# ruanjue/smartdenovo

Hardware: AMD Instinct MI355X
Metric: Gbp of candidate pairs aligned/sec (wtzmo all-vs-all) (higher is better)
Workload: dtype int32/int16

## Files before the change

### smartdenovo_amd/csrc/wtz_ctx.h

```cpp
struct wtz_switches {
	uint32_t xcd_group = 256;
	int zread = 1;
	int ext_fused = 1;
	int ext_pk = 1;
	int heavy_first = -1;
	int gap_lane = 1;
	int lane = 1;
	bool trace = false;
	bool fail_once = false;
	unsigned fail_at = 0, tfail_at = 0;
	int dm_first_big = 1;
	int sw_mode = 0;
	int gap_side = 0;
	bool profile = false;
};
static int env_int(const char *name, int dflt){ const char *e = getenv(name); return e ? atoi(e) : dflt; }
static void wtz_switches_read(wtz_switches *s){
	s->xcd_group = (uint32_t)env_int("WTZ_XCD_GROUP", (int)s->xcd_group);
	s->zread = env_int("WTZ_ZREAD", s->zread);
	s->ext_fused = env_int("WTZ_EXT_FUSED", s->ext_fused);
	s->ext_pk = env_int("WTZ_EXT_PK", s->ext_pk);
	s->heavy_first = env_int("WTZ_PAIR_HEAVY_FIRST", s->heavy_first);
	s->gap_lane = env_int("WTZ_GAP_LANE", s->gap_lane);
	s->lane = env_int("WTZ_WINALIGN_LANE", s->lane);
	s->trace = getenv("WTZ_STAGE_TRACE") != NULL;
	s->fail_once = getenv("WTZ_POOL_FAIL_ONCE") != NULL;
	s->fail_at = (unsigned)env_int("WTZ_POOL_FAIL_AT", 0);
	s->tfail_at = (unsigned)env_int("WTZ_TPOOL_FAIL_AT", 0);
#ifndef WTZ_EMUL
	s->dm_first_big = env_int("WTZ_DM_FIRST_BIG", s->dm_first_big);
	s->sw_mode = env_int("WTZ_SW_CHECK", 0) ? 2 : env_int("WTZ_SW_SCALAR", 0) ? 1 : 0;
	s->gap_side = env_int("WTZ_GAP_SIDESTREAM", 0) ? 1 : 0;
	s->profile = getenv("WTZ_PROFILE_PAIR") != NULL;
#endif
}

struct wtz_ctx {
	int device = 0;
	wtz_switches sw;
	struct zslot_t {
		std::vector<std::pair<void*, size_t> > parked, live;
		uint64_t *zoff = NULL; uint64_t n_z = 0; wtz_zindex_t Z; bool have = false; bool sub = false; uint64_t sub_cap = 0;
		std::vector<uint32_t> members;
		zslot_t(){ memset(&Z, 0, sizeof Z); }
		bool holds(uint32_t r) const { return have && (!sub || std::binary_search(members.begin(), members.end(), r)); }
	} zs[2];
#ifndef WTZ_EMUL
	hipStream_t stream = 0;
	hipStream_t stream_side = 0; hipEvent_t ev_side_fork = 0, ev_side_join = 0;
	hipStream_t stream_gap = 0; hipEvent_t ev_gap_fork = 0, ev_gap_join = 0;
#endif
	bool shares_indexes = false;
	void *kpark_p[2] = {NULL, NULL}; size_t kpark_b[2] = {0, 0}, klive_b[2] = {0, 0};
	wtz_arena arena;
	uint32_t cap_pairs = 0, cap_items = 0;
	wtz_params_t P = wtz_params_t(); wtz_params_t *dP = NULL;
	uint64_t *bits = NULL; uint64_t n_words = 0; uint64_t *rdoff = NULL; uint32_t *rdlen = NULL; uint32_t n_reads = 0;
	std::vector<uint32_t> h_rdlen;
	wtz_kslot_t *ktab = NULL; uint64_t kmask = 0; uint32_t *kseeds = NULL; uint64_t n_kocc = 0;
	uint64_t *pend_keys = NULL; uint32_t *pend_vals = NULL; uint64_t pend_tot = 0; uint64_t *pend_dk = NULL, *pend_dstart = NULL; uint32_t *pend_dc = NULL; uint64_t pend_nd = 0; uint32_t pend_beg = 0, pend_end = 0;
	uint64_t *cq_gptr = NULL; uint32_t cq_gcap = 0; bool cq_groups = false; std::vector<uint32_t> cq_ng;
	uint32_t idx_beg = 0, idx_end = 0; bool idx_len_sorted = false;
	wtz_pool_t *dpool = NULL; uint8_t *pool_base = NULL; uint64_t pool_bytes = 0, main_bytes = 0;
	uint32_t *d_qid = NULL, *d_cid = NULL; wtz_pairres_t *d_pairres = NULL; uint32_t n_pairs = 0; std::vector<wtz_pairres_t> h_pairres;
	wtz_alnres_dev_t *d_alnres = NULL; uint32_t n_items = 0; std::vector<wtz_alnres_dev_t> h_alnres;
	char *d_text = NULL; size_t cap_text = 0;
#ifndef WTZ_EMUL
	hipStream_t stream_copy = 0; hipEvent_t ev_text_ready = 0, ev_text_done[2] = {0, 0}; std::atomic<uint64_t> text_begun{0}, text_known_done{0}, text_ended{0};
#endif
	bool have_pairs = false, have_items = false;
	uint32_t *cq_thr = NULL;
	uint32_t *cq_q = NULL, *cq_nc = NULL; uint64_t *cq_cand = NULL; unsigned long long *cq_bytes = NULL; uint32_t cq_cap = 0, cq_n = 0; bool cq_pending = false; wtz_timer cq_tm;
	wtz_counters_t cnt = wtz_counters_t();
	uint64_t tpool_peak_call = 0, main_used_call = 0;
	int last_pool_fail = 0;
	double ext_use_ratio = 0.4; uint64_t tpool_last_used = 0;
	bool fused_ran = false;
	unsigned long long ext_fr_total = 0;
	unsigned long long ext_open_total = 0;
};

#ifndef WTZ_EMUL
#define CTX_ENTER(c) (void)hipSetDevice((c)->device); g_stream = (c)->stream; wtz_arena_scope arena_scope_(&(c)->arena)
#else
#define CTX_ENTER(c) wtz_arena_scope arena_scope_(&(c)->arena)
#endif

#define STAGE(c, name) do { if((c)->sw.trace){ (void)dev_sync(); fprintf(stderr, "[stage] %s\n", name); fflush(stderr); } } while(0)

static wtz_reads_t ctx_reads(const wtz_ctx *c){ wtz_reads_t R; R.bits = c->bits; R.rdoff = c->rdoff; R.rdlen = c->rdlen; R.n_reads = c->n_reads; return R; }
static wtz_env_t ctx_env(const wtz_ctx *c){ wtz_env_t V; V.R = ctx_reads(c); V.Z = c->zs[0].Z; V.ZQ = c->zs[1].have ? c->zs[1].Z : c->zs[0].Z; V.P = c->dP; V.pool = c->dpool; V.dm_first_big = (uint32_t)c->sw.dm_first_big; return V; }

static int tpool_reset(wtz_ctx *c){
	wtz_pool_t p; wtz_pool_init(&p, c->pool_base + c->main_bytes, c->pool_bytes - c->main_bytes, c->sw.tfail_at);
	return dev_h2d(c->dpool + 1, &p, sizeof p);
}
static int pool_reset(wtz_ctx *c){
	wtz_pool_t p; wtz_pool_init(&p, c->pool_base, c->main_bytes, c->sw.fail_at);
	CHK(dev_h2d(c->dpool, &p, sizeof p));
	c->tpool_peak_call = 0;
	return tpool_reset(c);
}
static int tpool_check(wtz_ctx *c, const char *stage){
	wtz_pool_t p; CHK(dev_d2h(&p, c->dpool + 1, sizeof p));
	const uint64_t u = p.used > p.cap ? p.cap : p.used;
	c->tpool_last_used = u;
	if(u > c->tpool_peak_call) c->tpool_peak_call = u;
	if(p.overflow && c->sw.fail_once) c->sw.tfail_at = 0;
	if(p.overflow) c->last_pool_fail = 2;
	if(p.overflow) return wtz_fail(WTZ_E_POOL, "%s: transient trace pool exhausted (%llu of %llu bytes requested); use a larger pool",
		stage, (unsigned long long)p.used, (unsigned long long)p.cap);
	return WTZ_OK;
}
static int pool_check(wtz_ctx *c, const char *stage){
	wtz_pool_t p; CHK(dev_d2h(&p, c->dpool, sizeof p));
	const uint64_t u = (p.used > p.cap ? p.cap : p.used);
	c->main_used_call = u;
	if(u + c->tpool_peak_call > c->cnt.pool_peak) c->cnt.pool_peak = u + c->tpool_peak_call;
	if(p.overflow && c->sw.fail_once) c->sw.fail_at = 0;
	if(p.overflow) c->last_pool_fail = 1;
	if(p.overflow) return wtz_fail(WTZ_E_POOL, "%s: device scratch pool exhausted (%llu of %llu bytes requested); use fewer items per call or a larger pool",
		stage, (unsigned long long)p.used, (unsigned long long)p.cap);
	return WTZ_OK;
}
extern "C" int wtz_device_count(void){
#ifndef WTZ_EMUL
	int n = 0; if(hipGetDeviceCount(&n) != hipSuccess) return 0; return n;
#else
	return 1;
#endif
}

extern "C" int wtz_device_memory(int device, uint64_t *free_bytes, uint64_t *total_bytes){
	if(!free_bytes || !total_bytes) return wtz_fail(WTZ_E_ARG, "null argument");
#ifndef WTZ_EMUL
	int prev = 0; HIPCHK(hipGetDevice(&prev)); HIPCHK(hipSetDevice(device));
	size_t fr = 0, tot = 0; const hipError_t e = hipMemGetInfo(&fr, &tot); (void)hipSetDevice(prev);
	if(e != hipSuccess) return wtz_fail(WTZ_E_HIP, "hipMemGetInfo: %s", hipGetErrorString(e));
	*free_bytes = fr; *total_bytes = tot;
#else
	(void)device; *free_bytes = *total_bytes = 16ull << 30;
#endif
	return WTZ_OK;
}

extern "C" int wtz_ctx_create(int device, const wtz_params_c *params, uint64_t pool_bytes, wtz_ctx_t **out){
	if(!params || !out) return wtz_fail(WTZ_E_ARG, "null argument");
	if(params->ksize < 5 || params->ksize > 32 || params->zsize < 5 || params->zsize > 16 || params->ksave < 1) return wtz_fail(WTZ_E_ARG, "k/z/S out of range (wtzmo.c:1658-1660)");
#ifndef WTZ_EMUL
	int ndev = 0;
	if(hipGetDeviceCount(&ndev) != hipSuccess || ndev == 0) return wtz_fail(WTZ_E_HIP, "no HIP device visible: libwtzmo_hip needs an MI355X (gfx950); there is no CPU fallback");
	if(device < 0 || device >= ndev) return wtz_fail(WTZ_E_ARG, "device %d out of range (%d visible)", device, ndev);
	HIPCHK(hipSetDevice(device));
#endif
	wtz_ctx *c = new wtz_ctx();
	c->device = device; c->P = *params; wtz_switches_read(&c->sw);
	c->pool_bytes = pool_bytes ? pool_bytes : (4ull << 30);
#ifndef WTZ_EMUL
	if(!pool_bytes){
		size_t fr = 0, tot = 0;
		if(hipMemGetInfo(&fr, &tot) == hipSuccess && fr / 20 * 9 > c->pool_bytes) c->pool_bytes = (uint64_t)(fr / 20 * 9);
		if(c->pool_bytes > (128ull << 30)) c->pool_bytes = 128ull << 30;
		if(const char *e = getenv("WTZ_DEFAULT_POOL_MB")){ const long long mb = atoll(e); if(mb >= 64 && ((uint64_t)mb << 20) < c->pool_bytes) c->pool_bytes = (uint64_t)mb << 20; }
	}
#endif
	c->pool_bytes &= ~(uint64_t)4095; c->main_bytes = (c->pool_bytes / 2) & ~(uint64_t)4095;
#ifndef WTZ_EMUL
	{ void *ab = NULL; const size_t acap = (size_t)3 << 29;
	  if(hipMalloc(&ab, acap) == hipSuccess){ c->arena.base = (uint8_t*)ab; c->arena.cap = acap; } }
	if(hipStreamCreateWithFlags(&c->stream, hipStreamNonBlocking) != hipSuccess
			|| hipStreamCreateWithFlags(&c->stream_side, hipStreamNonBlocking) != hipSuccess || hipEventCreateWithFlags(&c->ev_side_fork, hipEventDisableTiming) != hipSuccess
			|| hipEventCreateWithFlags(&c->ev_side_join, hipEventDisableTiming) != hipSuccess
			|| hipStreamCreateWithFlags(&c->stream_gap, hipStreamNonBlocking) != hipSuccess || hipEventCreateWithFlags(&c->ev_gap_fork, hipEventDisableTiming) != hipSuccess
			|| hipEventCreateWithFlags(&c->ev_gap_join, hipEventDisableTiming) != hipSuccess){ wtz_ctx_destroy(c); return wtz_fail(WTZ_E_HIP, "hipStreamCreate / hipEventCreate failed"); }
	g_stream = c->stream;
#endif
	int rc;
	if((rc = dev_alloc_persist((void**)&c->dP, sizeof(wtz_params_t))) || (rc = dev_h2d(c->dP, &c->P, sizeof(wtz_params_t))) ||
	   (rc = dev_alloc_persist((void**)&c->dpool, 2 * sizeof(wtz_pool_t)))){
		wtz_ctx_destroy(c); return rc;
	}
	for(;;){
#ifndef WTZ_EMUL
		if(!pool_bytes && c->pool_bytes > (4ull << 30)){
			if(hipMalloc((void**)&c->pool_base, c->pool_bytes) == hipSuccess){ rc = WTZ_OK; break; }
			(void)hipGetLastError();
			c->pool_base = NULL;
			uint64_t nb = c->pool_bytes / 2; if(nb < (4ull << 30)) nb = 4ull << 30;
			c->pool_bytes = nb & ~(uint64_t)4095; c->main_bytes = (c->pool_bytes / 2) & ~(uint64_t)4095;
			continue;
		}
#endif
		rc = dev_alloc_persist((void**)&c->pool_base, c->pool_bytes);
		break;
	}
	if(rc || (rc = pool_reset(c))){
		wtz_ctx_destroy(c); return rc;
	}
	*out = c;
	return WTZ_OK;
}

static void free_pending_index(wtz_ctx *c);
static void kpark(wtz_ctx *c, int w, void *p, size_t bytes){ if(!p) return; if(c->kpark_p[w]) dev_free_persist(c->kpark_p[w]); c->kpark_p[w] = p; c->kpark_b[w] = bytes; }
static void kflush(wtz_ctx *c){ for(int w = 0; w < 2; w++){ if(c->kpark_p[w]) dev_free_persist(c->kpark_p[w]); c->kpark_p[w] = NULL; c->kpark_b[w] = 0; } }
static int kalloc(wtz_ctx *c, int w, void **p, size_t n){
	if(c->kpark_p[w] && c->kpark_b[w] >= n && c->kpark_b[w] <= n + n / 8 + ((size_t)1 << 20)){ *p = c->kpark_p[w]; c->klive_b[w] = c->kpark_b[w]; c->kpark_p[w] = NULL; c->kpark_b[w] = 0; return WTZ_OK; }
	if(c->kpark_p[w]){ dev_free_persist(c->kpark_p[w]); c->kpark_p[w] = NULL; c->kpark_b[w] = 0; }
	int rc = dev_alloc_persist(p, n); if(rc == WTZ_OK) c->klive_b[w] = n; return rc;
}
static void free_kindex(wtz_ctx *c){
	if(!c->shares_indexes){
		if(c->klive_b[0]) kpark(c, 0, c->ktab, c->klive_b[0]); else dev_free_persist(c->ktab);
		if(c->klive_b[1]) kpark(c, 1, c->kseeds, c->klive_b[1]); else dev_free_persist(c->kseeds);
		c->klive_b[0] = c->klive_b[1] = 0;
	}
	c->ktab = NULL; c->kseeds = NULL; c->kmask = 0;
}
static int zalloc(wtz_ctx::zslot_t *z, void **p, size_t n){
	if(n == 0) n = 16;
	for(size_t i = 0; i < z->parked.size(); i++){
		if(z->parked[i].second >= n && z->parked[i].second <= n + n / 8 + 4096){
			*p = z->parked[i].first; z->live.push_back(z->parked[i]); z->parked.erase(z->parked.begin() + (long)i); return WTZ_OK;
		}
	}
	int rc = dev_alloc_persist(p, n); if(rc) return rc;
	z->live.push_back(std::make_pair(*p, n)); return WTZ_OK;
}
static void zpark_all(wtz_ctx::zslot_t *z){ for(size_t i = 0; i < z->live.size(); i++) z->parked.push_back(z->live[i]); z->live.clear(); }
static void zflush_parked(wtz_ctx::zslot_t *z){ for(size_t i = 0; i < z->parked.size(); i++) dev_free_persist(z->parked[i].first); z->parked.clear(); }
static void free_zindex(wtz_ctx *c){
	for(int k = 0; k < 2; k++){
		wtz_ctx::zslot_t *z = &c->zs[k];
		if(!c->shares_indexes){ zpark_all(z); zflush_parked(z); }
		z->zoff = NULL; memset(&z->Z, 0, sizeof z->Z); z->have = false; z->sub = false; z->sub_cap = 0; z->n_z = 0; z->members.clear();
	}
}
static void free_batch(wtz_ctx *c){ c->n_pairs = 0; c->n_items = 0; c->have_pairs = false; c->have_items = false; }
static void free_batch_storage(wtz_ctx *c){
	dev_free_persist(c->d_qid); dev_free_persist(c->d_cid); dev_free_persist(c->d_pairres); dev_free_persist(c->d_alnres);
	c->d_qid = c->d_cid = NULL; c->d_pairres = NULL; c->d_alnres = NULL; c->cap_pairs = c->cap_items = 0; free_batch(c);
}
static int reserve_pairs(wtz_ctx *c, uint32_t n){
	if(n <= c->cap_pairs && c->d_pairres) return WTZ_OK;
	uint32_t cap = c->cap_pairs ? c->cap_pairs : 4096; while(cap < n) cap *= 2;
	(void)dev_sync();
	dev_free_persist(c->d_qid); dev_free_persist(c->d_cid); dev_free_persist(c->d_pairres); c->d_qid = c->d_cid = NULL; c->d_pairres = NULL; c->cap_pairs = 0;
	CHK(dev_alloc_persist((void**)&c->d_qid, (size_t)cap * 4)); CHK(dev_alloc_persist((void**)&c->d_cid, (size_t)cap * 4));
	CHK(dev_alloc_persist((void**)&c->d_pairres, (size_t)cap * sizeof(wtz_pairres_t)));
	c->cap_pairs = cap; return WTZ_OK;
}
static int reserve_items(wtz_ctx *c, uint32_t m){
	if(m <= c->cap_items && c->d_alnres) return WTZ_OK;
	uint32_t cap = c->cap_items ? c->cap_items : 4096; while(cap < m) cap *= 2;
	(void)dev_sync();
	dev_free_persist(c->d_alnres); c->d_alnres = NULL; c->cap_items = 0;
	CHK(dev_alloc_persist((void**)&c->d_alnres, (size_t)cap * sizeof(wtz_alnres_dev_t)));
	c->cap_items = cap; return WTZ_OK;
}

extern "C" void wtz_ctx_destroy(wtz_ctx_t *c){
	if(!c) return;
	{ CTX_ENTER(c); (void)dev_sync(); }
	free_batch_storage(c); free_kindex(c); if(!c->shares_indexes) kflush(c); free_zindex(c);
	dev_free_persist(c->d_text);
	dev_free_persist(c->cq_q); dev_free_persist(c->cq_nc); dev_free_persist(c->cq_cand); dev_free_persist(c->cq_bytes); dev_free_persist(c->cq_thr); dev_free_persist(c->cq_gptr);
	free_pending_index(c);
#ifndef WTZ_EMUL
	arena_cache_flush(&c->arena);
	if(c->arena.base) (void)hipFree(c->arena.base);
#endif
	if(!c->shares_indexes){ dev_free_persist(c->bits); dev_free_persist(c->rdoff); dev_free_persist(c->rdlen); }
	dev_free_persist(c->dP); dev_free_persist(c->dpool); dev_free_persist(c->pool_base);
#ifndef WTZ_EMUL
	if(c->stream_side) (void)hipStreamDestroy(c->stream_side);
	if(c->stream_gap) (void)hipStreamDestroy(c->stream_gap);
	if(c->stream_copy){ (void)hipStreamSynchronize(c->stream_copy); (void)hipStreamDestroy(c->stream_copy); if(c->ev_text_ready) (void)hipEventDestroy(c->ev_text_ready); for(int k = 0; k < 2; k++) if(c->ev_text_done[k]) (void)hipEventDestroy(c->ev_text_done[k]); }
	{ hipEvent_t evs[4] = { c->ev_side_fork, c->ev_side_join, c->ev_gap_fork, c->ev_gap_join }; for(int k = 0; k < 4; k++) if(evs[k]) (void)hipEventDestroy(evs[k]); }
	if(c->stream) (void)hipStreamDestroy(c->stream);
#endif
	delete c;
}

extern "C" int wtz_ctx_clone(wtz_ctx_t *p, uint64_t pool_bytes, wtz_ctx_t **out){
	if(!p || !out) return wtz_fail(WTZ_E_ARG, "null argument");
	wtz_ctx_t *c = NULL;
	int rc = wtz_ctx_create(p->device, &p->P, pool_bytes ? pool_bytes : p->pool_bytes, &c);
	if(rc) return rc;
	c->shares_indexes = true;
	c->bits = p->bits; c->n_words = p->n_words; c->rdoff = p->rdoff; c->rdlen = p->rdlen; c->n_reads = p->n_reads; c->h_rdlen = p->h_rdlen;
	c->ktab = p->ktab; c->kmask = p->kmask; c->kseeds = p->kseeds; c->n_kocc = p->n_kocc;
	c->idx_beg = p->idx_beg; c->idx_end = p->idx_end; c->idx_len_sorted = p->idx_len_sorted;
	for(int k = 0; k < 2; k++){ c->zs[k].zoff = p->zs[k].zoff; c->zs[k].n_z = p->zs[k].n_z; c->zs[k].Z = p->zs[k].Z; c->zs[k].have = p->zs[k].have; c->zs[k].sub = p->zs[k].sub; c->zs[k].members = p->zs[k].members; }
	*out = c;
	return WTZ_OK;
}
```

### smartdenovo_amd/csrc/wtz_lib_align.h

```cpp
#ifndef WTZ_EMUL
WTZ_HD uint64_t wtz_ext_trace_need(int32_t qlen, int32_t tlen, int32_t init, int32_t W, int32_t M, int32_t O, int32_t E, int32_t T, int32_t *ql_out, int32_t *ncol_out){
	if(ql_out) *ql_out = 0;
	if(ncol_out) *ncol_out = 0;
	if(qlen <= 0 || tlen <= 0) return 0;
	if(init < 0) init = 0;
	int32_t ql, tl, n_col;
	wtz_ext_geometry(qlen, tlen, init, W, M, O, O, E, T, ql, tl, n_col);
	if(ql_out) *ql_out = ql;
	if(ncol_out) *ncol_out = n_col;
	const uint64_t c_reg = ((uint64_t)(n_col + 63) / 64 + 3) / 4, c_mw = ((uint64_t)(n_col + 255) / 256 + 3) / 4 * 4, c_gen = ((((uint64_t)(n_col + 63) / 64) | 1) + 3) / 4;
	uint64_t zrow = (c_reg > c_gen ? c_reg : c_gen) * 256; if(c_mw * 256 > zrow) zrow = c_mw * 256;
	uint64_t nb = ((uint64_t)(ql + 63) / 64) * 64 * zrow + (uint64_t)WTZ_TRACE_MAXCHUNK * 8 + (uint64_t)(ql + 2) * 4 + 256;
	if((n_col + 63) / 64 > 32 || (tl + 63) / 32 + 1 > 1032){
		uint64_t z = 1024; while(z < (uint64_t)ql * (uint64_t)n_col) z <<= 1;
		uint64_t r = 64; while(r < (uint64_t)tl + 3) r <<= 1;
		uint64_t zb = 64; while(zb < (uint64_t)ql + 2) zb <<= 1;
		nb = z + 8 * r + 4 * zb + 256;
	}
	return nb;
}
static uint64_t ext_trace_need(const wtz_ctx *c, int32_t qlen, int32_t tlen, int32_t init, int32_t W, int32_t *ql_out, int32_t *ncol_out){
	return wtz_ext_trace_need(qlen, tlen, init, W, c->P.M, c->P.O, c->P.E, c->P.T, ql_out, ncol_out);
}

static int run_stitch_fused(wtz_ctx *c, const wtz_env_t &V, const wtz_alnitem_t *d_items, wtz_stitch_state_t *d_st, wtz_extjob_t *d_jl, wtz_extjob_t *d_jr, const wtz_gapres_t *d_gaps, const int32_t *d_rgeo, uint32_t m){
	c->fused_ran = false;
	if(m == 0) return WTZ_OK;
	uint64_t *d_k = NULL; uint32_t *d_order = NULL; unsigned long long *d_acc = NULL;
	uint32_t *d_open = NULL;
	CHK(dev_alloc((void**)&d_k, (size_t)m * 8)); CHK(dev_alloc((void**)&d_order, (size_t)m * 4)); CHK(dev_alloc((void**)&d_acc, 24)); CHK(dev_set(d_acc, 0, 24));
	if(c->sw.ext_pk) CHK(dev_alloc((void**)&d_open, ((size_t)m + 1) * 4));
	{
		const int32_t pM = c->P.M, pO = c->P.O, pE = c->P.E, pT = c->P.T, pW = -c->P.ew;
		const bool use_pk = c->sw.ext_pk != 0; const wtz_params_t *dP = V.P;
		CHK(wtz_launch<K_misc>(m, [=] WTZ_LAMBDA (uint64_t t){
			const wtz_extjob_t &j = d_jl[t];
			int32_t qa = 0, qb = 0;
			unsigned long long nb = wtz_ext_trace_need(j.valid ? j.qlen : -1, j.tlen, 0, pW, pM, pO, pE, pT, &qa, (int32_t*)NULL);
			nb += wtz_ext_trace_need(d_rgeo[2 * t], d_rgeo[2 * t + 1], 0, pW, pM, pO, pE, pT, &qb, (int32_t*)NULL);
			const uint32_t rows = (uint32_t)qa + (uint32_t)qb;
			uint32_t to_fr = 0;
			if(use_pk){
				if(j.valid && j.qlen > 0 && j.tlen > 0){
					int32_t W = pW, ql = 0, tl = 0, nc = 0, bias, ng, sh; const int32_t in0 = j.init_score < 0 ? 0 : j.init_score;
					wtz_ext_geometry(j.qlen, j.tlen, in0, W, pM, pO, pO, pE, pT, ql, tl, nc);
					if(!wtz_pk_window(dP, in0, ql, tl, &bias, &ng, &sh)) to_fr = 1;
				}
				if(d_rgeo[2 * t] > 0 && d_rgeo[2 * t + 1] > 0){
					const wtz_stitch_state_t &st = d_st[t]; const wtz_alnitem_t &it = d_items[t];
					long long i_lo = st.x.score, gain = 0;
					if(j.valid && j.qlen > 0 && j.tlen > 0) gain = (long long)pM * (j.qlen < j.tlen ? j.qlen : j.tlen);
					const wtz_gapres_t *gp = d_gaps + (it.regs - d_items[0].regs);
					for(uint32_t k = st.first + 1; k < it.nwin; k++) if(it.regs[k].pass == 1) i_lo += (long long)gp[k].score + it.regs[k].x.score;
					int32_t W = pW, ql = 0, tl = 0, nc = 0;
					wtz_ext_geometry(d_rgeo[2 * t], d_rgeo[2 * t + 1], 0, W, pM, pO, pO, pE, pT, ql, tl, nc);
					if(!wtz_pk_window_range(dP, ql, tl, i_lo, i_lo + gain)) to_fr = 1;
				}
			}
			d_k[t] = ((uint64_t)to_fr << 32) | (uint64_t)(0xFFFFFFFFu - rows); d_order[t] = (uint32_t)t;
			if(to_fr) WTZ_ATOMIC_ADD64(&d_acc[2], 1ull);
			if(nb) WTZ_ATOMIC_ADD64(&d_acc[0], nb);
			if(rows) WTZ_ATOMIC_ADD64(&d_acc[1], (unsigned long long)rows);
		}));
	}
	CHK(dev_sort_pairs_u64_u32(d_k, d_order, m, 33));
	unsigned long long h_acc[3] = {0, 0, 0}; CHK(dev_d2h(h_acc, d_acc, 24));
	const uint64_t acc = h_acc[0]; const unsigned long long ext_sum = h_acc[1];
	const uint64_t budget = (c->pool_bytes - c->main_bytes) / 16 * 15;
	uint32_t ng = 1; while(ng < 4 && (double)acc * c->ext_use_ratio / ng > (double)budget) ng++;
	if((double)acc * c->ext_use_ratio / ng > (double)budget){ if(c->sw.profile) fprintf(stderr, "[ext-profile] fused launch declined: %u items, trace bounds %.1f GB x %.2f against %.1f GB\n", m, acc / 1e9, c->ext_use_ratio, budget / 1e9); return WTZ_OK; }
	double ms_l = 0; uint64_t used_sum = 0;
	for(uint32_t g = 0; g < ng; g++){
		const uint32_t mg = (m - g + ng - 1) / ng;
		if(mg == 0) continue;
		CHK(tpool_reset(c));
		wtz_timer te; te.start();
		if(c->sw.ext_pk){
			uint32_t n_fr = ng == 1 ? (uint32_t)h_acc[2] : 0u;
			if(n_fr > mg) n_fr = mg;
			CHK(dev_set(d_open, 0, 4));
			if(n_fr){
				HIPCHK(hipEventRecord(c->ev_side_fork, g_stream)); HIPCHK(hipStreamWaitEvent(c->stream_side, c->ev_side_fork, 0));
				WTZ_LAUNCH((wtz_kernel_stitch_ext_fr<1032>), n_fr, 64, WTZ_WAVE_LDS_BYTES, c->stream_side, V, d_items, d_st, d_jl, d_jr, d_gaps, (const uint32_t*)d_order + (mg - n_fr), n_fr, 1u, 0u);
				HIPCHK(hipEventRecord(c->ev_side_join, c->stream_side));
			}
			const uint32_t n_pk = mg - n_fr;
			if(n_pk){
				WTZ_LAUNCH((wtz_kernel_stitch_ext_pk<1032>), n_pk, 64, WTZ_PK_LDS_BYTES(1032), g_stream, V, d_items, d_st, d_jl, d_jr, d_gaps, (const uint32_t*)d_order, n_pk, ng, g, d_open);
			}
			if(n_fr) HIPCHK(hipStreamWaitEvent(g_stream, c->ev_side_join, 0));
			uint32_t n_open = 0; CHK(dev_d2h(&n_open, d_open, 4));
			c->ext_open_total += n_open; c->ext_fr_total += n_fr;
			if(n_open){ WTZ_LAUNCH((wtz_kernel_stitch_ext_fr<1032>), n_open, 64, WTZ_WAVE_LDS_BYTES, g_stream, V, d_items, d_st, d_jl, d_jr, d_gaps, (const uint32_t*)d_open + 1, n_open, 1u, 0u); }
		} else WTZ_LAUNCH((wtz_kernel_stitch_ext_fr<1032>), mg, 64, WTZ_WAVE_LDS_BYTES, g_stream, V, d_items, d_st, d_jl, d_jr, d_gaps, (const uint32_t*)d_order, mg, ng, g);
		ms_l += te.stop();
		{
			const int rc_t = tpool_check(c, "K-sw3 extension jobs (both ends on one wavefront)");
			if(rc_t != WTZ_OK){
				c->ext_use_ratio = c->ext_use_ratio * 2.0 > 1.0 ? 1.0 : c->ext_use_ratio * 2.0;
				return rc_t;
			}
		}
		used_sum += c->tpool_last_used;
	}
	c->cnt.ms_ext += ms_l; c->cnt.n_extjobs += 2ull * m;
	c->fused_ran = true;
	if(c->sw.profile) fprintf(stderr, "[ext-profile] fused launch: %u items in %u group(s), rows (upper bound) sum %llu, %.2f ms; items of the 32-bit form so far: dealt %llu, declined by the packed form %llu\n", m, ng, ext_sum, ms_l, c->ext_fr_total, c->ext_open_total);
	c->tpool_last_used = used_sum;
	if(acc){ const double seen = 1.3 * (double)c->tpool_last_used / (double)acc, keep = c->ext_use_ratio * 0.9; c->ext_use_ratio = seen > keep ? seen : keep; if(c->ext_use_ratio < 0.2) c->ext_use_ratio = 0.2; if(c->ext_use_ratio > 1.0) c->ext_use_ratio = 1.0; }
	return WTZ_OK;
}
#endif

static int run_extjobs(wtz_ctx *c, const wtz_env_t &V, wtz_extjob_t *d_jobs, uint32_t m, bool leftover = false){
	if(m == 0) return WTZ_OK;
#ifdef WTZ_EMUL
	(void)c; (void)leftover;
	return wtz_launch_wave<K_extjob_scalar>(m, [=] WTZ_LAMBDA (uint64_t t){ wtz_task_extjob_scalar((uint32_t)t, V, d_jobs); });
#else
	if(leftover){
		if(!c->fused_ran) leftover = false;
		else {
			wtz_timer te; te.start();
			WTZ_LAUNCH((wtz_kernel_extjobs<2048, 1032>), m, 64, 0, g_stream, d_jobs, (const uint32_t*)NULL, m, V.P, V.pool, V.pool + 1);
			c->cnt.ms_ext += te.stop();
			return tpool_check(c, "K-sw3 extension jobs");
		}
	}
	const int mode = c->sw.sw_mode;
	if(mode == 1) return wtz_launch_wave<K_extjob_scalar>(m, [=] WTZ_LAMBDA (uint64_t t){ wtz_task_extjob_scalar((uint32_t)t, V, d_jobs); });
	std::vector<wtz_extjob_t> ref;
	if(mode == 2){
		wtz_extjob_t *d_copy = NULL; CHK(dev_alloc((void**)&d_copy, (size_t)m * sizeof(wtz_extjob_t)));
		HIPCHK(hipMemcpyAsync(d_copy, d_jobs, (size_t)m * sizeof(wtz_extjob_t), hipMemcpyDeviceToDevice, g_stream));
		CHK(wtz_launch_wave<K_extjob_scalar>(m, [=] WTZ_LAMBDA (uint64_t t){ wtz_task_extjob_scalar((uint32_t)t, V, d_copy); }));
		CHK(dev_sync());
		ref.resize(m); CHK(dev_d2h(ref.data(), d_copy, (size_t)m * sizeof(wtz_extjob_t)));
	}
	uint32_t *d_order = NULL; unsigned long long ext_sum = 0; int32_t ext_max = 0;
	std::vector<uint32_t> ord(m); std::vector<uint64_t> need(m); std::vector<uint8_t> cw(m, 0);
	unsigned long long geo_n[9] = {0}, geo_rows[9] = {0}, geo_cells[9] = {0};
	{
		int32_t *d_key = NULL; CHK(dev_alloc((void**)&d_key, (size_t)m * 16));
		CHK(wtz_launch<K_misc>(m, [=] WTZ_LAMBDA (uint64_t t){ const wtz_extjob_t &j = d_jobs[t]; d_key[4 * t] = j.valid ? j.qlen : -1; d_key[4 * t + 1] = j.tlen; d_key[4 * t + 2] = j.init_score; d_key[4 * t + 3] = j.W; }));
		std::vector<int32_t> key4((size_t)m * 4); CHK(dev_d2h(key4.data(), d_key, (size_t)m * 16));
		std::vector<int32_t> key(m);
		for(uint32_t i = 0; i < m; i++){ key[i] = key4[(size_t)i * 4]; if(key[i] > 0){ ext_sum += (unsigned long long)key[i]; if(key[i] > ext_max) ext_max = key[i]; } }
		std::vector<int32_t> rows(m, -1);
		for(uint32_t i = 0; i < m; i++){
			const int32_t qlen = key4[(size_t)i * 4], tlen = key4[(size_t)i * 4 + 1];
			need[i] = 0;
			if(qlen <= 0 || tlen <= 0) continue;
			int32_t ql = 0, n_col = 0;
			need[i] = ext_trace_need(c, qlen, tlen, key4[(size_t)i * 4 + 2], key4[(size_t)i * 4 + 3], &ql, &n_col);
			cw[i] = (uint8_t)((n_col + 63) / 64 > 255 ? 255 : (n_col + 63) / 64);
			rows[i] = ql;
			if(c->sw.profile){ const int b = (n_col + 63) / 64 > 32 ? 8 : ((n_col + 63) / 64 - 1) / 4; geo_n[b]++; geo_rows[b] += (unsigned long long)ql; geo_cells[b] += (unsigned long long)ql * (unsigned long long)n_col; }
		}
		for(uint32_t i = 0; i < m; i++) ord[i] = i;
		std::stable_sort(ord.begin(), ord.end(), [&](uint32_t a, uint32_t b){ return rows[a] > rows[b]; });
		CHK(dev_alloc((void**)&d_order, (size_t)m * 4)); CHK(dev_h2d(d_order, ord.data(), (size_t)m * 4));
		if(c->sw.profile){
			fprintf(stderr, "[ext-profile] geometry by columns per lane (upper bounds):");
			for(int b = 0; b < 9; b++) if(geo_n[b]) fprintf(stderr, " C<=%d: %llu jobs %.1f Mrows %.1f Gcells;", b < 8 ? 4 * b + 4 : 999, geo_n[b], (double)geo_rows[b] / 1e6, (double)geo_cells[b] / 1e9);
			fprintf(stderr, "\n");
		}
	}
	{
		wtz_timer te; te.start();
		const uint64_t budget = (c->pool_bytes - c->main_bytes) / 16 * 15;
		uint32_t g0 = 0, n_groups = 0;
		while(g0 < m){
			uint32_t g1 = g0; uint64_t acc = 0;
			while(g1 < m && (g1 == g0 || acc + need[ord[g1]] <= budget)){ acc += need[ord[g1]]; g1++; }
			CHK(tpool_reset(c));
			if(c->sw.ext_pk){
				WTZ_LAUNCH((wtz_kernel_extjobs_pk<1032>), g1 - g0, 64, 0, g_stream, d_jobs, (const uint32_t*)d_order + g0, g1 - g0, V.P, V.pool, V.pool + 1);
			}
			WTZ_LAUNCH((wtz_kernel_extjobs_fr<1032>), g1 - g0, 64, 0, g_stream, d_jobs, (const uint32_t*)d_order + g0, g1 - g0, V.P, V.pool, V.pool + 1);
			WTZ_LAUNCH((wtz_kernel_extjobs<2048, 1032>), g1 - g0, 64, 0, g_stream, d_jobs, (const uint32_t*)d_order + g0, g1 - g0, V.P, V.pool, V.pool + 1);
			if(g1 < m || n_groups){ CHK(dev_sync()); CHK(tpool_check(c, "K-sw3 extension jobs")); }
			g0 = g1; n_groups++;
		}
		const double ms_l = te.stop();
		CHK(tpool_check(c, "K-sw3 extension jobs"));
		c->cnt.ms_ext += ms_l; c->cnt.n_extjobs += m;
		if(c->sw.profile){
			std::vector<int32_t> key(m); uint32_t nv = 0, n256 = 0, n512 = 0, n1k = 0, n2k = 0, n4k = 0; unsigned long long s512 = 0;
			CHK(dev_sync());
			{ std::vector<wtz_extjob_t> jj(m); CHK(dev_d2h(jj.data(), d_jobs, (size_t)m * sizeof(wtz_extjob_t))); uint32_t nd[4] = {0, 0, 0, 0}; for(uint32_t i = 0; i < m; i++){ key[i] = jj[i].valid ? jj[i].x.qe : -1; if(jj[i].valid) nd[jj[i].done & 3]++; }
			  if(const char *dp = getenv("WTZ_EXT_DUMP")){
				if(FILE *df = fopen(dp, "ab")){ for(uint32_t i = 0; i < m; i++) if(jj[i].valid){ const int32_t r[8] = {jj[i].qlen, jj[i].tlen, jj[i].init_score, jj[i].W, jj[i].x.qe, jj[i].x.te, (int32_t)(jj[i].cells > 0x7FFFFFFFull ? 0x7FFFFFFF : jj[i].cells), (int32_t)jj[i].done}; fwrite(r, 4, 8, df); } fclose(df); } }
			  fprintf(stderr, "[ext-profile] %u launch group(s); valid jobs finished by: nobody %u, 32-bit frame form %u, packed form or general kernel %u\n", n_groups, nd[0], nd[1], nd[3]); }
			for(uint32_t i = 0; i < m; i++){ if(key[i] < 0) continue; nv++; if(key[i] >= 256) n256++; if(key[i] >= 512){ n512++; s512 += key[i]; } if(key[i] >= 1024) n1k++; if(key[i] >= 2048) n2k++; if(key[i] >= 4096) n4k++; }
			fprintf(stderr, "[ext-profile] %u jobs (%u valid), rows (upper bound) sum %llu max %d, %.2f ms; qe>=256 %u >=512 %u (sum %llu) >=1k %u >=2k %u >=4k %u; transient pool peak %.2f GB\n", m, nv, ext_sum, ext_max, ms_l, n256, n512, s512, n1k, n2k, n4k, c->tpool_peak_call / 1073741824.0);
		}
	}
	if(mode == 2){
		CHK(dev_sync());
		std::vector<wtz_extjob_t> got(m); CHK(dev_d2h(got.data(), d_jobs, (size_t)m * sizeof(wtz_extjob_t)));
		for(uint32_t i = 0; i < m; i++){
			if(!got[i].valid) continue;
			if(memcmp(&got[i].x, &ref[i].x, sizeof(wtz_aln_t)) || got[i].cigar_len != ref[i].cigar_len || got[i].cells != ref[i].cells)
				return wtz_fail(WTZ_E_STATE, "K-sw3 wave kernel differs from the scalar body on job %u: qlen %d tlen %d init %d W %d; score %d/%d qe %d/%d te %d/%d aln %d/%d cigar %u/%u cells %llu/%llu",
					i, got[i].qlen, got[i].tlen, got[i].init_score, got[i].W, got[i].x.score, ref[i].x.score, got[i].x.qe, ref[i].x.qe, got[i].x.te, ref[i].x.te,
					got[i].x.aln, ref[i].x.aln, got[i].cigar_len, ref[i].cigar_len, (unsigned long long)got[i].cells, (unsigned long long)ref[i].cells);
			if(got[i].cigar_len){
				std::vector<uint32_t> a(got[i].cigar_len), b(got[i].cigar_len);
				CHK(dev_d2h(a.data(), got[i].cigar, a.size() * 4)); CHK(dev_d2h(b.data(), ref[i].cigar, b.size() * 4));
				if(a != b) return wtz_fail(WTZ_E_STATE, "K-sw3 wave kernel: CIGAR differs on job %u", i);
			}
		}
	}
	return WTZ_OK;
#endif
}

#ifdef WTZ_EMUL
#define WTZ_HOST_WAVE 1u
#else
#define WTZ_HOST_WAVE 64u
#endif
static int pool_alloc_host(wtz_ctx *c, int which, size_t bytes, void **out){
	unsigned long long *d_p = NULL; CHK(dev_alloc((void**)&d_p, 8));
	wtz_pool_t *pool = c->dpool + which;
	CHK(wtz_launch<K_poolalloc>(1, [=] WTZ_LAMBDA (uint64_t){ *d_p = (unsigned long long)(uintptr_t)wtz_pool_alloc(pool, bytes); }));
	unsigned long long h = 0; CHK(dev_d2h(&h, d_p, 8));
	if(h == 0) return wtz_fail(WTZ_E_POOL, "device scratch pool exhausted (%zu bytes for the K-sw1 problem lists)", bytes);
	*out = (void*)(uintptr_t)h; return WTZ_OK;
}
static uint32_t lane_classes(const uint32_t ccnt[4], wtz_lclass_t *L){
	uint32_t lo = 0, wv = 0;
	for(int k = 0; k < 4; k++){ const uint32_t n = ccnt[3 - k]; L->lo[k] = lo; L->hi[k] = lo + n; wv += (n + WTZ_HOST_WAVE - 1) / WTZ_HOST_WAVE; L->wend[k] = wv; lo += n; }
	return wv;
}
static size_t carve_bytes(size_t n, size_t elem){ return (n * elem + 255) & ~(size_t)255; }
template<typename T> static void carve(uint8_t *&blk, T *&out, size_t n){ out = (T*)blk; blk += carve_bytes(n, sizeof(T)); }
template<typename KEYS> static int sort_leftovers(uint32_t *d_list, uint32_t nl, KEYS launch_keys){
	if(nl <= 64) return WTZ_OK;
	uint64_t *d_k2 = NULL; CHK(dev_alloc((void**)&d_k2, (size_t)nl * 8));
	CHK(launch_keys(d_k2));
	return dev_sort_pairs_u64_u32(d_k2, d_list + 1, nl, 32);
}
static int run_winalign_lane(wtz_ctx *c, const wtz_env_t &V, const wtz_wintask_t *d_wt, uint64_t nwt, const wtz_alnitem_t *d_items, uint32_t *d_fb, uint32_t *n_fb){
	*n_fb = 0;
	if(nwt == 0) return WTZ_OK;
	const bool prof = c->sw.profile; double tp[8] = {0, 0, 0, 0, 0, 0, 0, 0}, tp0 = 0;
	if(prof){ (void)dev_sync(); tp0 = wtz_wall(); }
	auto lap = [&](int k){ if(prof){ (void)dev_sync(); const double t = wtz_wall(); tp[k] += t - tp0; tp0 = t; } };
	uint32_t *d_na = NULL, *d_woff = NULL;
	CHK(dev_alloc((void**)&d_na, (nwt + 1) * 4)); CHK(dev_alloc((void**)&d_woff, (nwt + 1) * 4));
	CHK(dev_set(d_na, 0, (nwt + 1) * 4));
	CHK(wtz_launch<K_lcount>(nwt, [=] WTZ_LAMBDA (uint64_t t){ wtz_task_lcount((uint32_t)t, d_wt, d_items, d_na); }));
	CHK(dev_exclusive_scan_u32(d_na, d_woff, nwt + 1));
	uint32_t NS = 0; CHK(dev_d2h(&NS, d_woff + nwt, 4));
	lap(0);
	wtz_lprob_t *d_prob = NULL; uint32_t *d_cap = NULL, *d_roff = NULL, *d_val = NULL, *d_ccnt = NULL, *d_uidx = NULL, *d_nu = NULL; uint64_t *d_key = NULL; uint8_t *d_flag = NULL; wtz_lres_t *d_res = NULL;
	{
		const size_t nsp = (size_t)NS + 64;
		uint8_t *blk = NULL; CHK(pool_alloc_host(c, 0, carve_bytes(nsp, sizeof(wtz_lprob_t)) + carve_bytes(nsp, sizeof(wtz_lres_t)) + 4 * carve_bytes(nsp, 4) + carve_bytes(nsp, 8), (void**)&blk));
		carve(blk, d_prob, nsp); carve(blk, d_res, nsp); carve(blk, d_cap, nsp); carve(blk, d_roff, nsp); carve(blk, d_val, nsp); carve(blk, d_uidx, nsp); carve(blk, d_key, nsp);
	}
	CHK(dev_alloc((void**)&d_flag, nwt + 16)); CHK(dev_alloc((void**)&d_nu, (nwt + 1) * 4)); CHK(dev_alloc((void**)&d_ccnt, 32)); CHK(dev_set(d_ccnt, 0, 32));
	CHK(dev_set(d_cap, 0, ((size_t)NS + 1) * 4));
	CHK(dev_set(d_res, 0, ((size_t)NS + 1) * sizeof(wtz_lres_t)));
	CHK(wtz_launch<K_lplan>(nwt, [=] WTZ_LAMBDA (uint64_t t){ wtz_task_lplan((uint32_t)t, V, d_wt, d_items, d_woff, d_prob, d_cap, d_key, d_val, d_flag, d_ccnt, d_uidx, d_nu); }));
	lap(1);
	CHK(dev_exclusive_scan_u32(d_cap, d_roff, (uint64_t)NS + 1));
	uint32_t NR = 0, ccnt[4] = {0, 0, 0, 0};
	CHK(dev_d2h(&NR, d_roff + NS, 4)); CHK(dev_d2h(ccnt, d_ccnt, 16));
	uint32_t *d_runs = NULL; CHK(pool_alloc_host(c, 0, ((size_t)NR + 16) * 4, (void**)&d_runs));
	lap(2);
	CHK(dev_sort_pairs_u64_u32(d_key, d_val, NS, 16));
	lap(3);
	CHK(dev_set(d_fb, 0, 4));
	{
		const uint32_t *d_ord = d_val; const wtz_lprob_t *pp = d_prob; const uint32_t *ro = d_roff; uint32_t *rn = d_runs; wtz_lres_t *rs = d_res;
		wtz_lclass_t L; const uint32_t wv = lane_classes(ccnt, &L);
		uint64_t *d_wtr = NULL; uint32_t *d_wrm = NULL;
		CHK(dev_alloc((void**)&d_wtr, ((size_t)wv + 1) * 8)); CHK(dev_alloc((void**)&d_wrm, ((size_t)wv + 1) * 4)); CHK(dev_set(d_wtr, 0, ((size_t)wv + 1) * 8));
		if(wv) CHK(wtz_launch_coop<K_ldp>(wv, [=] WTZ_LAMBDA (uint64_t t){ wtz_task_ldp_all((uint32_t)t, L, V, d_wt, d_items, d_ord, pp, rs, d_wtr, d_wrm); }, 0));
		lap(4);
		if(wv) CHK(wtz_launch_coop<K_ltb>(wv, [=] WTZ_LAMBDA (uint64_t t){ wtz_task_ltb_all((uint32_t)t, L, V, d_wt, d_items, d_ord, pp, ro, rn, rs, d_wtr, d_wrm); }, 0));
		lap(6);
		CHK(wtz_launch<K_lfold>(nwt, [=] WTZ_LAMBDA (uint64_t t){ wtz_task_lfold((uint32_t)t, V, d_wt, d_items, d_woff, pp, ro, rn, rs, d_flag, d_fb, d_uidx, d_nu); }));
	}
	CHK(dev_d2h(n_fb, d_fb, 4));
	{
		const uint32_t nl = *n_fb; const uint32_t *lst = d_fb + 1;
		CHK(sort_leftovers(d_fb, nl, [&](uint64_t *d_k2){ return wtz_launch<K_misc>(nl, [=] WTZ_LAMBDA (uint64_t i){
			const wtz_wintask_t tk = d_wt[lst[i]];
			const wtz_win_t &w = d_items[tk.item].win[tk.widx];
			d_k2[i] = 0xFFFFFFFFull - (unsigned long long)(w.anchors[1] - w.anchors[0]);
		}); }));
	}
	lap(5);
	if(c->sw.profile) fprintf(stderr, "[lane-profile] %llu windows, %u anchor slots, K-sw1 problems by band class <=16 / <=32 / <=64 / <=104: %u / %u / %u / %u, %u run entries, %u windows left to the chained kernel; ms: count+scan %.2f plan %.2f scan+alloc %.2f sort %.2f dp %.2f traceback %.2f fold %.2f\n",
		(unsigned long long)nwt, NS, ccnt[0], ccnt[1], ccnt[2], ccnt[3], NR, *n_fb, tp[0] * 1e3, tp[1] * 1e3, tp[2] * 1e3, tp[3] * 1e3, tp[4] * 1e3, tp[6] * 1e3, tp[5] * 1e3);
	return WTZ_OK;
}

static int run_gap_lane(wtz_ctx *c, const wtz_env_t &V, const wtz_wintask_t *d_wt, uint64_t nwt, const wtz_alnitem_t *d_items, wtz_gapres_t *d_gaps, uint32_t *d_list, uint32_t *n_list){
	*n_list = 0;
	if(nwt == 0) return WTZ_OK;
	wtz_lgap_t *d_gp = NULL; uint32_t *d_cap = NULL, *d_roff = NULL, *d_val = NULL, *d_ccnt = NULL; uint64_t *d_key = NULL; uint8_t *d_done = NULL;
	{
		const size_t nsp = (size_t)nwt + 64;
		uint8_t *blk = NULL; CHK(pool_alloc_host(c, 0, carve_bytes(nsp, sizeof(wtz_lgap_t)) + 3 * carve_bytes(nsp, 4) + carve_bytes(nsp, 8) + carve_bytes(nsp, 1), (void**)&blk));
		carve(blk, d_gp, nsp); carve(blk, d_cap, nsp); carve(blk, d_roff, nsp); carve(blk, d_val, nsp); carve(blk, d_key, nsp); carve(blk, d_done, nsp);
	}
	CHK(dev_alloc((void**)&d_ccnt, 32)); CHK(dev_set(d_ccnt, 0, 32));
	CHK(dev_set(d_cap, 0, ((size_t)nwt + 1) * 4));
	CHK(wtz_launch<K_gplan>(nwt, [=] WTZ_LAMBDA (uint64_t t){ wtz_task_gplan((uint32_t)t, V, d_wt, d_items, d_gaps, d_gp, d_cap, d_key, d_val, d_done, d_ccnt); }));
	CHK(dev_exclusive_scan_u32(d_cap, d_roff, nwt + 1));
	uint32_t NR = 0, ccnt[4] = {0, 0, 0, 0};
	CHK(dev_d2h(&NR, d_roff + nwt, 4)); CHK(dev_d2h(ccnt, d_ccnt, 16));
	uint32_t *d_runs = NULL; CHK(pool_alloc_host(c, 0, ((size_t)NR + 16) * 4, (void**)&d_runs));
	CHK(dev_sort_pairs_u64_u32(d_key, d_val, nwt, 18));
	CHK(dev_set(d_list, 0, 4));
	{
		const uint32_t *d_ord = d_val; const wtz_lgap_t *gp = d_gp; const uint32_t *ro = d_roff; uint32_t *rn = d_runs; uint8_t *dn = d_done;
		wtz_lclass_t L; const uint32_t wv = lane_classes(ccnt, &L);
		uint64_t *d_wtr = NULL; uint32_t *d_wrm = NULL; wtz_lres_t *d_res = NULL;
		CHK(dev_alloc((void**)&d_wtr, ((size_t)wv + 1) * 8)); CHK(dev_alloc((void**)&d_wrm, ((size_t)wv + 1) * 4)); CHK(dev_set(d_wtr, 0, ((size_t)wv + 1) * 8));
		CHK(pool_alloc_host(c, 0, ((size_t)nwt + 1) * sizeof(wtz_lres_t), (void**)&d_res)); CHK(dev_set(d_res, 0, ((size_t)nwt + 1) * sizeof(wtz_lres_t)));
		if(wv) CHK(wtz_launch_coop<K_gdp>(wv, [=] WTZ_LAMBDA (uint64_t t){ wtz_task_gdp_all((uint32_t)t, L, V, d_wt, d_items, d_ord, gp, d_res, d_wtr, d_wrm); }, 0));
		if(wv) CHK(wtz_launch_coop<K_gtb>(wv, [=] WTZ_LAMBDA (uint64_t t){ wtz_task_gtb_all((uint32_t)t, L, V, d_wt, d_items, d_ord, gp, ro, rn, d_res, d_gaps, dn, d_wtr, d_wrm); }, 0));
		CHK(wtz_launch<K_glist>(nwt, [=] WTZ_LAMBDA (uint64_t t){ wtz_task_glist((uint32_t)t, dn, d_list); }));
	}
	CHK(dev_d2h(n_list, d_list, 4));
	{
		const uint32_t nl = *n_list; const wtz_lgap_t *gp = d_gp; const uint32_t *lst = d_list + 1;
		CHK(sort_leftovers(d_list, nl, [&](uint64_t *d_k2){ return wtz_launch<K_misc>(nl, [=] WTZ_LAMBDA (uint64_t i){
			const wtz_lgap_t G = gp[lst[i]];
			const int32_t nc = G.dq < 2 * G.w + 1 ? G.dq : 2 * G.w + 1;
			unsigned long long wgt = (unsigned long long)(G.dt > 0 ? G.dt : 0) * (unsigned long long)((nc > 0 ? nc : 0) / 64 + 1);
			if(wgt > 0xFFFFFFFEull) wgt = 0xFFFFFFFEull;
			d_k2[i] = 0xFFFFFFFFull - wgt;
		}); }));
	}
	if(c->sw.profile) fprintf(stderr, "[lane-profile] %llu window slots, K-sw2 gaps by band class <=16 / <=32 / <=64 / <=104: %u / %u / %u / %u, %u left to the wavefront kernel\n",
		(unsigned long long)nwt, ccnt[0], ccnt[1], ccnt[2], ccnt[3], *n_list);
	return WTZ_OK;
}

static int run_winalign_chained(wtz_ctx *c, const wtz_env_t &V, const wtz_wintask_t *d_wt, const wtz_alnitem_t *d_items, uint32_t *d_list, uint64_t n, uint32_t *n_redone = NULL){
	if(n_redone) *n_redone = 0;
	if(n == 0) return WTZ_OK;
#ifdef WTZ_EMUL
	if(d_list) return wtz_launch_coop<K_winalign>(n, [=] WTZ_LAMBDA (uint64_t t){ wtz_task_winalign((uint32_t)t, V, d_wt, d_items, (uint32_t*)NULL, d_list); }, WTZ_WINALIGN_LDS_BYTES + WTZ_WINALIGN_QW_BYTES);
	return wtz_launch_coop<K_winalign>(n, [=] WTZ_LAMBDA (uint64_t t){ wtz_task_winalign((uint32_t)t, V, d_wt, d_items); }, WTZ_WINALIGN_LDS_BYTES + WTZ_WINALIGN_QW_BYTES);
#else
	uint32_t *d_defer = NULL, n_def = 0; CHK(dev_alloc((void**)&d_defer, ((size_t)n + 1) * 4)); CHK(dev_set(d_defer, 0, 4));
	if(d_list) CHK(wtz_launch_coop<K_winalign>(n, [=] WTZ_LAMBDA (uint64_t t){ wtz_task_winalign<false>((uint32_t)t, V, d_wt, d_items, d_defer, d_list); }, WTZ_WINALIGN_LDS_BYTES + WTZ_WINALIGN_QW_BYTES));
	else CHK(wtz_launch_coop<K_winalign>(n, [=] WTZ_LAMBDA (uint64_t t){ wtz_task_winalign<false>((uint32_t)t, V, d_wt, d_items, d_defer, NULL); }, WTZ_WINALIGN_LDS_BYTES + WTZ_WINALIGN_QW_BYTES));
	CHK(dev_d2h(&n_def, d_defer, 4));
	if(n_def) CHK(wtz_launch_coop<K_winalign_big>(n_def, [=] WTZ_LAMBDA (uint64_t t){ wtz_task_winalign<true>((uint32_t)t, V, d_wt, d_items, NULL, d_defer); }, WTZ_WINALIGN_LDS_BYTES + WTZ_WINALIGN_QW_BYTES));
	if(n_redone) *n_redone = n_def;
	return WTZ_OK;
#endif
}

static int compare_lane_with_chained(const wtz_reg_t *ra, const wtz_reg_t *rb, uint64_t nreg){
	unsigned int *d_bad = NULL; CHK(dev_alloc((void**)&d_bad, 16)); CHK(dev_set(d_bad, 0, 16));
	CHK(wtz_launch<K_misc>(nreg, [=] WTZ_LAMBDA (uint64_t i){
		const wtz_reg_t &a = ra[i], &b = rb[i];
		bool same = a.pass == 2 || b.pass == 2 || (a.x.score == b.x.score && a.x.tb == b.x.tb && a.x.te == b.x.te && a.x.qb == b.x.qb && a.x.qe == b.x.qe && a.x.aln == b.x.aln && a.x.mat == b.x.mat && a.x.mis == b.x.mis && a.x.ins == b.x.ins && a.x.del == b.x.del && a.pass == b.pass && a.cigar_len == b.cigar_len && (a.cells == b.cells || a.cells == 0 || b.cells == 0));
		if(same && a.pass != 2 && b.pass != 2) for(uint32_t k = 0; k < a.cigar_len; k++) if(a.cigar[k] != b.cigar[k]){ same = false; break; }
		if(!same){ const unsigned int z = WTZ_ATOMIC_INC32(&d_bad[0]); if(z == 0) d_bad[1] = (unsigned int)i; }
	}));
	unsigned int hb[4]; CHK(dev_d2h(hb, d_bad, 16));
	if(hb[0]){
		wtz_reg_t a, b; CHK(dev_d2h(&a, ra + hb[1], sizeof a)); CHK(dev_d2h(&b, rb + hb[1], sizeof b));
		return wtz_fail(WTZ_E_STATE, "K-sw1 lane pipeline differs from the chained kernel on %u of %llu windows; first: window slot %u chained/lane score %d/%d tb %d/%d te %d/%d qb %d/%d qe %d/%d aln %d/%d mat %d/%d mis %d/%d ins %d/%d del %d/%d cigar %u/%u pass %u/%u cells %llu/%llu",
			hb[0], (unsigned long long)nreg, hb[1], a.x.score, b.x.score, a.x.tb, b.x.tb, a.x.te, b.x.te, a.x.qb, b.x.qb, a.x.qe, b.x.qe, a.x.aln, b.x.aln, a.x.mat, b.x.mat, a.x.mis, b.x.mis, a.x.ins, b.x.ins, a.x.del, b.x.del, a.cigar_len, b.cigar_len, a.pass, b.pass, a.cells, b.cells);
	}
	return WTZ_OK;
}

static int run_gap_wave(wtz_ctx *c, const wtz_env_t &V, const wtz_wintask_t *d_wt, const wtz_alnitem_t *d_items, wtz_gapres_t *d_gaps, const uint32_t *d_glist, uint32_t n_glist, uint64_t nwt){
#ifdef WTZ_EMUL
	(void)c; (void)nwt;
	return wtz_launch_coop<K_gap>(n_glist, [=] WTZ_LAMBDA (uint64_t t){ wtz_task_gap((uint32_t)t, V, d_wt, d_items, d_gaps, (uint32_t*)NULL, (const uint32_t*)d_glist); }, WTZ_GAP_LDS_BYTES);
#else
	uint32_t *d_defer = NULL, n_def = 0; CHK(dev_alloc((void**)&d_defer, (size_t)(nwt + 1) * 4)); CHK(dev_set(d_defer, 0, 4));
	STAGE(c, "K_gap");
	CHK(wtz_launch_coop<K_gap>(n_glist, [=] WTZ_LAMBDA (uint64_t t){ wtz_task_gap((uint32_t)t, V, d_wt, d_items, d_gaps, d_defer, (const uint32_t*)d_glist, 0u); }, WTZ_GAP_LDS_BYTES));
	CHK(dev_d2h(&n_def, d_defer, 4));
	if(n_def) CHK(wtz_launch_coop<K_gap_wide>(n_def, [=] WTZ_LAMBDA (uint64_t t){ wtz_task_gap((uint32_t)t, V, d_wt, d_items, d_gaps, NULL, d_defer, (uint32_t)WTZ_GAP_WIDE_LDS_BYTES); }, WTZ_GAP_WIDE_LDS_BYTES));
	if(c->sw.profile){ CHK(dev_sync()); fprintf(stderr, "[gap-profile] %llu window slots, %u wide gaps redone with 72 KB of LDS\n", (unsigned long long)nwt, n_def); }
	return WTZ_OK;
#endif
}

#ifdef WTZ_EMUL
static int check_right_geometry(const int32_t *d_rgeo, const wtz_extjob_t *d_jr, const wtz_stitch_state_t *d_st, uint32_t m){
	for(uint32_t t = 0; t < m; t++){
		const wtz_extjob_t &jr = d_jr[t];
		const int32_t pq = d_rgeo[2 * (size_t)t], pt = d_rgeo[2 * (size_t)t + 1];
		if(jr.valid ? (pq != jr.qlen || pt != jr.tlen) : (pq >= 0 && !d_st[t].bad))
			return wtz_fail(WTZ_E_STATE, "stitch: predicted right extension of item %u (%d x %d) differs from the one K_stitch_mid asks for (valid %u: %d x %d)", t, pq, pt, jr.valid, jr.qlen, jr.tlen);
	}
	return WTZ_OK;
}
#endif

extern "C" int wtz_pairs_align(wtz_ctx_t *c, const uint32_t *pair_idx, const uint8_t *dir, uint32_t m, wtz_aln_result_t *out){
	if(!c || !c->have_pairs) return wtz_fail(WTZ_E_STATE, "wtz_pairs_align before wtz_pairs_seed");
	if(m == 0) return WTZ_OK;
	CTX_ENTER(c);
	if(!pair_idx || !dir || !out) return wtz_fail(WTZ_E_ARG, "null argument");
	c->n_items = 0; c->have_items = false;
	const bool prof_wall = c->sw.profile; double tw[6] = {0, 0, 0, 0, 0, 0}; double tw0 = prof_wall ? wtz_wall() : 0;
	auto lapw = [&](int k){ if(prof_wall){ const double t = wtz_wall(); tw[k] += t - tw0; tw0 = t; } };
	CHK(reserve_items(c, m));
	std::vector<wtz_alnitem_t> items(m); uint64_t nreg = 0;
	std::vector<uint32_t> h_q(c->n_pairs), h_c(c->n_pairs);
	CHK(dev_d2h(h_q.data(), c->d_qid, (size_t)c->n_pairs * 4)); CHK(dev_d2h(h_c.data(), c->d_cid, (size_t)c->n_pairs * 4));
	for(uint32_t i = 0; i < m; i++){
		if(pair_idx[i] >= c->n_pairs || dir[i] > 1) return wtz_fail(WTZ_E_ARG, "align item %u out of range", i);
		const wtz_pairres_t &r = c->h_pairres[pair_idx[i]];
		wtz_alnitem_t it; it.q = h_q[pair_idx[i]]; it.c = h_c[pair_idx[i]]; it.dir = dir[i];
		it.win = r.win[dir[i]]; it.anchors = r.anchors[dir[i]]; it.nwin = r.nwin[dir[i]]; it.regs = (wtz_reg_t*)(uintptr_t)nreg;
		nreg += it.nwin; items[i] = it;
	}
	const uint64_t nwt = (size_t)nreg;
	wtz_reg_t *d_regs = NULL; wtz_alnitem_t *d_items = NULL; wtz_wintask_t *d_wt = NULL;
	CHK(dev_alloc((void**)&d_regs, (size_t)(nreg + 1) * sizeof(wtz_reg_t)));
	for(uint32_t i = 0; i < m; i++) items[i].regs = d_regs + (uintptr_t)items[i].regs;
	CHK(dev_alloc((void**)&d_items, (size_t)m * sizeof(wtz_alnitem_t))); CHK(dev_h2d(d_items, items.data(), (size_t)m * sizeof(wtz_alnitem_t)));
	CHK(dev_alloc((void**)&d_wt, (size_t)(nreg + 1) * sizeof(wtz_wintask_t)));
	{ const wtz_alnitem_t *di = d_items; wtz_wintask_t *dw = d_wt; const wtz_reg_t *r0 = d_regs;
	  CHK(wtz_launch<K_misc>(m, [=] WTZ_LAMBDA (uint64_t i){ const wtz_alnitem_t &it = di[i]; wtz_wintask_t *w = dw + (it.regs - r0); for(uint32_t k = 0; k < it.nwin; k++){ w[k].item = (uint32_t)i; w[k].widx = k; } })); }
	const wtz_env_t V = ctx_env(c); wtz_alnres_dev_t *d_res = c->d_alnres;
	lapw(0);
	wtz_timer tm; tm.start();
	wtz_reg_t *d_regs_chk = NULL;
	if(c->sw.lane){
		uint32_t *d_fb = NULL, n_fb = 0;
		CHK(dev_alloc((void**)&d_fb, (nwt + 1) * 4));
		STAGE(c, "K-sw1 lane pipeline");
		CHK(run_winalign_lane(c, V, d_wt, nwt, d_items, d_fb, &n_fb));
		CHK(run_winalign_chained(c, V, d_wt, d_items, d_fb, n_fb));
		if(c->sw.lane == 2){ CHK(dev_sync()); CHK(dev_alloc((void**)&d_regs_chk, (size_t)(nreg + 1) * sizeof(wtz_reg_t))); CHK(dev_d2d(d_regs_chk, d_regs, (size_t)nreg * sizeof(wtz_reg_t))); }
	}
	if(c->sw.lane == 0 || c->sw.lane == 2){
		uint32_t n_redone = 0;
		STAGE(c, "K_winalign");
		CHK(run_winalign_chained(c, V, d_wt, d_items, NULL, nwt, &n_redone));
		if(c->sw.profile) fprintf(stderr, "[winalign-profile] %zu windows, %u redone by the full task\n", (size_t)nreg, n_redone);
	}
	CHK(dev_sync());
	if(d_regs_chk) CHK(compare_lane_with_chained(d_regs, d_regs_chk, nreg));
	c->cnt.ms_winalign += tm.stop(); c->cnt.n_winalign += (size_t)nreg;
	lapw(1);
	tm.start();
	wtz_stitch_state_t *d_st = NULL; wtz_extjob_t *d_jl = NULL, *d_jr = NULL; wtz_gapres_t *d_gaps = NULL; int32_t *d_rgeo = NULL;
	CHK(dev_alloc((void**)&d_st, (size_t)m * sizeof(wtz_stitch_state_t)));
	CHK(dev_alloc((void**)&d_jl, (size_t)m * sizeof(wtz_extjob_t))); CHK(dev_alloc((void**)&d_jr, (size_t)m * sizeof(wtz_extjob_t)));
	CHK(dev_alloc((void**)&d_gaps, (size_t)(nreg + 1) * sizeof(wtz_gapres_t)));
#ifndef WTZ_EMUL
	const bool fused = c->sw.ext_fused && c->sw.sw_mode == 0, gap_side = c->sw.gap_side != 0;
	if(fused) CHK(dev_alloc((void**)&d_rgeo, (size_t)m * 8));
#else
	const bool fused = false, gap_side = false;
	CHK(dev_alloc((void**)&d_rgeo, (size_t)m * 8));
#endif
	STAGE(c, "K_stitch_left");
	CHK(wtz_launch_wave<K_stitch_left>(m, [=] WTZ_LAMBDA (uint64_t t){ wtz_task_stitch_left((uint32_t)t, V, d_items, d_st, d_jl, d_rgeo); }));
	uint32_t *d_glist = NULL, n_glist = (uint32_t)nwt;
	wtz_timer tgap; tgap.start();
	if(c->sw.gap_lane){
		CHK(dev_alloc((void**)&d_glist, (size_t)(nwt + 1) * 4));
		STAGE(c, "K-sw2 lane pipeline");
		CHK(run_gap_lane(c, V, d_wt, nwt, d_items, d_gaps, d_glist, &n_glist));
	}
#ifndef WTZ_EMUL
	if(gap_side){ HIPCHK(hipEventRecord(c->ev_gap_fork, g_stream)); HIPCHK(hipStreamWaitEvent(c->stream_gap, c->ev_gap_fork, 0)); }
	{ wtz_stream_scope on_gap_stream(gap_side ? c->stream_gap : g_stream); CHK(run_gap_wave(c, V, d_wt, d_items, d_gaps, d_glist, n_glist, nwt)); }
	if(gap_side) HIPCHK(hipEventRecord(c->ev_gap_join, c->stream_gap));
#else
	CHK(run_gap_wave(c, V, d_wt, d_items, d_gaps, d_glist, n_glist, nwt));
#endif
	if(!gap_side) tgap.lap();
#ifndef WTZ_EMUL
	if(fused){
		if(gap_side) HIPCHK(hipStreamWaitEvent(g_stream, c->ev_gap_join, 0));
		STAGE(c, "extjobs left + join + right on one wavefront"); CHK(run_stitch_fused(c, V, d_items, d_st, d_jl, d_jr, d_gaps, d_rgeo, m));
	}
#endif
	STAGE(c, "extjobs left");
	CHK(run_extjobs(c, V, d_jl, m, fused));
#ifndef WTZ_EMUL
	if(gap_side) HIPCHK(hipStreamWaitEvent(g_stream, c->ev_gap_join, 0));
#endif
	if(!gap_side) c->cnt.ms_gap += tgap.read();
	STAGE(c, "K_stitch_mid");
	CHK(wtz_launch_coop<K_stitch_mid>(m, [=] WTZ_LAMBDA (uint64_t t){ wtz_task_stitch_mid((uint32_t)t, V, d_items, d_st, d_jl, d_jr, d_gaps); }));
	STAGE(c, "extjobs right");
#ifdef WTZ_EMUL
	CHK(check_right_geometry(d_rgeo, d_jr, d_st, m));
#endif
	CHK(run_extjobs(c, V, d_jr, m, fused));
	STAGE(c, "K_stitch_fin");
	CHK(wtz_launch_coop<K_stitch_fin>(m, [=] WTZ_LAMBDA (uint64_t t){ wtz_task_stitch_fin((uint32_t)t, V, d_items, d_st, d_jl, d_jr, d_res); }));
	if(c->P.refine) STAGE(c, "K_refine");
	if(c->P.refine) CHK(wtz_launch_coop<K_refine>(m, [=] WTZ_LAMBDA (uint64_t t){ wtz_task_refine((uint32_t)t, V, d_items, d_res); }, WTZ_REFINE_LDS_BYTES));
	CHK(dev_sync());
	c->cnt.ms_stitch += tm.stop(); c->cnt.n_stitch += m;
	lapw(2);
	c->h_alnres.resize(m); c->n_items = m; c->have_items = true;
	CHK(dev_d2h(c->h_alnres.data(), c->d_alnres, (size_t)m * sizeof(wtz_alnres_dev_t)));
	CHK(pool_check(c, "wtz_pairs_align"));
	uint64_t coff = 0, toff = 0;
	for(uint32_t i = 0; i < m; i++){
		const wtz_alnres_dev_t &r = c->h_alnres[i];
		if(r.bad) return wtz_fail(WTZ_E_POOL, "wtz_pairs_align: item %u ran out of scratch", i);
		wtz_aln_result_t o; memset(&o, 0, sizeof o);
		o.score = r.x.score; o.tb = r.x.tb; o.te = r.x.te; o.qb = r.x.qb; o.qe = r.x.qe; o.aln = r.x.aln; o.mat = r.x.mat; o.mis = r.x.mis; o.ins = r.x.ins; o.del = r.x.del;
		o.n_regs = r.n_regs; o.cigar_len = r.cigar_len; o.cigar_off = coff; coff += r.cigar_len; o.text_len = r.text_len; o.text_off = toff; toff += r.text_len;
		c->cnt.cells_shift += r.cells_shift; c->cnt.cells_fixed += r.cells_fixed; c->cnt.cells_global += r.cells_global;
		out[i] = o;
	}
	lapw(3);
	if(prof_wall) fprintf(stderr, "[align-profile] %u items: host wall ms prep %.2f winalign %.2f stitch %.2f results %.2f\n", m, tw[0] * 1e3, tw[1] * 1e3, tw[2] * 1e3, tw[3] * 1e3);
	return WTZ_OK;
}
```

### smartdenovo_amd/csrc/wtz_tasks.h

```cpp
#ifndef WTZ_TASKS_H
#define WTZ_TASKS_H

#include "wtz_sw.h"
#include "wtz_sw_wave.h"
#include "wtz_sw_lane.h"
#include "wtz_dotmatrix.h"

typedef struct {
	wtz_reads_t R; wtz_zindex_t Z; const wtz_params_t *P; wtz_pool_t *pool;
	wtz_zindex_t ZQ;
	uint32_t dm_first_big;
} wtz_env_t;

#define WTZ_WAVE_LDS_BYTES 8192
#ifndef WTZ_GAP_LDS_BYTES
#define WTZ_GAP_LDS_BYTES 12288
#endif
#ifndef WTZ_PAIR_LDS_BYTES
#define WTZ_PAIR_LDS_BYTES 8192
#endif
#ifndef WTZ_PAIR_DM_LDS_BYTES
#define WTZ_PAIR_DM_LDS_BYTES 24576
#endif
#if defined(__HIP_DEVICE_COMPILE__)
WTZ_D int32_t *wtz_wave_scratch(){ extern __shared__ int32_t wtz_dyn_lds[]; return wtz_dyn_lds; }
#else
WTZ_COOP_HOST int32_t *wtz_wave_scratch(){ return NULL; }
#endif

#if defined(WTZ_DEBUG_CRUMBS) && defined(__HIPCC__)
__device__ unsigned int *wtz_crumbs = NULL;
#endif
#if defined(WTZ_DEBUG_CRUMBS) && defined(__HIP_DEVICE_COMPILE__)
#define WTZ_CRUMB(t, code) do { if(wtz_crumbs && WTZ_LANE == 0) __hip_atomic_store(&wtz_crumbs[t], (unsigned int)(code), __ATOMIC_RELAXED, __HIP_MEMORY_SCOPE_SYSTEM); } while(0)
#else
#define WTZ_CRUMB(t, code) do { } while(0)
#endif
#define WTZ_PAIR_NEEDS_ZBIG (-3)
template<int ENGINE = -1, bool ZBIG = true, bool REGION = false>
WTZ_HD void wtz_task_pair(uint32_t t, const wtz_env_t &V, const uint32_t *qid, const uint32_t *cid, wtz_pairres_t *res, const int32_t *reg_beg = NULL, const int32_t *reg_end = NULL){
	const wtz_params_t *P = V.P;
	const int32_t rtb = REGION ? reg_beg[t] : 0, rte = REGION ? reg_end[t] : 0;
	const bool dm = ENGINE < 0 ? (P->dot_matrix != 0) : (ENGINE == 1);
	const uint32_t q = qid[t], c = cid[t];
	wtz_pairres_t r; memset(&r, 0, sizeof r);
	wtz_zhit_t *hits = NULL; uint32_t n = 0;
#if defined(__HIP_DEVICE_COMPILE__)
#define WTZ_TICK() ((uint64_t)clock64())
#else
#define WTZ_TICK() ((uint64_t)0)
#endif
	const uint64_t tk0 = WTZ_TICK();
	WTZ_CRUMB(t, 1);
	const bool aux = P->aux_strand != 0;
#if defined(__HIP_DEVICE_COMPILE__)
	const bool ok0 = wtz_zmatch_coop<REGION>(V.ZQ, V.Z, q, c, V.R.rdlen[c], P->max_kmer_var, V.pool, &hits, &n, aux, (uint32_t*)wtz_wave_scratch(), dm ? (uint32_t)WTZ_PAIR_DM_LDS_BYTES : (uint32_t)WTZ_PAIR_LDS_BYTES, rtb, rte);
#else
	const bool ok0 = wtz_zmatch_coop<REGION>(V.ZQ, V.Z, q, c, V.R.rdlen[c], P->max_kmer_var, V.pool, &hits, &n, aux, NULL, 0, rtb, rte);
#endif
	const bool ok = wtz_coop_bcast32(ok0 ? 1u : 0u) != 0;
	n = wtz_coop_bcast32(n);
	hits = (wtz_zhit_t*)(uintptr_t)wtz_coop_bcast64((uint64_t)(uintptr_t)hits);
	const uint64_t tk1 = WTZ_TICK();
	WTZ_CRUMB(t, 2 | (n << 8));
	wtz_zhit_t *sorted = NULL;
#if defined(__HIP_DEVICE_COMPILE__)
	__threadfence_block();
	if(ok && (aux ? n > 0 : n * P->zsize >= P->ztot)){
		int pbad = 0;
		if(dm) sorted = wtz_sort_hits_wave<1>(hits, n, V.pool, (uint64_t*)wtz_wave_scratch(), WTZ_PAIR_DM_LDS_BYTES / 8, &pbad);
		else              sorted = wtz_sort_hits_wave<0>(hits, n, V.pool, (uint64_t*)wtz_wave_scratch(), WTZ_PAIR_LDS_BYTES / 8, &pbad);
		if(wtz_coop_bcast32((uint32_t)pbad)) r.bad = 1;
		sorted = (wtz_zhit_t*)(uintptr_t)wtz_coop_bcast64((uint64_t)(uintptr_t)sorted);
	}
#endif
	const uint32_t lane = WTZ_LANE;
	WTZ_CRUMB(t, 3 | (n << 8));
	if(!ok || r.bad){ r.bad = 1; if(lane == 0) res[t] = r; WTZ_CRUMB(t, 0xFF); return; }
	r.n_hits = n;
	if(aux ? n == 0 : n * P->zsize < P->ztot){ r.gate = 0; if(lane == 0) res[t] = r; WTZ_CRUMB(t, 0xFF); return; }
	r.gate = 1;
	if(dm){
		wtz_vec<wtz_zhit_t> cache; cache.a = sorted ? sorted : hits; cache.n = n; cache.cap = n + 2; cache.pool = V.pool; cache.bad = 0;
		const uint64_t tk2 = WTZ_TICK();
		uint64_t tkd = 0;
#if defined(__HIP_DEVICE_COMPILE__)
		uint8_t *dlds = (uint8_t*)wtz_wave_scratch();
#else
		static thread_local uint64_t emul_dm_lds[WTZ_PAIR_DM_LDS_BYTES / 8];
		uint8_t *dlds = (uint8_t*)emul_dm_lds;
#endif
		wtz_dm_result_t d = wtz_dot_matrix_align(cache, V.pool, (int32_t)V.R.rdlen[q], (int32_t)V.R.rdlen[c], P, &r.bad, sorted != NULL, &tkd, dlds, WTZ_PAIR_DM_LDS_BYTES, true, V.dm_first_big != 0);
		if(lane != 0) return;
		if(d.dir == -2){ r.anchors[0] = cache.a; r.nanchors[0] = cache.n; }
		r.dm_score = d.score; r.dm_qb = d.qb; r.dm_qe = d.qe; r.dm_tb = d.tb; r.dm_te = d.te; r.dm_dir = d.dir;
		{ const uint64_t tk3 = WTZ_TICK(); r.tick[0] = (uint32_t)((tk1 - tk0) >> 10); r.tick[1] = (uint32_t)((tk2 - tk1) >> 10); r.tick[2] = (uint32_t)((tkd - tk2) >> 10); r.tick[3] = (uint32_t)((tk3 - tk0) >> 10); }
		res[t] = r; return;
	}
	if(sorted) hits = sorted;
	else { WTZ_CRUMB(t, 4 | (n << 8)); if(lane == 0) wtz_sort_exact(hits, (size_t)n, wtz_gt_off12()); WTZ_WAVE_SYNC(); }
	WTZ_CRUMB(t, 5 | (n << 8));
	const uint64_t tk2 = WTZ_TICK();
	wtz_winscratch_t sc;
	{
		uint64_t pa = 0;
		if(lane == 0) pa = (uint64_t)(uintptr_t)wtz_pool_alloc(V.pool, (size_t)(n + 2) * (4 * 7 + 8 + sizeof(wtz_zhit_t)) + 16);
		pa = wtz_coop_bcast64(pa);
		sc.ts = (uint32_t*)(uintptr_t)pa;
	}
	if(sc.ts == NULL){ r.bad = 1; if(lane == 0) res[t] = r; WTZ_CRUMB(t, 0xFF); return; }
	sc.as = (int32_t*)(sc.ts + (n + 2)); sc.wb = sc.ts + 2 * (n + 2); sc.we = sc.ts + 3 * (n + 2); sc.wo = sc.ts + 4 * (n + 2); sc.wf = sc.ts + 5 * (n + 2); sc.wd = sc.ts + 6 * (n + 2);
	sc.tk = (uint64_t*)(sc.ts + 7 * (n + 2) + ((7 * (n + 2)) & 1)); sc.ztmp = (wtz_zhit_t*)(sc.tk + (n + 2));
#if defined(__HIP_DEVICE_COMPILE__)
	sc.lds = (uint64_t*)wtz_wave_scratch();
#else
	static thread_local uint64_t emul_lds[WTZ_PAIR_LDS_BYTES / 8];
	sc.lds = emul_lds;
#endif
	sc.lds_u64 = WTZ_PAIR_LDS_BYTES / 8;
	sc.big = NULL; sc.big_u64 = 0; sc.need_big = 0;
#ifndef WTZ_MERGE_SCALAR
	wtz_merge_prepare(hits, n, sc, P->kwin);
#endif
	for(uint32_t dir = 0; dir < 2; dir++){
		wtz_vec<wtz_win_t> wins; wtz_vec<wtz_zhit_t> anchors;
		wins.a = NULL; wins.n = wins.cap = 0; wins.pool = V.pool; wins.bad = 0;
		anchors.a = NULL; anchors.n = anchors.cap = 0; anchors.pool = V.pool; anchors.bad = 0;
		if(lane == 0){ wins.init(V.pool, 16); anchors.init(V.pool, n + 16); }
		WTZ_CRUMB(t, (6 + dir) | (n << 8));
		const unsigned long long ptm = WTZ_PROF_T(); (void)ptm;
#ifdef WTZ_MERGE_SCALAR
		const uint32_t nw = wtz_merge_windows_coop<ZBIG>(hits, n, dir, wins, anchors, sc, P->zsize, P->kwin, P->kstep, P->zovl);
#else
		const uint32_t nw = wtz_merge_windows_wave<ZBIG>(hits, n, dir, wins, anchors, sc, P->zsize, P->kwin, P->kstep, P->zovl);
#endif
		WTZ_PROF_ADD(63, ptm);
		if(!ZBIG && sc.need_big){
			if(lane == 0){ wtz_pairres_t r2; memset(&r2, 0, sizeof r2); r2.n_hits = r.n_hits; r2.gate = 1; r2.dm_dir = WTZ_PAIR_NEEDS_ZBIG; res[t] = r2; }
			WTZ_CRUMB(t, 0xFF);
			return;
		}
		WTZ_CRUMB(t, (8 + dir) | (n << 8));
		if(wtz_coop_bcast32((uint32_t)(wins.bad | anchors.bad))){ r.bad = 1; continue; }
		if(nw == 0) continue;
		const unsigned long long ptc = WTZ_PROF_T(); (void)ptc;
		WTZ_WAVE_SYNC();
		const uint32_t wn = wtz_coop_bcast32(wins.n);
		wtz_win_t *wa = (wtz_win_t*)(uintptr_t)wtz_coop_bcast64((uint64_t)(uintptr_t)wins.a);
		int32_t *mem = NULL;
		if(wn > 64u || WTZ_NLANES == 1u){
			uint64_t pa = 0;
			if(lane == 0) pa = (uint64_t)(uintptr_t)wtz_pool_alloc(V.pool, (size_t)wn * 8 + 8);
			mem = (int32_t*)(uintptr_t)wtz_coop_bcast64(pa);
			if(mem == NULL){ r.bad = 1; continue; }
		}
		r.ovl[dir] = WTZ_OVL29(wtz_chain_windows_wave(wa, wn, P->W, mem));
		if(r.ovl[dir] < P->ztot) continue;
		const uint32_t k = wtz_keep_chain_members(wa, wn);
		r.nwin[dir] = k; r.win[dir] = wa; r.anchors[dir] = anchors.a; r.nanchors[dir] = anchors.n;
		WTZ_PROF_ADD(62, ptc);
	}
	if(lane != 0) return;
	{ const uint64_t tk3 = WTZ_TICK(); r.tick[0] = (uint32_t)((tk1 - tk0) >> 10); r.tick[1] = (uint32_t)((tk2 - tk1) >> 10); r.tick[2] = (uint32_t)((tk3 - tk2) >> 10); r.tick[3] = (uint32_t)((tk3 - tk0) >> 10); }
	res[t] = r;
	WTZ_CRUMB(t, 0xFF);
}

WTZ_HD void wtz_task_pair_dm_big(uint32_t t, const wtz_env_t &V, const uint32_t *list, const uint32_t *qid, const uint32_t *cid, wtz_pairres_t *res, uint32_t lds_bytes, bool last, bool big){
	const wtz_params_t *P = V.P;
	const uint32_t pi = list[t], q = qid[pi], c = cid[pi];
	wtz_pairres_t r = res[pi];
	wtz_vec<wtz_zhit_t> cache; cache.a = r.anchors[0]; cache.n = r.nanchors[0]; cache.cap = cache.n + 2; cache.pool = V.pool; cache.bad = 0;
	uint64_t tkd = 0;
#if defined(__HIP_DEVICE_COMPILE__)
	uint8_t *dlds = (uint8_t*)wtz_wave_scratch();
	wtz_dm_result_t d = wtz_dot_matrix_align(cache, V.pool, (int32_t)V.R.rdlen[q], (int32_t)V.R.rdlen[c], P, &r.bad, true, &tkd, dlds, lds_bytes, !last, big);
#else
	(void)lds_bytes; (void)last; (void)big;
	wtz_dm_result_t d = wtz_dot_matrix_align(cache, V.pool, (int32_t)V.R.rdlen[q], (int32_t)V.R.rdlen[c], P, &r.bad, true, &tkd, (uint8_t*)NULL, 0, false, false);
#endif
	if(WTZ_LANE != 0) return;
	r.dm_score = d.score; r.dm_qb = d.qb; r.dm_qe = d.qe; r.dm_tb = d.tb; r.dm_te = d.te; r.dm_dir = d.dir;
	res[pi] = r;
}

typedef struct {
	uint32_t item;
	uint32_t widx;
} wtz_wintask_t;

typedef struct { wtz_aln_t x; uint32_t *cigar; uint32_t cigar_len; uint32_t pass; unsigned long long cells; } wtz_reg_t;

typedef struct {
	uint32_t q, c, dir;
	const wtz_win_t *win; const wtz_zhit_t *anchors; uint32_t nwin;
	wtz_reg_t *regs;
} wtz_alnitem_t;

typedef struct {
	wtz_aln_t x; uint32_t n_regs; uint32_t cigar_len; uint32_t *cigar; int32_t bad;
	unsigned long long cells_shift, cells_fixed, cells_global;
	uint32_t text_len;
} wtz_alnres_dev_t;

WTZ_HD uint32_t wtz_cigar_text_len(const uint32_t *c, uint32_t n){
	uint32_t k = 0;
	for(uint32_t i = 0; i < n; i++){ uint32_t len = c[i] >> 4; if(len == 0) continue; uint32_t d = 1; while(len >= 10){ len /= 10; d++; } k += d + 1; }
	return k;
}
WTZ_HD void wtz_cigar_text_write(const uint32_t *c, uint32_t n, char *s){
	uint32_t k = 0;
	for(uint32_t i = 0; i < n; i++){
		uint32_t op = c[i] & 0xF, len = c[i] >> 4;
		if(len == 0) continue;
		char d[12]; int nd = 0;
		while(len){ d[nd++] = (char)('0' + len % 10); len /= 10; }
		while(nd) s[k++] = d[--nd];
		s[k++] = op == 0 ? 'M' : (op == 1 ? 'I' : 'D');
	}
}

WTZ_HD bool wtz_cigar_reserve_coop(wtz_cigar_t &c, uint32_t want){
	if(want <= c.cap) return true;
	uint32_t cap = c.cap ? c.cap : 16; while(cap < want) cap <<= 1;
	uint64_t a = 0;
	if(WTZ_LANE == 0) a = (uint64_t)(uintptr_t)wtz_pool_alloc(c.pool, (size_t)cap * 4);
	a = wtz_coop_bcast64(a);
	uint32_t *b = (uint32_t*)(uintptr_t)a;
	if(b == NULL){ c.bad = 1; return false; }
	for(uint32_t i = WTZ_LANE; i < c.n; i += WTZ_NLANES) b[i] = c.a[i];
	WTZ_WAVE_SYNC();
	c.a = b; c.cap = cap; return true;
}
WTZ_HD void wtz_cigar_concat_coop(wtz_cigar_t &c, const uint32_t *src, uint32_t n){
	if(n == 0) return;
	uint32_t k0 = 0;
	if(c.n && (c.a[c.n - 1] & 0xFu) == (src[0] & 0xFu)){ if(WTZ_LANE == 0) c.a[c.n - 1] += src[0] & 0xFFFFFFF0u; k0 = 1; }
	if(!wtz_cigar_reserve_coop(c, c.n + n)) return;
	for(uint32_t k = k0 + WTZ_LANE; k < n; k += WTZ_NLANES) c.a[c.n + k - k0] = src[k];
	c.n += n - k0;
	WTZ_WAVE_SYNC();
}
WTZ_HD void wtz_cigar_reverse_coop(uint32_t *a, uint32_t n){
	for(uint32_t i = WTZ_LANE; i < n / 2; i += WTZ_NLANES){ const uint32_t t = a[i]; a[i] = a[n - 1 - i]; a[n - 1 - i] = t; }
	WTZ_WAVE_SYNC();
}
template<typename PF>
WTZ_HD bool wtz_cigar_join_coop(wtz_cigar_t &c, uint32_t np, PF piece, uint32_t *lds, uint32_t lds_words){
	if((uint64_t)np * 6u > lds_words) return false;
	const uint32_t lane = WTZ_LANE;
	uint32_t *LB = lds, *LN = lds + np, *LF = lds + 2 * np, *LW = lds + 3 * np; uint64_t *LS = (uint64_t*)(lds + 4 * np);
	uint32_t carry_valid = c.n ? 1u : 0u, carry_last = c.n ? c.a[c.n - 1] : 0u, total = 0;
	for(uint32_t p0 = 0; p0 < np; p0 += WTZ_NLANES){
		const uint32_t p = p0 + lane;
		const uint32_t *src = NULL; uint32_t n = 0, rev = 0, fw = 0, lw = 0;
		if(p < np){ piece(p, &src, &n, &rev); if(n){ fw = rev ? src[n - 1] : src[0]; lw = rev ? src[0] : src[n - 1]; } }
		const unsigned long long mask = wtz_coop_ballot(n != 0);
		const unsigned long long below = mask & ((1ull << lane) - 1ull);
		const uint32_t from = below ? 63u - (uint32_t)__builtin_clzll(below) : 0u;
		const uint32_t plw = wtz_coop_shfl32(lw, from);
		const uint32_t prev = below ? plw : carry_last; const bool prev_ok = below ? true : (carry_valid != 0);
		const uint32_t merged = (n && prev_ok && (fw & 0xFu) == (prev & 0xFu)) ? 1u : 0u;
		uint32_t tot; const uint32_t ex = wtz_coop_excl_scan(n - merged, &tot);
		if(p < np){ LB[p] = total + ex; LN[p] = n; LF[p] = merged | (rev << 1); LW[p] = fw; LS[p] = (uint64_t)(uintptr_t)src; }
		if(mask){ const uint32_t top = 63u - (uint32_t)__builtin_clzll(mask); carry_last = wtz_coop_lane32(lw, top); carry_valid = 1; }
		total += tot;
	}
	WTZ_WAVE_SYNC();
	const uint32_t n0 = c.n;
	if(!wtz_cigar_reserve_coop(c, n0 + total)) return true;
	uint32_t *dst = c.a + n0;
	for(uint32_t e = lane; e < total; e += WTZ_NLANES){
		uint32_t lo = 0, hi = np - 1;
		while(lo < hi){ const uint32_t mid = (lo + hi + 1) >> 1; if(LB[mid] <= e) lo = mid; else hi = mid - 1; }
		const uint32_t fl = LF[lo], n = LN[lo], k = e - LB[lo] + (fl & 1u);
		const uint32_t *src = (const uint32_t*)(uintptr_t)LS[lo];
		dst[e] = (fl & 2u) ? src[n - 1 - k] : src[k];
	}
	WTZ_WAVE_SYNC();
	for(uint32_t p = lane; p < np; p += WTZ_NLANES) if(LF[p] & 1u){
		const uint32_t add = LW[p] & 0xFFFFFFF0u;
		uint32_t *w = dst + LB[p]; w--;
#if defined(__HIP_DEVICE_COMPILE__)
		atomicAdd(w, add);
#else
		*w += add;
#endif
	}
	c.n = n0 + total;
	WTZ_WAVE_SYNC();
	return true;
}
WTZ_HD uint32_t wtz_cigar_text_len_coop(const uint32_t *c, uint32_t n){
	uint32_t tot = 0;
	for(uint32_t i0 = 0; i0 < n; i0 += WTZ_NLANES){
		const uint32_t i = i0 + WTZ_LANE;
		uint32_t k = 0;
		if(i < n){ uint32_t len = c[i] >> 4; if(len){ uint32_t d = 1; while(len >= 10){ len /= 10; d++; } k = d + 1; } }
		uint32_t t; (void)wtz_coop_excl_scan(k, &t); tot += t;
	}
	return tot;
}
WTZ_HD void wtz_cigar_text_write_coop(const uint32_t *c, uint32_t n, char *s){
	uint32_t base = 0;
	for(uint32_t i0 = 0; i0 < n; i0 += WTZ_NLANES){
		const uint32_t i = i0 + WTZ_LANE;
		uint32_t k = 0, op = 0, len = 0;
		if(i < n){ op = c[i] & 0xFu; len = c[i] >> 4; if(len){ uint32_t l2 = len, d = 1; while(l2 >= 10){ l2 /= 10; d++; } k = d + 1; } }
		uint32_t t; const uint32_t ex = wtz_coop_excl_scan(k, &t);
		if(k){
			char *o = s + base + ex; uint32_t p = k - 1;
			o[p] = op == 0 ? 'M' : (op == 1 ? 'I' : 'D');
			while(p){ o[--p] = (char)('0' + len % 10); len /= 10; }
		}
		base += t;
	}
}

WTZ_HD wtz_readview wtz_view(const wtz_reads_t &R, uint32_t id, uint32_t rev){ wtz_readview v; v.bits = R.bits; v.off = R.rdoff[id]; v.len = R.rdlen[id]; v.rev = rev; return v; }

template<bool FULL = true>
WTZ_HD void wtz_task_winalign(uint32_t t, const wtz_env_t &V, const wtz_wintask_t *tasks, const wtz_alnitem_t *items, uint32_t *defer = NULL, const uint32_t *list = NULL){
	if(list) t = list[1 + t];
	const wtz_params_t *P = V.P;
	const wtz_alnitem_t &it = items[tasks[t].item];
	const wtz_win_t &w = it.win[tasks[t].widx];
	wtz_reg_t reg; memset(&reg, 0, sizeof reg);
	wtz_cigar_t cigar, tmp;
	cigar.init(V.pool, WTZ_LANE == 0 ? (w.anchors[1] - w.anchors[0]) * 14u + 16u : 0); tmp.init(V.pool, 0);
	unsigned long long cells = 0;
	int32_t bad = 0;
#if defined(__HIP_DEVICE_COMPILE__)
	bool ok = true, dfr = false;
	reg.x = wtz_align_window_wave<FULL>(wtz_view(V.R, it.q, 0), wtz_view(V.R, it.c, it.dir), w, it.anchors, cigar, tmp, P, V.pool, wtz_wave_scratch(), &cells, &ok, &dfr);
	if(!FULL && dfr){ if(WTZ_LANE == 0){ const uint32_t idx = atomicAdd(&defer[0], 1u); defer[1 + idx] = t; } return; }
	if(!ok) bad = 1;
	if(WTZ_LANE != 0) return;
#else
	wtz_swmem_t mem; wtz_swmem_init_lds(mem, V.pool, wtz_wave_scratch(), WTZ_WAVE_LDS_BYTES / 4);
	reg.x = wtz_align_window(wtz_view(V.R, it.q, 0), wtz_view(V.R, it.c, it.dir), w, it.anchors, cigar, mem, tmp, P);
	if(mem.bad) bad = 1;
#endif
	reg.cigar = cigar.a; reg.cigar_len = cigar.n; reg.cells = cells;
	reg.pass = !(reg.x.aln * 2 < (int32_t)P->zovl || (float)reg.x.mat < (float)reg.x.aln * P->min_id);
	if(cigar.bad || tmp.bad || bad) reg.pass = 2;
	it.regs[tasks[t].widx] = reg;
}

#if defined(__HIP_DEVICE_COMPILE__)
#define WTZ_ATOMIC_INC32(p) atomicAdd((p), 1u)
#define WTZ_ATOMIC_ADD64(p, v) atomicAdd((p), (unsigned long long)(v))
#else
#define WTZ_ATOMIC_INC32(p) ((*(p))++)
#define WTZ_ATOMIC_ADD64(p, v) (*(p) += (unsigned long long)(v))
#endif
WTZ_HD void wtz_task_lcount(uint32_t t, const wtz_wintask_t *tasks, const wtz_alnitem_t *items, uint32_t *na){
	const wtz_alnitem_t &it = items[tasks[t].item];
	const wtz_win_t &w = it.win[tasks[t].widx];
	na[t] = w.anchors[1] - w.anchors[0];
}
WTZ_HD void wtz_task_lplan(uint32_t t, const wtz_env_t &V, const wtz_wintask_t *tasks, const wtz_alnitem_t *items, const uint32_t *woff,
		wtz_lprob_t *prob, uint32_t *runcap, uint64_t *key, uint32_t *val, uint8_t *wflag, uint32_t *ccnt, uint32_t *uidx, uint32_t *nu){
	const wtz_params_t *P = V.P;
	const wtz_alnitem_t &it = items[tasks[t].item];
	const wtz_win_t &w = it.win[tasks[t].widx];
	const wtz_readview pb1 = wtz_view(V.R, it.q, 0), pb2 = wtz_view(V.R, it.c, it.dir);
	const uint32_t base = woff[t], na = w.anchors[1] - w.anchors[0];
	const int32_t M = P->M, I = P->O, D = P->O, E = P->E, T = P->T;
	int32_t te = 0, qe = 0; bool first = true, fb = false, ended = false;
	uint32_t cc[4] = {0u, 0u, 0u, 0u}, n_used = 0;
	for(uint32_t k0 = 0; k0 < na; k0 += 4){
		wtz_zhit_t A[4]; wtz_seq_w2 Z1[4], Z2[4];
		#pragma unroll
		for(uint32_t j = 0; j < 4; j++) if(k0 + j < na) A[j] = it.anchors[w.anchors[0] + k0 + j];
		#pragma unroll
		for(uint32_t j = 0; j < 4; j++){
			Z1[j].w0 = Z1[j].w1 = Z2[j].w0 = Z2[j].w1 = 0;
			if(k0 + j < na && !ended && ZH_LEN1(A[j]) <= 64 && ZH_LEN2(A[j]) <= 64){
				Z1[j] = wtz_seq_load_w2(pb1.sub((int32_t)ZH_OFF1(A[j]), 1), ZH_LEN1(A[j])); Z2[j] = wtz_seq_load_w2(pb2.sub((int32_t)ZH_OFF2(A[j]), 1), ZH_LEN2(A[j]));
			}
		}
		#pragma unroll
		for(uint32_t j = 0; j < 4; j++){
			const uint32_t k = k0 + j;
			if(k >= na) break;
			wtz_lprob_t pr; pr.win = t; pr.qoff = pr.toff = 0; pr.qlen = -1; pr.tlen = 0; pr.run_off = 0;
			uint32_t cap = 0; uint64_t ky = 0xFFFFull;
			if(!ended){
				const wtz_zhit_t p = A[j];
				const int32_t off1 = (int32_t)ZH_OFF1(p), off2 = (int32_t)ZH_OFF2(p);
				if(first){ te = off1; qe = off2; first = false; }
				if(off1 >= te && off2 >= qe){
					pr.qoff = qe; pr.toff = te; pr.qlen = off2 - qe; pr.tlen = off1 - te;
					uidx[base + n_used++] = k;
					if(pr.qlen > 0 && pr.tlen > 0){
						int32_t W0 = P->w, W1 = P->w, ql, tl, n_col, ql1, tl1, nc1;
						wtz_ext_geometry(pr.qlen, pr.tlen, 0, W0, M, I, D, E, T, ql, tl, n_col);
						wtz_ext_geometry(pr.qlen, pr.tlen, 1 << 24, W1, M, I, D, E, T, ql1, tl1, nc1);
						if(W0 != W1 || n_col > WTZ_LN_MAXCOLS || ql > WTZ_LN_MAXROWS || ql + tl > WTZ_LN_MAXSPAN) fb = true;
						else { cap = (uint32_t)(ql + tl + 2); ky = 0xFFFFull - (uint64_t)(((uint32_t)n_col << 9) | (uint32_t)ql); cc[wtz_lane_class(n_col)]++; }
					}
					int32_t dte = 0, dqe = 0; bool past = false, ok;
					const uint32_t len1 = ZH_LEN1(p), len2 = ZH_LEN2(p);
					if(len1 <= 64 && len2 <= 64) ok = wtz_zmer_advance_w2(Z1[j], len1, Z2[j], len2, &dte, &dqe, &past); else { ok = false; past = true; }
					if(past) ok = wtz_zmer_advance_slow(pb1.sub(off1, 1), len1, pb2.sub(off2, 1), len2, &dte, &dqe);
					if(!ok) ended = true;
					else { te = off1 + dte; qe = off2 + dqe; }
				}
			}
			prob[base + k] = pr; runcap[base + k] = cap; key[base + k] = ky; val[base + k] = base + k;
		}
	}
	nu[t] = n_used;
	wflag[t] = fb ? 1 : 0;
	if(fb){ for(uint32_t k = 0; k < na; k++){ key[base + k] = 0xFFFFull; runcap[base + k] = 0; } }
#if defined(__HIP_DEVICE_COMPILE__)
	{
		const bool full = __ballot(1) == ~0ull;
		#pragma unroll
		for(int q4 = 0; q4 < 4; q4++){
			uint32_t v = fb ? 0u : cc[q4];
			if(full){
				#pragma unroll
				for(int o = 32; o > 0; o >>= 1) v += (uint32_t)__shfl_xor((int)v, o, 64);
				if((threadIdx.x & 63u) == 0u && v) atomicAdd(&ccnt[q4], v);
			} else if(v) atomicAdd(&ccnt[q4], v);
		}
	}
#else
	if(!fb) for(int q4 = 0; q4 < 4; q4++) ccnt[q4] += cc[q4];
#endif
}

template<int NC>
WTZ_HD void wtz_task_ldp(uint32_t gw, uint32_t wv, const wtz_env_t &V, const wtz_wintask_t *tasks, const wtz_alnitem_t *items, const uint32_t *order, uint32_t lo, uint32_t hi,
		const wtz_lprob_t *prob, wtz_lres_t *res, uint64_t *wtr, uint32_t *wrm){
	const wtz_params_t *P = V.P;
	const uint32_t idx = lo + wv * WTZ_NLANES + WTZ_LANE;
	const bool live = idx < hi;
	const uint32_t slot = live ? order[idx] : 0u;
	wtz_lprob_t pr; pr.win = 0; pr.qoff = pr.toff = 0; pr.qlen = pr.tlen = 0; pr.run_off = 0;
	if(live) pr = prob[slot];
	const int32_t M = P->M, X = P->X, I = P->O, D = P->O, E = P->E, T = P->T;
	int32_t W = P->w, ql = 0, tl = 0, n_col = 0;
	wtz_seq_packed q, tt; q.bits = tt.bits = V.R.bits; q.start = tt.start = 0; q.strand = tt.strand = 1; q.comp = tt.comp = 0;
	if(live){
		wtz_ext_geometry(pr.qlen, pr.tlen, 0, W, M, I, D, E, T, ql, tl, n_col);
		const wtz_alnitem_t &it = items[tasks[pr.win].item];
		q = wtz_view(V.R, it.c, it.dir).sub(pr.qoff, 1); tt = wtz_view(V.R, it.q, 0).sub(pr.toff, 1);
	}
	constexpr uint32_t RS = (uint32_t)wtz_lane_geo<NC>::RS;
	const uint32_t rows_max = (uint32_t)wtz_lane_wmax(ql);
	uint64_t pa = 0;
	if(WTZ_LANE == 0){
		pa = (uint64_t)(uintptr_t)wtz_pool_alloc(V.pool + 1, (size_t)WTZ_NLANES * rows_max * RS * 4 + 16);
		wtr[gw] = pa; wrm[gw] = rows_max;
	}
	pa = wtz_coop_bcast64(pa);
	if(pa == 0) return;
	uint32_t *tr = (uint32_t*)(uintptr_t)pa;
	wtz_lres_t R; memset(&R, 0, sizeof R);
	wtz_lane_fixed<NC, false>(live, pr.qlen, q, pr.tlen, tt, 0, W, ql, tl, M, X, I, D, E, T, tr, R);
	if(live) res[slot] = R;
}
WTZ_HD void wtz_task_ltb(uint32_t gw, uint32_t wv, uint32_t RS, const wtz_env_t &V, const wtz_wintask_t *tasks, const wtz_alnitem_t *items, const uint32_t *order, uint32_t lo, uint32_t hi,
		const wtz_lprob_t *prob, const uint32_t *runoff, uint32_t *runs, wtz_lres_t *res, const uint64_t *wtr, const uint32_t *wrm){
	const wtz_params_t *P = V.P;
	const uint32_t idx = lo + wv * WTZ_NLANES + WTZ_LANE;
	const uint64_t pa = wtr[gw];
	if(idx >= hi || pa == 0) return;
	const uint32_t slot = order[idx];
	const wtz_lprob_t pr = prob[slot];
	wtz_lres_t R = res[slot];
	int32_t W = P->w, ql, tl, n_col;
	wtz_ext_geometry(pr.qlen, pr.tlen, 0, W, P->M, P->O, P->O, P->E, P->T, ql, tl, n_col);
	const wtz_alnitem_t &it = items[tasks[pr.win].item];
	const wtz_seq_packed q = wtz_view(V.R, it.c, it.dir).sub(pr.qoff, 1), tt = wtz_view(V.R, it.q, 0).sub(pr.toff, 1);
	const uint32_t *tr = (const uint32_t*)(uintptr_t)pa;
	wtz_lane_traceback<false>(true, R.qe - 1, R.te - 1, W, RS, q, pr.qlen, tt, pr.tlen, tr, runs + runoff[slot], R);
	res[slot] = R;
}

typedef struct { uint32_t wend[4], lo[4], hi[4]; } wtz_lclass_t;
WTZ_HD void wtz_task_ldp_all(uint32_t wv, const wtz_lclass_t &L, const wtz_env_t &V, const wtz_wintask_t *tasks, const wtz_alnitem_t *items, const uint32_t *order,
		const wtz_lprob_t *prob, wtz_lres_t *res, uint64_t *wtr, uint32_t *wrm){
	uint32_t k = 0; while(k < 3 && wv >= L.wend[k]) k++;
	const uint32_t wl = wv - (k ? L.wend[k - 1] : 0u);
	if(k == 0)      wtz_task_ldp<104>(wv, wl, V, tasks, items, order, L.lo[0], L.hi[0], prob, res, wtr, wrm);
	else if(k == 1) wtz_task_ldp<64>(wv, wl, V, tasks, items, order, L.lo[1], L.hi[1], prob, res, wtr, wrm);
	else if(k == 2) wtz_task_ldp<32>(wv, wl, V, tasks, items, order, L.lo[2], L.hi[2], prob, res, wtr, wrm);
	else            wtz_task_ldp<16>(wv, wl, V, tasks, items, order, L.lo[3], L.hi[3], prob, res, wtr, wrm);
}
WTZ_HD void wtz_task_ltb_all(uint32_t wv, const wtz_lclass_t &L, const wtz_env_t &V, const wtz_wintask_t *tasks, const wtz_alnitem_t *items, const uint32_t *order,
		const wtz_lprob_t *prob, const uint32_t *runoff, uint32_t *runs, wtz_lres_t *res, const uint64_t *wtr, const uint32_t *wrm){
	uint32_t k = 0; while(k < 3 && wv >= L.wend[k]) k++;
	const uint32_t wl = wv - (k ? L.wend[k - 1] : 0u);
	wtz_task_ltb(wv, wl, 16u >> k, V, tasks, items, order, L.lo[k], L.hi[k], prob, runoff, runs, res, wtr, wrm);
}

typedef struct { wtz_cigar_t v; uint32_t tail; } wtz_lcig_t;
WTZ_HD void wtz_lcig_push(wtz_lcig_t &w, uint32_t op, uint32_t len){
	if(len == 0) return;
	if(w.tail && (w.tail & 0xFu) == op) w.tail += len << 4;
	else { if(w.tail) w.v.push(w.tail); w.tail = (len << 4) | op; }
}
template<typename S1, typename S2>
WTZ_HD wtz_aln_t wtz_align_zmer_lane_t(const S1 &pb1, uint32_t len1, const S2 &pb2, uint32_t len2, int32_t M, int32_t I, int32_t D, int32_t E, wtz_lcig_t &cw, bool bounded, bool *past){
	wtz_aln_t x, zero; memset(&zero, 0, sizeof zero); x = zero;
	uint32_t s0 = 0, s1 = 0;
	while(s0 < len1 || s1 < len2){
		if(bounded && (s0 >= len1 || s1 >= len2)){ *past = true; return zero; }
		const uint32_t b = pb1.at((int32_t)s0);
		if(b != pb2.at((int32_t)s1)) return zero;
		uint32_t e0 = s0 + 1; while(e0 < len1 && pb1.at((int32_t)e0) == b) e0++;
		uint32_t e1 = s1 + 1; while(e1 < len2 && pb2.at((int32_t)e1) == b) e1++;
		const uint32_t l0 = e0 - s0, l1 = e1 - s1;
		if(l0 < l1){ x.aln += l1; x.mat += l0; x.ins += l1 - l0; x.score += (int32_t)l0 * M + I + (int32_t)(l1 - l0) * E; wtz_lcig_push(cw, 0, l0); wtz_lcig_push(cw, 1, l1 - l0); }
		else if(l0 == l1){ x.aln += l0; x.mat += l0; x.score += (int32_t)l0 * M; wtz_lcig_push(cw, 0, l0); }
		else { x.aln += l0; x.mat += l1; x.del += l0 - l1; x.score += (int32_t)l1 * M + D + (int32_t)(l0 - l1) * E; wtz_lcig_push(cw, 0, l1); wtz_lcig_push(cw, 2, l0 - l1); }
		s0 = e0; s1 = e1;
	}
	x.te = x.mat + x.del; x.qe = x.mat + x.ins;
	return x;
}
WTZ_HD wtz_aln_t wtz_align_zmer_lane(const wtz_seq_packed &pb1, uint32_t len1, const wtz_seq_packed &pb2, uint32_t len2, int32_t M, int32_t I, int32_t D, int32_t E, wtz_lcig_t &cw){
	bool past = false;
	if(len1 <= 64 && len2 <= 64){
		const wtz_seq_w2 r1 = wtz_seq_load_w2(pb1, len1), r2 = wtz_seq_load_w2(pb2, len2);
		if(len1 == len2 && len1 && r1.w0 == r2.w0 && r1.w1 == r2.w1){
			wtz_aln_t y; memset(&y, 0, sizeof y);
			y.aln = y.mat = (int32_t)len1; y.te = y.qe = (int32_t)len1; y.score = (int32_t)len1 * M;
			wtz_lcig_push(cw, 0, len1);
			return y;
		}
		const uint32_t keep_tail = cw.tail, keep_n = cw.v.n;
		const wtz_aln_t y = wtz_align_zmer_lane_t(r1, len1, r2, len2, M, I, D, E, cw, true, &past);
		if(!past) return y;
		cw.tail = keep_tail; cw.v.n = keep_n;
	}
	return wtz_align_zmer_lane_t(pb1, len1, pb2, len2, M, I, D, E, cw, false, &past);
}

WTZ_HD void wtz_task_lfold(uint32_t t, const wtz_env_t &V, const wtz_wintask_t *tasks, const wtz_alnitem_t *items, const uint32_t *woff,
		const wtz_lprob_t *prob, const uint32_t *runoff, const uint32_t *runs, const wtz_lres_t *res, const uint8_t *wflag, uint32_t *fblist, const uint32_t *uidx, const uint32_t *nu){
	if(wflag[t]){ const uint32_t k = WTZ_ATOMIC_INC32(&fblist[0]); fblist[1 + k] = t; return; }
	const wtz_params_t *P = V.P;
	const wtz_alnitem_t &it = items[tasks[t].item];
	const wtz_win_t &w = it.win[tasks[t].widx];
	const wtz_readview pb1 = wtz_view(V.R, it.q, 0), pb2 = wtz_view(V.R, it.c, it.dir);
	const uint32_t base = woff[t], na = w.anchors[1] - w.anchors[0];
	const int32_t M = P->M, I = P->O, D = P->O, E = P->E;
	wtz_reg_t reg; memset(&reg, 0, sizeof reg);
	wtz_lcig_t cw; cw.v.init(V.pool, na * 14u + 16u); cw.tail = 0;
	wtz_aln_t x; memset(&x, 0, sizeof x);
	unsigned long long cells = 0; int32_t bad = 0;
	bool stop = false;
	const uint32_t n_used = nu[t];
	for(uint32_t u0 = 0; u0 < n_used && !stop; u0 += 2){
		uint32_t KK[2]; wtz_lprob_t PR[2]; wtz_lres_t RES[2]; wtz_zhit_t AN[2]; uint32_t RO[2];
		#pragma unroll
		for(uint32_t j = 0; j < 2; j++) KK[j] = u0 + j < n_used ? uidx[base + u0 + j] : 0u;
		#pragma unroll
		for(uint32_t j = 0; j < 2; j++) if(u0 + j < n_used){ PR[j] = prob[base + KK[j]]; AN[j] = it.anchors[w.anchors[0] + KK[j]]; RES[j] = res[base + KK[j]]; RO[j] = runoff[base + KK[j]]; }
		#pragma unroll
		for(uint32_t j = 0; j < 2; j++){
			if(u0 + j >= n_used || stop) break;
			const wtz_lprob_t pr = PR[j];
			if(pr.qlen < 0) continue;
			const wtz_zhit_t p = AN[j];
			const int32_t off1 = (int32_t)ZH_OFF1(p), off2 = (int32_t)ZH_OFF2(p);
			if(x.aln == 0){ x.tb = x.te = off1; x.qb = x.qe = off2; }
			const int32_t a = x.score < 0 ? 0 : x.score;
			if(pr.qlen > 0 && pr.tlen > 0){
				const wtz_lres_t r = RES[j];
				if(!(r.flags & WTZ_LR_DONE)){ bad = 1; stop = true; break; }
				if(a + r.minrow <= 0 || ((r.flags & WTZ_LR_USEDG) && a + r.score <= 0)){ const uint32_t z = WTZ_ATOMIC_INC32(&fblist[0]); fblist[1 + z] = t; return; }
				x.score = a + r.score;
				x.aln += r.mat + r.mis + r.ins + r.del; x.mat += r.mat; x.mis += r.mis; x.ins += r.ins; x.del += r.del;
				x.te += r.te; x.qe += r.qe;
				const uint32_t *rr = runs + RO[j];
				uint32_t jj = r.n_runs;
				for(; jj >= 4; jj -= 4){
					const uint32_t v0 = rr[jj - 1], v1 = rr[jj - 2], v2 = rr[jj - 3], v3 = rr[jj - 4];
					wtz_lcig_push(cw, v0 & 0xFu, v0 >> 4); wtz_lcig_push(cw, v1 & 0xFu, v1 >> 4); wtz_lcig_push(cw, v2 & 0xFu, v2 >> 4); wtz_lcig_push(cw, v3 & 0xFu, v3 >> 4);
				}
				for(; jj-- > 0;){ const uint32_t v = rr[jj]; wtz_lcig_push(cw, v & 0xFu, v >> 4); }
				cells += r.cells;
			} else x.score = a;
			if(x.te < off1){ x.del += off1 - x.te; x.aln += off1 - x.te; wtz_lcig_push(cw, 2, (uint32_t)(off1 - x.te)); x.te = off1; }
			if(x.qe < off2){ x.ins += off2 - x.qe; x.aln += off2 - x.qe; wtz_lcig_push(cw, 1, (uint32_t)(off2 - x.qe)); x.qe = off2; }
			const uint32_t keep_tail = cw.tail, keep_n = cw.v.n;
			const wtz_aln_t y = wtz_align_zmer_lane(pb1.sub(off1, 1), ZH_LEN1(p), pb2.sub(off2, 1), ZH_LEN2(p), M, I, D, E, cw);
			if(y.aln == 0){ cw.tail = keep_tail; cw.v.n = keep_n; stop = true; break; }
			x.score += y.score;
			x.aln += y.aln; x.mat += y.mat; x.mis += y.mis; x.ins += y.ins; x.del += y.del;
			x.te += y.te; x.qe += y.qe;
		}
	}
	if(cw.tail){ cw.v.push(cw.tail); cw.tail = 0; }
	reg.x = x; reg.cigar = cw.v.a; reg.cigar_len = cw.v.n; reg.cells = cells;
	reg.pass = !(reg.x.aln * 2 < (int32_t)P->zovl || (float)reg.x.mat < (float)reg.x.aln * P->min_id);
	if(cw.v.bad || bad) reg.pass = 2;
	it.regs[tasks[t].widx] = reg;
}

typedef struct { wtz_aln_t x; wtz_cigar_t cigar; uint32_t first, nreg; int32_t bad; unsigned long long cells_global;
	uint32_t mid;
} wtz_stitch_state_t;

typedef struct { int32_t score, aln, mat, mis, ins, del; uint32_t *cigar; uint32_t cigar_len; int32_t bad, valid; unsigned long long cells; } wtz_gapres_t;
WTZ_HD unsigned long long wtz_global_cells(int32_t qlen, int32_t tlen, int32_t w){
	unsigned long long n = 0;
	for(int32_t i = 0; i < tlen; i++){ const int32_t beg = i > w ? i - w : 0; int32_t end = i + w + 1; if(end > qlen) end = qlen; if(end > beg) n += (unsigned long long)(end - beg); }
	return n;
}

#define WTZ_GAP_WIDE_LDS_BYTES (8192 + 2 * 8192 * 4)
typedef struct { int32_t score; bool from_reg, want_defer; int32_t bad; uint32_t *runs; uint32_t n_runs; int32_t r_mat, r_mis; int form; } wtz_gapdp_t;
#define WTZ_FORM_RING 32
#if defined(__HIP_DEVICE_COMPILE__)
template<bool TEST>
WTZ_D void wtz_gap_problem_wave(int32_t dq, const wtz_seq_packed &q, int32_t dt, const wtz_seq_packed &tt, const wtz_params_t *P, int32_t w,
		int32_t *lds, uint32_t wide_lds, bool may_defer, wtz_pool_t *pool, wtz_cigar_t &tmp, wtz_trace_t &tr, wtz_swmem_t &mem, int force, wtz_gapdp_t &R){
	const int32_t M = P->M, X = P->X, I = P->O, D = P->O, E = P->E;
	wtz_wave_lds_t L; L.tb = (uint64_t*)lds; L.Hs = lds + 256; L.Es = lds + 768; L.PM = 511; L.tw = 128;
	wtz_wave_lds_t LW = L;
	if(wide_lds >= WTZ_GAP_WIDE_LDS_BYTES){ LW.Hs = lds + 2048; LW.Es = lds + 2048 + 8192; LW.PM = 8191; LW.tw = 1024; }
	uint8_t *ztr = (uint8_t*)(lds + 256); const int32_t ztr_bytes = WTZ_GAP_LDS_BYTES - 1024;
	R.score = 0; R.from_reg = false; R.want_defer = false; R.bad = 0; R.runs = NULL; R.n_runs = 0; R.r_mat = R.r_mis = 0; R.form = 0;
	int32_t score = 0;
	const int32_t n_col = dq < 2 * w + 1 ? dq : 2 * w + 1;
	const int32_t zrow = (n_col + 3) & ~3, run_bytes = 4 * (dq + dt + 4);
	const unsigned long long pt_g = WTZ_PROF_T(); (void)pt_g;
	const int32_t qwords = (dq + 63) / 32 + 1, qbytes = (qwords * 8 + 15) & ~15;
	bool lds_shape = (dq > 0 && dt > 0 && n_col <= 128 && dt <= 2048 && qwords <= 128 && ((dt + 1) / 2) * zrow + run_bytes <= ztr_bytes);
	bool reg_shape = lds_shape || (dq > 0 && dt > 0 && n_col <= 512 && qbytes + 4096 <= WTZ_GAP_LDS_BYTES);
	int32_t cmin = n_col <= 64 ? 1 : (n_col <= 128 ? 2 : (n_col <= 256 ? 4 : 8));
	bool ring_ok = true, scalar_only = false;
	if constexpr(TEST){
		if(force == 255){ lds_shape = reg_shape = false; ring_ok = false; scalar_only = true; may_defer = false; }
		else if(force == WTZ_FORM_RING){ lds_shape = reg_shape = false; may_defer = false; }
		else if(force){
			const int32_t fc = force & 15; const bool zg = (force & 16) != 0;
			const bool can = (fc == 1 || fc == 2 || fc == 4 || fc == 8) && fc >= cmin && n_col <= 64 * fc && (zg ? (dq > 0 && dt > 0 && qbytes + 4096 <= WTZ_GAP_LDS_BYTES) : (lds_shape && fc <= 2));
			if(!can){ R.form = -1; return; }
			lds_shape = !zg; reg_shape = true; cmin = fc;
		}
	}
	if(reg_shape && !lds_shape){
		uint8_t *stg = (uint8_t*)lds + qbytes;
		const bool runs_lds = (qbytes + 4096 + run_bytes <= WTZ_GAP_LDS_BYTES);
		unsigned long long za = 0, ra = 0;
		if(WTZ_LANE == 0){
			za = (unsigned long long)(uintptr_t)wtz_pool_alloc(pool, (size_t)((dt + 1) / 2) * zrow);
			if(!runs_lds) ra = (unsigned long long)(uintptr_t)wtz_pool_alloc(pool, (size_t)run_bytes);
		}
		za = __shfl(za, 0, 64); ra = __shfl(ra, 0, 64);
		if(za == 0 || (!runs_lds && ra == 0)){ R.bad = 1; score = 0; }
		else {
			R.runs = runs_lds ? (uint32_t*)(stg + 4096) : (uint32_t*)(uintptr_t)ra; R.from_reg = true; R.form = cmin | 16;
			uint8_t *zg = (uint8_t*)(uintptr_t)za;
			if(cmin == 1)      score = wtz_global_reg<1, true>(dq, q, dt, tt, M, X, -I, -E, -D, -E, w, L.tb, zg, (uint32_t)zrow, R.runs, &R.n_runs, &R.r_mat, &R.r_mis, stg);
			else if(cmin == 2) score = wtz_global_reg<2, true>(dq, q, dt, tt, M, X, -I, -E, -D, -E, w, L.tb, zg, (uint32_t)zrow, R.runs, &R.n_runs, &R.r_mat, &R.r_mis, stg);
			else if(cmin == 4) score = wtz_global_reg<4, true>(dq, q, dt, tt, M, X, -I, -E, -D, -E, w, L.tb, zg, (uint32_t)zrow, R.runs, &R.n_runs, &R.r_mat, &R.r_mis, stg);
			else               score = wtz_global_reg<8, true>(dq, q, dt, tt, M, X, -I, -E, -D, -E, w, L.tb, zg, (uint32_t)zrow, R.runs, &R.n_runs, &R.r_mat, &R.r_mis, stg);
		}
		WTZ_PROF_ADD(43, pt_g); WTZ_PROF_CNT(44, 1000000); WTZ_PROF_MAX(45, pt_g);
	} else if(lds_shape){
		R.runs = (uint32_t*)(ztr + ztr_bytes - run_bytes); R.from_reg = true; R.form = cmin;
		if(cmin == 1) score = wtz_global_reg<1>(dq, q, dt, tt, M, X, -I, -E, -D, -E, w, L.tb, ztr, (uint32_t)zrow, R.runs, &R.n_runs, &R.r_mat, &R.r_mis);
		else          score = wtz_global_reg<2>(dq, q, dt, tt, M, X, -I, -E, -D, -E, w, L.tb, ztr, (uint32_t)zrow, R.runs, &R.n_runs, &R.r_mat, &R.r_mis);
		WTZ_PROF_ADD(32, pt_g); WTZ_PROF_CNT(33, 1000000); WTZ_PROF_MAX(34, pt_g);
	} else if(may_defer && dq > 0 && dt > 0 && !(n_col + 2 <= 512 && qwords <= 128) && n_col + 2 <= 8192 && qwords <= 1024 && (dt + 63) / 64 <= WTZ_TRACE_MAXCHUNK){
		R.want_defer = true;
		return;
	} else if(ring_ok && dq > 0 && dt > 0 && n_col + 2 <= LW.PM + 1 && qwords <= LW.tw && (dt + 63) / 64 <= WTZ_TRACE_MAXCHUNK){
		bool ok = true;
		R.form = WTZ_FORM_RING;
		score = wtz_global_wave(dq, q, dt, tt, M, X, -I, -E, -D, -E, w, LW, tr, pool, tmp, &ok);
		if(!ok) R.bad = 1;
#ifdef WTZ_GAP_CHECK
		if(ok && WTZ_LANE == 0){
			wtz_cigar_t t2; t2.init(pool, 32); wtz_swmem_t m2; wtz_swmem_init(m2, pool);
			const int32_t s2 = wtz_global_banded(dq, q, dt, tt, M, X, -I, -E, -D, -E, w, m2, t2);
			uint32_t firstdiff = 0xFFFFFFFFu;
			if(!m2.bad){ if(t2.n != tmp.n) firstdiff = 0xFFFFFFFEu; else for(uint32_t z9 = 0; z9 < t2.n; z9++) if(t2.a[z9] != tmp.a[z9]){ firstdiff = z9; break; } }
			if(!m2.bad && (s2 != score || firstdiff != 0xFFFFFFFFu)) printf("[gap-check] dq %d dt %d w %d n_col %d: score wave %d scalar %d; cigar n %u / %u first diff %u\n", dq, dt, w, n_col, score, s2, tmp.n, t2.n, firstdiff);
		}
#endif
		WTZ_PROF_ADD(35, pt_g); WTZ_PROF_CNT(36, 1000000); WTZ_PROF_MAX(37, pt_g);
		WTZ_PROF_CNT(46, (unsigned long long)dt * 1000); if(n_col > 256) WTZ_PROF_CNT(47, 1000000);
	} else {
		if constexpr(TEST){ if(force == WTZ_FORM_RING){ R.form = -1; return; } }
		(void)scalar_only;
		score = 0; R.form = 255;
		if(WTZ_LANE == 0){ score = wtz_global_banded(dq, q, dt, tt, M, X, -I, -E, -D, -E, w, mem, tmp); if(mem.bad) R.bad = 1; }
		WTZ_PROF_ADD(38, pt_g); WTZ_PROF_CNT(39, 1000000); WTZ_PROF_MAX(40, pt_g);
	}
	R.score = __shfl(score, 0, 64);
	R.bad = __shfl(R.bad, 0, 64) ? 1 : 0;
}
#endif

WTZ_HD void wtz_task_gap(uint32_t t, const wtz_env_t &V, const wtz_wintask_t *tasks, const wtz_alnitem_t *items, wtz_gapres_t *gaps,
		uint32_t *defer = NULL, const uint32_t *list = NULL, uint32_t wide_lds = 0){
	if(list) t = list[1 + t];
	const wtz_params_t *P = V.P;
	const wtz_alnitem_t &it = items[tasks[t].item];
	const uint32_t k = tasks[t].widx;
	wtz_gapres_t g; memset(&g, 0, sizeof g);
	const unsigned long long pt_task = WTZ_PROF_T(); (void)pt_task;
	wtz_gapres_t *slot = gaps + (it.regs - items[0].regs) + k;
	if(k == 0 || it.regs[k].pass != 1){ if(WTZ_LANE == 0) *slot = g; return; }
	int32_t prev = -1;
	for(int32_t j = (int32_t)k - 1; j >= 0; j--) if(it.regs[j].pass == 1){ prev = j; break; }
	if(prev < 0){ if(WTZ_LANE == 0) *slot = g; return; }
	const int32_t M = P->M, X = P->X, I = P->O, D = P->O, E = P->E;
	const wtz_reg_t *reg1 = &it.regs[prev], *reg2 = &it.regs[k];
	const wtz_readview pb1 = wtz_view(V.R, it.q, 0), pb2 = wtz_view(V.R, it.c, it.dir);
	const int32_t dq = reg2->x.qb - reg1->x.qe, dt = reg2->x.tb - reg1->x.te;
	const wtz_seq_packed q = pb2.sub(reg1->x.qe, 1), tt = pb1.sub(reg1->x.te, 1);
	wtz_cigar_t tmp; tmp.init(V.pool, WTZ_LANE == 0 ? 32 : 0);
	int32_t w = P->w, score, bad = 0;
#if defined(__HIP_DEVICE_COMPILE__)
	bool from_reg = false; uint32_t n_runs = 0; uint32_t *runs = NULL; int32_t r_mat = 0, r_mis = 0;
	{
		(void)M; (void)X; (void)I; (void)D; (void)E;
		int32_t *lds = wtz_wave_scratch();
		wtz_trace_t tr; tr.chunk = NULL; tr.zb = NULL; tr.n_chunk = 0; tr.zrow = 0; tr.cap_rows = 0;
		wtz_swmem_t mem; wtz_swmem_init(mem, V.pool);
		for(;;){
			if(w < WTZ_ABSDIFF(dq, dt)){ w <<= 1; continue; }
			wtz_gapdp_t G;
			wtz_gap_problem_wave<false>(dq, q, dt, tt, P, w, lds, wide_lds, defer != NULL, V.pool, tmp, tr, mem, 0, G);
			if(G.want_defer){
				if(WTZ_LANE == 0){ const uint32_t idx = atomicAdd(&defer[0], 1u); defer[1 + idx] = t; }
				return;
			}
			score = G.score; from_reg = G.from_reg; runs = G.runs; n_runs = G.n_runs; r_mat = G.r_mat; r_mis = G.r_mis;
			if(WTZ_LANE == 0) g.cells += wtz_global_cells(dq, dt, w);
			if(G.bad){ bad = 1; break; }
			if(score < 0 && w < P->W && w < WTZ_MAX(dq, dt)) w <<= 1;
			else break;
		}
	}
	if(WTZ_LANE != 0) return;
	if(from_reg){
		g.score = score; g.valid = 1; g.mat = r_mat; g.mis = r_mis;
		tmp.n = 0;
		for(uint32_t k = n_runs; k-- > 0;){
			const uint32_t r = runs[k], op = r & 0xFu; const int32_t len = (int32_t)(r >> 4);
			tmp.push(r);
			g.aln += len;
			if(op == 1) g.ins += len; else if(op == 2) g.del += len;
		}
		g.cigar = tmp.a; g.cigar_len = tmp.n; g.bad = (tmp.bad || bad);
		*slot = g;
		WTZ_PROF_ADD(41, pt_task); WTZ_PROF_MAX(42, pt_task);
		return;
	}
#else
	{
		wtz_swmem_t mem; wtz_swmem_init_lds(mem, V.pool, wtz_wave_scratch(), WTZ_WAVE_LDS_BYTES / 4);
		for(;;){
			if(w < WTZ_ABSDIFF(dq, dt)){ w <<= 1; continue; }
			score = wtz_global_banded(dq, q, dt, tt, M, X, -I, -E, -D, -E, w, mem, tmp);
			g.cells += wtz_global_cells(dq, dt, w);
			if(score < 0 && w < P->W && w < WTZ_MAX(dq, dt)) w <<= 1;
			else break;
		}
		if(mem.bad) bad = 1;
	}
#endif
	g.score = score; g.valid = 1;
	int32_t x1 = 0, x2 = 0;
	for(uint32_t idx = 0; idx < tmp.n; idx++){
		int32_t op = (int32_t)(tmp.a[idx] & 0xF), len = (int32_t)(tmp.a[idx] >> 4);
		g.aln += len;
		if(op == 0){ for(int32_t j = 0; j < len; j++){ if(q.at(x1 + j) == tt.at(x2 + j)) g.mat++; else g.mis++; } x1 += len; x2 += len; }
		else if(op == 1){ x1 += len; g.ins += len; }
		else if(op == 2){ x2 += len; g.del += len; }
	}
	g.cigar = tmp.a; g.cigar_len = tmp.n; g.bad = (tmp.bad || bad);
	*slot = g;
}

#define WTZ_LG_MAXROWS 768
typedef struct { uint32_t slot; int32_t dq, dt, w; } wtz_lgap_t;
WTZ_HD void wtz_task_gplan(uint32_t t, const wtz_env_t &V, const wtz_wintask_t *tasks, const wtz_alnitem_t *items, wtz_gapres_t *gaps,
		wtz_lgap_t *gp, uint32_t *runcap, uint64_t *key, uint32_t *val, uint8_t *done, uint32_t *ccnt){
	const wtz_params_t *P = V.P;
	const wtz_alnitem_t &it = items[tasks[t].item];
	const uint32_t k = tasks[t].widx;
	wtz_lgap_t G; G.slot = t; G.dq = G.dt = 0; G.w = 0;
	uint32_t cap = 0; uint64_t ky = 0x3FFFFull; uint8_t dn = 0; int32_t cls = -1;
	wtz_gapres_t *slot = gaps + (it.regs - items[0].regs) + k;
	int32_t prev = -1;
	if(k && it.regs[k].pass == 1) for(int32_t j = (int32_t)k - 1; j >= 0; j--) if(it.regs[j].pass == 1){ prev = j; break; }
	if(prev < 0){ wtz_gapres_t g; memset(&g, 0, sizeof g); *slot = g; dn = 1; }
	else {
		const wtz_reg_t *reg1 = &it.regs[prev], *reg2 = &it.regs[k];
		const int32_t dq = reg2->x.qb - reg1->x.qe, dt = reg2->x.tb - reg1->x.te;
		if(dq > 0 && dt > 0){
			int32_t w = P->w; while(w < WTZ_ABSDIFF(dq, dt)) w <<= 1;
			const int32_t n_col = dq < 2 * w + 1 ? dq : 2 * w + 1;
			G.dq = dq; G.dt = dt; G.w = w;
			if(n_col <= WTZ_LN_MAXCOLS && dt <= WTZ_LG_MAXROWS){
				cap = (uint32_t)(dq + dt + 2);
				ky = 0x3FFFFull - (uint64_t)(((uint32_t)n_col << 11) | (uint32_t)dt);
				cls = (int32_t)wtz_lane_class(n_col);
			}
		}
	}
#if defined(__HIP_DEVICE_COMPILE__)
	#pragma unroll
	for(int32_t c4 = 0; c4 < 4; c4++){
		const unsigned long long m = __ballot(cls == c4);
		if(m && (threadIdx.x & 63u) == (uint32_t)__builtin_ctzll(m)) atomicAdd(&ccnt[c4], (uint32_t)__popcll(m));
	}
#else
	if(cls >= 0) WTZ_ATOMIC_INC32(&ccnt[cls]);
#endif
	gp[t] = G; runcap[t] = cap; key[t] = ky; val[t] = t; done[t] = dn;
}
template<int NC>
WTZ_HD void wtz_task_gdp(uint32_t gw, uint32_t wv, const wtz_env_t &V, const wtz_wintask_t *tasks, const wtz_alnitem_t *items, const uint32_t *order, uint32_t lo, uint32_t hi,
		const wtz_lgap_t *gp, wtz_lres_t *res, uint64_t *wtr, uint32_t *wrm){
	const wtz_params_t *P = V.P;
	const uint32_t idx = lo + wv * WTZ_NLANES + WTZ_LANE;
	const bool live = idx < hi;
	const uint32_t t = live ? order[idx] : 0u;
	wtz_lgap_t G; G.slot = 0; G.dq = G.dt = 0; G.w = P->w;
	if(live) G = gp[t];
	const int32_t M = P->M, X = P->X, I = P->O, D = P->O, E = P->E;
	wtz_seq_packed q, tt; q.bits = tt.bits = V.R.bits; q.start = tt.start = 0; q.strand = tt.strand = 1; q.comp = tt.comp = 0;
	if(live){
		const wtz_alnitem_t &it = items[tasks[t].item];
		const uint32_t k = tasks[t].widx;
		int32_t prev = -1;
		for(int32_t j = (int32_t)k - 1; j >= 0; j--) if(it.regs[j].pass == 1){ prev = j; break; }
		const wtz_reg_t *reg1 = &it.regs[prev];
		q = wtz_view(V.R, it.c, it.dir).sub(reg1->x.qe, 1); tt = wtz_view(V.R, it.q, 0).sub(reg1->x.te, 1);
	}
	constexpr uint32_t RS = (uint32_t)wtz_lane_geo<NC>::RS;
	const uint32_t rows_max = (uint32_t)wtz_lane_wmax(G.dt);
	uint64_t pa = 0;
	if(WTZ_LANE == 0){
		pa = (uint64_t)(uintptr_t)wtz_pool_alloc(V.pool + 1, (size_t)WTZ_NLANES * rows_max * RS * 4 + 16);
		wtr[gw] = pa; wrm[gw] = rows_max;
	}
	pa = wtz_coop_bcast64(pa);
	if(pa == 0) return;
	uint32_t *tr = (uint32_t*)(uintptr_t)pa;
	wtz_lres_t R; memset(&R, 0, sizeof R);
	wtz_lane_global<NC>(live, G.dq, q, G.dt, tt, G.w, M, X, -I, -E, -D, -E, tr, R);
	if(live) res[t] = R;
}
WTZ_HD void wtz_task_gtb(uint32_t gw, uint32_t wv, uint32_t RS, const wtz_env_t &V, const wtz_wintask_t *tasks, const wtz_alnitem_t *items, const uint32_t *order, uint32_t lo, uint32_t hi,
		const wtz_lgap_t *gp, const uint32_t *runoff, uint32_t *runs, const wtz_lres_t *res, wtz_gapres_t *gaps, uint8_t *done, const uint64_t *wtr, const uint32_t *wrm){
	const wtz_params_t *P = V.P;
	const uint32_t idx = lo + wv * WTZ_NLANES + WTZ_LANE;
	const uint64_t pa = wtr[gw];
	if(idx >= hi || pa == 0) return;
	const uint32_t t = order[idx];
	const wtz_lgap_t G = gp[t];
	wtz_lres_t R = res[t];
	if(!(R.flags & WTZ_LR_DONE)) return;
	if(R.score < 0 && G.w < (int32_t)P->W && G.w < WTZ_MAX(G.dq, G.dt)) return;
	const wtz_alnitem_t &it = items[tasks[t].item];
	const uint32_t k = tasks[t].widx;
	int32_t prev = -1;
	for(int32_t j = (int32_t)k - 1; j >= 0; j--) if(it.regs[j].pass == 1){ prev = j; break; }
	const wtz_reg_t *reg1 = &it.regs[prev];
	const wtz_seq_packed q = wtz_view(V.R, it.c, it.dir).sub(reg1->x.qe, 1), tt = wtz_view(V.R, it.q, 0).sub(reg1->x.te, 1);
	const uint32_t *tr = (const uint32_t*)(uintptr_t)pa;
	uint32_t *rr = runs + runoff[t];
	const int32_t r0 = G.dt - 1, c0 = (r0 + G.w + 1 < G.dq ? r0 + G.w + 1 : G.dq) - 1;
	wtz_lane_traceback<true>(true, r0, c0, G.w, RS, tt, G.dt, q, G.dq, tr, rr, R);
	wtz_gapres_t g; memset(&g, 0, sizeof g);
	g.score = R.score; g.valid = 1; g.mat = R.mat; g.mis = R.mis; g.ins = R.ins; g.del = R.del; g.aln = R.mat + R.mis + R.ins + R.del;
	for(uint32_t a = 0, b = R.n_runs; a + 1 < b; a++, b--){ const uint32_t x = rr[a]; rr[a] = rr[b - 1]; rr[b - 1] = x; }
	g.cigar = rr; g.cigar_len = R.n_runs; g.cells = R.cells;
	gaps[(it.regs - items[0].regs) + k] = g; done[t] = 1;
}
WTZ_HD void wtz_task_gdp_all(uint32_t wv, const wtz_lclass_t &L, const wtz_env_t &V, const wtz_wintask_t *tasks, const wtz_alnitem_t *items, const uint32_t *order,
		const wtz_lgap_t *gp, wtz_lres_t *res, uint64_t *wtr, uint32_t *wrm){
	uint32_t k = 0; while(k < 3 && wv >= L.wend[k]) k++;
	const uint32_t wl = wv - (k ? L.wend[k - 1] : 0u);
	if(k == 0)      wtz_task_gdp<104>(wv, wl, V, tasks, items, order, L.lo[0], L.hi[0], gp, res, wtr, wrm);
	else if(k == 1) wtz_task_gdp<64>(wv, wl, V, tasks, items, order, L.lo[1], L.hi[1], gp, res, wtr, wrm);
	else if(k == 2) wtz_task_gdp<32>(wv, wl, V, tasks, items, order, L.lo[2], L.hi[2], gp, res, wtr, wrm);
	else            wtz_task_gdp<16>(wv, wl, V, tasks, items, order, L.lo[3], L.hi[3], gp, res, wtr, wrm);
}
WTZ_HD void wtz_task_gtb_all(uint32_t wv, const wtz_lclass_t &L, const wtz_env_t &V, const wtz_wintask_t *tasks, const wtz_alnitem_t *items, const uint32_t *order,
		const wtz_lgap_t *gp, const uint32_t *runoff, uint32_t *runs, const wtz_lres_t *res, wtz_gapres_t *gaps, uint8_t *done, const uint64_t *wtr, const uint32_t *wrm){
	uint32_t k = 0; while(k < 3 && wv >= L.wend[k]) k++;
	const uint32_t wl = wv - (k ? L.wend[k - 1] : 0u);
	wtz_task_gtb(wv, wl, 16u >> k, V, tasks, items, order, L.lo[k], L.hi[k], gp, runoff, runs, res, gaps, done, wtr, wrm);
}
WTZ_HD void wtz_task_glist(uint32_t t, const uint8_t *done, uint32_t *list){ if(!done[t]){ const uint32_t k = WTZ_ATOMIC_INC32(&list[0]); list[1 + k] = t; } }

WTZ_HD void wtz_task_stitch_left(uint32_t t, const wtz_env_t &V, const wtz_alnitem_t *items, wtz_stitch_state_t *sts, wtz_extjob_t *jobs, int32_t *rgeo = NULL){
	const wtz_params_t *P = V.P;
	const wtz_alnitem_t &it = items[t];
	wtz_stitch_state_t st; memset(&st, 0, sizeof st);
	wtz_extjob_t jb; memset(&jb, 0, sizeof jb); jb.item = t;
	st.first = 0xFFFFFFFFu;
	for(uint32_t k = 0; k < it.nwin; k++){ if(it.regs[k].pass == 2) st.bad = 1; if(it.regs[k].pass == 1){ if(st.first == 0xFFFFFFFFu) st.first = k; st.nreg++; } }
	if(st.nreg && !st.bad){
		st.cigar.init(V.pool, 256);
		st.x = it.regs[st.first].x;
		if(st.x.qb && st.x.tb){
			const wtz_readview pb1 = wtz_view(V.R, it.q, 0), pb2 = wtz_view(V.R, it.c, it.dir);
			jb.valid = 1; jb.qlen = st.x.qb; jb.tlen = st.x.tb; jb.q = pb2.sub(st.x.qb - 1, -1); jb.t = pb1.sub(st.x.tb - 1, -1);
			jb.init_score = st.x.score + 100 * P->M; jb.W = -P->ew;
		}
	}
	if(rgeo){
		int32_t rq = -1, rt = -1;
		if(st.nreg && !st.bad){
			int32_t qe = st.x.qe, te = st.x.te;
			for(uint32_t k = st.first + 1; k < it.nwin; k++) if(it.regs[k].pass == 1){ qe = it.regs[k].x.qe; te = it.regs[k].x.te; }
			const int32_t len1 = (int32_t)V.R.rdlen[it.q], len2 = (int32_t)V.R.rdlen[it.c];
			if(te < len1 && qe < len2){ rq = len2 - qe; rt = len1 - te; }
		}
		rgeo[2 * (size_t)t] = rq; rgeo[2 * (size_t)t + 1] = rt;
	}
	sts[t] = st; jobs[t] = jb;
}

WTZ_HD void wtz_task_stitch_mid(uint32_t t, const wtz_env_t &V, const wtz_alnitem_t *items, wtz_stitch_state_t *sts, const wtz_extjob_t *jobsL, wtz_extjob_t *jobsR, const wtz_gapres_t *gaps, bool fused = false){
	const wtz_params_t *P = V.P;
	const wtz_alnitem_t &it = items[t];
	const int32_t M = P->M;
	const bool l0 = (WTZ_LANE == 0);
	wtz_stitch_state_t st = sts[t];
	if(st.mid) return;
	wtz_extjob_t jr; memset(&jr, 0, sizeof jr); jr.item = t;
	if(st.nreg == 0 || st.bad){ if(l0){ jobsR[t] = jr; if(fused) sts[t].mid = 1; } return; }
	const wtz_readview pb1 = wtz_view(V.R, it.q, 0), pb2 = wtz_view(V.R, it.c, it.dir);
	const int32_t len1 = (int32_t)pb1.len, len2 = (int32_t)pb2.len;
	const wtz_gapres_t *gp = gaps + (it.regs - items[0].regs);
	wtz_aln_t x = st.x;
	if(jobsL[t].valid){
		const wtz_extjob_t &jl = jobsL[t];
		if(jl.bad) st.bad = 1;
		const wtz_aln_t y = jl.x;
		x.score = y.score - 100 * M;
		x.aln += y.aln; x.mat += y.mat; x.mis += y.mis; x.ins += y.ins; x.del += y.del;
		x.qb -= y.qe; x.tb -= y.te;
	}
	const uint32_t first = st.first, nwr = it.nwin - first - 1;
	const wtz_reg_t *regs = it.regs;
	const uint32_t *lc = jobsL[t].valid ? jobsL[t].cigar : NULL; const uint32_t ln = jobsL[t].valid ? jobsL[t].cigar_len : 0u;
#if defined(__HIP_DEVICE_COMPILE__)
	uint32_t *jlds = (uint32_t*)wtz_wave_scratch(); const uint32_t jwords = WTZ_WAVE_LDS_BYTES / 4;
#else
	std::vector<uint64_t> jbuf(3 * (size_t)(2u + 2u * nwr) + 1); uint32_t *jlds = (uint32_t*)jbuf.data(); const uint32_t jwords = (uint32_t)(jbuf.size() * 2);
#endif
#ifdef WTZ_NO_CIGAR_JOIN
	const bool joined = false; (void)jlds; (void)jwords; (void)lc;
#else
	const bool joined = wtz_cigar_join_coop(st.cigar, 2u + 2u * nwr, [=](uint32_t p, const uint32_t **src, uint32_t *n, uint32_t *rev){
		*rev = 0;
		if(p == 0){ *src = lc; *n = ln; *rev = 1; return; }
		if(p == 1){ *src = regs[first].cigar; *n = regs[first].cigar_len; return; }
		const uint32_t k = first + 1 + ((p - 2) >> 1);
		if(regs[k].pass != 1){ *src = NULL; *n = 0; return; }
		if(p & 1u){ *src = regs[k].cigar; *n = regs[k].cigar_len; } else { *src = gp[k].cigar; *n = gp[k].cigar_len; }
	}, jlds, jwords);
#endif
	if(!joined){
		if(ln){ wtz_cigar_reverse_coop(jobsL[t].cigar, ln); wtz_cigar_concat_coop(st.cigar, jobsL[t].cigar, ln); }
		wtz_cigar_concat_coop(st.cigar, regs[first].cigar, regs[first].cigar_len);
	}
	for(uint32_t k = first + 1; k < it.nwin; k++){
		if(regs[k].pass != 1) continue;
		const wtz_reg_t *reg2 = &regs[k];
		const wtz_gapres_t &g = gp[k];
		if(!g.valid || g.bad) st.bad = 1;
		st.cells_global += g.cells;
		x.score += g.score;
		x.aln += g.aln; x.mat += g.mat; x.mis += g.mis; x.ins += g.ins; x.del += g.del;
		if(!joined) wtz_cigar_concat_coop(st.cigar, g.cigar, g.cigar_len);
		x.score += reg2->x.score;
		x.aln += reg2->x.aln; x.mat += reg2->x.mat; x.mis += reg2->x.mis; x.ins += reg2->x.ins; x.del += reg2->x.del;
		x.qe = reg2->x.qe; x.te = reg2->x.te;
		if(!joined) wtz_cigar_concat_coop(st.cigar, reg2->cigar, reg2->cigar_len);
	}
	if(st.cigar.bad) st.bad = 1;
	if(x.te < len1 && x.qe < len2){
		jr.valid = 1; jr.qlen = len2 - x.qe; jr.tlen = len1 - x.te; jr.q = pb2.sub(x.qe, 1); jr.t = pb1.sub(x.te, 1);
		jr.init_score = x.score; jr.W = -P->ew;
	}
	if(l0){ st.x = x; st.mid = fused ? 1u : 0u; sts[t] = st; jobsR[t] = jr; }
}

WTZ_HD void wtz_task_stitch_fin(uint32_t t, const wtz_env_t &V, const wtz_alnitem_t *items, wtz_stitch_state_t *sts, const wtz_extjob_t *jobsL, const wtz_extjob_t *jobsR, wtz_alnres_dev_t *out){
	wtz_stitch_state_t st = sts[t];
	wtz_alnres_dev_t r; memset(&r, 0, sizeof r);
	r.n_regs = st.nreg; r.bad = st.bad; r.cells_global = st.cells_global;
	for(uint32_t k = 0; k < items[t].nwin; k++) r.cells_fixed += items[t].regs[k].cells;
	if(st.nreg && !st.bad){
		wtz_aln_t x = st.x;
		if(jobsR[t].valid){
			const wtz_extjob_t &jr = jobsR[t];
			if(jr.bad) r.bad = 1;
			const wtz_aln_t y = jr.x;
			x.score = y.score;
			x.aln += y.aln; x.mat += y.mat; x.mis += y.mis; x.ins += y.ins; x.del += y.del;
			x.qe += y.qe; x.te += y.te;
			wtz_cigar_concat_coop(st.cigar, jr.cigar, jr.cigar_len);
			r.cells_shift += jr.cells;
		}
		if(jobsL[t].valid) r.cells_shift += jobsL[t].cells;
		if(st.cigar.bad) r.bad = 1;
		r.x = x; r.cigar = st.cigar.a; r.cigar_len = st.cigar.n; r.text_len = wtz_cigar_text_len_coop(st.cigar.a, st.cigar.n);
	}
	if(WTZ_LANE == 0) out[t] = r;
}

#define WTZ_REFINE_LDS_BYTES (2048 * 4 * 2 + 1032 * 8)
#if !defined(__HIP_DEVICE_COMPILE__)
static inline bool wtz_refine_scalar(const wtz_seq_packed &query, int32_t qb, const wtz_seq_packed &target, int32_t tb, int32_t W, int32_t M, int32_t X, int32_t I, int32_t D, int32_t E,
		const uint32_t *cig, uint32_t ncig, wtz_pool_t *pool, wtz_cigar_t &out, wtz_aln_t *res){
	wtz_aln_t y; memset(&y, 0, sizeof y);
	out.n = 0;
	int32_t qe = qb, te = tb;
	for(uint32_t i = 0; i < ncig; i++){ const uint32_t op = cig[i] & 0xFu; const int32_t len = (int32_t)(cig[i] >> 4); if(op == 0){ qe += len; te += len; } else if(op == 1) qe += len; else te += len; }
	const int32_t ql = qe - qb, tl = te - tb;
	if(ql == 0 || tl == 0){ *res = y; return true; }
	int32_t *zw = (int32_t*)wtz_pool_alloc(pool, (size_t)(ql + 2) * (4 * 3 + 8) + (size_t)(tl + 2) * 8);
	if(zw == NULL) return false;
	unsigned long long *zoff = (unsigned long long*)zw; zw = (int32_t*)(zoff + (ql + 2));
	int32_t *zb = zw + (ql + 2), *ze = zb + (ql + 2);
	int32_t *rh = ze + (ql + 2), *re = rh + (tl + 2);
	for(int32_t i = 0; i < ql + 2; i++) zw[i] = 0;
	int32_t qx = 0, tx = 0;
	for(uint32_t i = 0; i < ncig; i++){
		const uint32_t op = cig[i] & 0xFu; const int32_t len = (int32_t)(cig[i] >> 4);
		if(op == 0){ for(int32_t j = 0; j < len; j++) zw[qx++] = W; } else if(op == 1){ for(int32_t j = 0; j < len; j++) zw[qx++] = W + len; }
	}
	qx = 0;
	for(uint32_t i = 0; i < ncig; i++){
		const uint32_t op = cig[i] & 0xFu; const int32_t len = (int32_t)(cig[i] >> 4);
		if(op == 0) qx += len;
		else if(op == 1){ for(int32_t j = 1; j < len && j < qx; j++) zw[qx - j] += len - j; qx += len - 1; for(int32_t j = 1; j < len && j + qx < ql; j++) zw[qx + j] += len - j; qx++; }
		else { for(int32_t j = 1; j < len && j < qx; j++) zw[qx - j] += len - j; for(int32_t j = 1; j < len && j + qx < ql; j++) zw[qx + j] += len - j; }
	}
	qx = 0;
	for(uint32_t i = 0; i < ncig; i++){
		const uint32_t op = cig[i] & 0xFu; const int32_t len = (int32_t)(cig[i] >> 4);
		if(op == 0 || op == 1){ for(int32_t j = 0; j < len; j++){ int32_t b = tx - zw[qx]; if(b < 0) b = 0; int32_t e = tx + 1 + zw[qx]; if(e > tl) e = tl; zb[qx] = b; ze[qx] = e; if(op == 0) tx++; qx++; } }
		else tx += len;
	}
	{ int32_t b = 0; for(int32_t i = 0; i < ql; i++){ if(zb[i] < b) zb[i] = b; else if(zb[i] > b) b = zb[i]; } }
	{ int32_t e = tl; for(int32_t i = ql - 1; i >= 0; i--){ if(ze[i] > e) ze[i] = e; else if(ze[i] < e) e = ze[i]; } }
	unsigned long long ztot = 0;
	for(int32_t i = 0; i < ql; i++){ zoff[i] = ztot; ztot += (unsigned long long)(ze[i] > zb[i] ? ze[i] - zb[i] : 0); }
	uint8_t *z = (uint8_t*)wtz_pool_alloc(pool, (size_t)ztot + 64);
	if(z == NULL) return false;
	rh[0] = 0; for(int32_t j = 1; j <= tl; j++) rh[j] = -10000;
	for(int32_t j = 0; j <= tl; j++) re[j] = -10000;
	for(int32_t i = 0; i < ql; i++){
		const uint32_t qc = query.at(i);
		int32_t h1 = -10000, f = -10000, j;
		uint8_t *zi = z + zoff[i];
		for(j = zb[i]; j < ze[i]; j++){
			const bool eq = (qc == target.at(j));
			int32_t m = rh[j] + (eq ? M : X), e, h, t; uint32_t d;
			rh[j] = h1;
			e = re[j];
			if(m >= e){ d = 0; h = m; } else { d = 1; h = e; }
			if(h < f){ d = 2; h = f; }
			h1 = h;
			t = m + I + E; e = e + E; if(e > t) d |= 1u << 2; else e = t;
			re[j] = e;
			t = m + D + E; f = f + E; if(f > t) d |= 2u << 4; else f = t;
			if(eq) d |= 0x80u;
			zi[j - zb[i]] = (uint8_t)d;
		}
		rh[j] = h1; re[j] = -10000;
	}
	y.qb = qb; y.qe = qe; y.tb = tb; y.te = te; y.score = rh[tl];
	int32_t i_ = ql - 1, j_ = tl - 1; uint32_t d_ = 0;
	while(i_ >= 0 && j_ >= 0){
		const uint32_t zv = (j_ >= zb[i_] && j_ < ze[i_]) ? z[zoff[i_] + (unsigned long long)(j_ - zb[i_])] : 0u;
		d_ = (zv >> (d_ << 1)) & 0x03;
		if(d_ == 0){ if(zv & 0x80u) y.mat++; else y.mis++; i_--; j_--; }
		else if(d_ == 1){ i_--; y.ins++; }
		else { j_--; y.del++; }
		wtz_cigar_push(out, d_, 1);
	}
	if(i_ >= 0){ y.ins += i_ + 1; wtz_cigar_push(out, 1, (uint32_t)(i_ + 1)); }
	if(j_ >= 0){ y.del += j_ + 1; wtz_cigar_push(out, 2, (uint32_t)(j_ + 1)); }
	wtz_cigar_reverse(out.a, out.n);
	y.aln = y.mat + y.mis + y.ins + y.del;
	*res = y;
	return true;
}
#endif

WTZ_HD void wtz_task_refine(uint32_t t, const wtz_env_t &V, const wtz_alnitem_t *items, wtz_alnres_dev_t *res){
	const wtz_params_t *P = V.P;
	wtz_alnres_dev_t r = res[t];
	if(r.n_regs == 0 || r.bad) return;
	const wtz_alnitem_t &it = items[t];
	if(P->aux_strand){
		const int32_t tl = (int32_t)V.R.rdlen[it.q], ql = (int32_t)V.R.rdlen[it.c];
		int32_t beg = r.x.qb - r.x.tb; if(beg < 0) beg = 0;
		int32_t end = r.x.qe + tl - r.x.te; if(end > ql) end = ql;
		const int32_t ovl = end - beg;
		if(r.x.score < 0 || (float)r.x.mat < (float)r.x.aln * P->min_id || (float)r.x.mat < (float)ovl * P->min_id){
			if(WTZ_LANE == 0){ r.n_regs = 0; res[t] = r; }
			return;
		}
	}
	const wtz_readview pb1 = wtz_view(V.R, it.q, 0), pb2 = wtz_view(V.R, it.c, it.dir);
	wtz_cigar_t out; out.a = NULL; out.n = out.cap = 0; out.pool = V.pool; out.bad = 0;
	if(WTZ_LANE == 0) out.init(V.pool, r.cigar_len + 64);
	wtz_aln_t y; memset(&y, 0, sizeof y);
	bool ok;
#if defined(__HIP_DEVICE_COMPILE__)
	int32_t *lds = wtz_wave_scratch();
	wtz_wave_lds_t L; L.Hs = lds; L.Es = lds + 2048; L.tb = (uint64_t*)(lds + 4096); L.PM = 2047; L.tw = 1032;
	ok = wtz_refine_wave(pb2.sub(r.x.qb, 1), r.x.qb, pb1.sub(r.x.tb, 1), r.x.tb, P->w, P->M, P->X, P->O, P->O, P->E, r.cigar, r.cigar_len, L, V.pool, out, &y);
	if(WTZ_LANE != 0) return;
#else
	ok = wtz_refine_scalar(pb2.sub(r.x.qb, 1), r.x.qb, pb1.sub(r.x.tb, 1), r.x.tb, P->w, P->M, P->X, P->O, P->O, P->E, r.cigar, r.cigar_len, V.pool, out, &y);
#endif
	if(!ok || out.bad){ r.bad = 1; res[t] = r; return; }
	r.x = y; r.cigar = out.a; r.cigar_len = out.n; r.text_len = wtz_cigar_text_len(out.a, out.n);
	res[t] = r;
}

WTZ_HD void wtz_task_extjob_scalar(uint32_t t, const wtz_env_t &V, wtz_extjob_t *jobs){
	const wtz_params_t *P = V.P;
	wtz_extjob_t &jb = jobs[t];
	if(!jb.valid) return;
	wtz_swmem_t mem; wtz_swmem_init(mem, V.pool);
	wtz_cigar_t cg; cg.init(V.pool, 64);
	unsigned long long cells = 0;
	jb.x = wtz_extend_shift(jb.qlen, jb.q, jb.tlen, jb.t, jb.init_score, jb.W, P->M, P->X, P->O, P->O, P->E, P->T, mem, cg, &cells);
	jb.cigar = cg.a; jb.cigar_len = cg.n; jb.bad = (mem.bad || cg.bad); jb.cells = cells;
}

#endif
```

### smartdenovo_amd/csrc/wtz_testdp.h

```cpp
#ifndef WTZ_TESTDP_H
#define WTZ_TESTDP_H

struct K_test_fixed;
struct K_test_global;
struct K_test_global_wide;
struct K_test_lane;

typedef struct { wtz_seq_packed q, t; int32_t qlen, tlen, init_score, W; } wtz_dpprob_dev_t;
typedef struct { wtz_aln_t x; uint32_t *cigar; uint32_t cigar_len; int32_t form, bad; unsigned long long cells; } wtz_dpres_dev_t;

#ifndef WTZ_EMUL
static __device__ void wtz_testdp_store(wtz_dpres_dev_t *res, const wtz_aln_t &x, bool from_runs, const uint32_t *runs, uint32_t n_runs, const wtz_cigar_t &tmp,
		wtz_pool_t *pool, int form, int bad, unsigned long long cells){
	wtz_dpres_dev_t r; memset(&r, 0, sizeof r);
	r.x = x; r.form = form; r.bad = bad; r.cells = cells;
	if(from_runs){
		wtz_cigar_t cg; cg.init(pool, n_runs ? n_runs : 1);
		for(uint32_t k = n_runs; k-- > 0;) cg.push(runs[k]);
		r.cigar = cg.a; r.cigar_len = cg.n; if(cg.bad) r.bad = 1;
	} else { r.cigar = tmp.a; r.cigar_len = tmp.n; if(tmp.bad) r.bad = 1; }
	*res = r;
}

static __device__ void wtz_task_test_fixed(uint32_t t, const wtz_dpprob_dev_t *pr, const wtz_params_t *P, wtz_pool_t *pool, int force, wtz_dpres_dev_t *res){
	const wtz_dpprob_dev_t p = pr[t];
	int32_t *lds = wtz_wave_scratch();
	wtz_wave_lds_t L; L.tb = (uint64_t*)lds; L.Hs = lds + 256; L.Es = lds + 768; L.PM = 511; L.tw = 128; L.qw = (uint32_t*)(lds + WTZ_WINALIGN_LDS_BYTES / 4);
	uint8_t *ztr = (uint8_t*)(lds + 256); const int32_t ztr_bytes = WTZ_WINALIGN_LDS_BYTES - 1024;
	wtz_swmem_t mem; wtz_swmem_init(mem, pool);
	wtz_cigar_t tmp; tmp.init(pool, WTZ_LANE == 0 ? 64 : 0);
	unsigned long long cells = 0;
	wtz_fixres_t R;
	wtz_fixed_problem_wave<true, true>(p.qlen, p.q, p.tlen, p.t, p.init_score, P, L, ztr, ztr_bytes, tmp, mem, pool, &cells, force, R);
	if(WTZ_LANE != 0) return;
	if(R.form < 0){ wtz_dpres_dev_t r; memset(&r, 0, sizeof r); r.form = 0; res[t] = r; return; }
	wtz_testdp_store(&res[t], R.y, R.lds_runs, R.runs, R.n_runs, tmp, pool, R.form ? R.form : (force ? force : 1), !R.ok, cells);
}

static __device__ void wtz_task_test_lane(uint32_t t, const wtz_dpprob_dev_t *pr, const wtz_params_t *P, wtz_pool_t *pool, wtz_dpres_dev_t *res){
	const wtz_dpprob_dev_t p = pr[t];
	const int32_t M = P->M, X = P->X, I = P->O, D = P->O, E = P->E, T = P->T;
	const int32_t init = p.init_score < 0 ? 0 : p.init_score;
	wtz_dpres_dev_t r; memset(&r, 0, sizeof r);
	if(p.qlen <= 0 || p.tlen <= 0){ r.x.score = init; r.form = 64; if(WTZ_LANE == 0) res[t] = r; return; }
	int32_t W = P->w, ql, tl, n_col;
	wtz_ext_geometry(p.qlen, p.tlen, init, W, M, I, D, E, T, ql, tl, n_col);
	if(n_col > WTZ_LN_MAXCOLS || ql > WTZ_LN_MAXROWS || ql + tl > WTZ_LN_MAXSPAN || init > (1 << 20)){ if(WTZ_LANE == 0) res[t] = r; return; }
	const uint32_t RS = wtz_lane_rs(n_col);
	unsigned long long pa = 0;
	if(WTZ_LANE == 0) pa = (unsigned long long)(uintptr_t)wtz_pool_alloc(pool, (size_t)ql * RS * 4 * WTZ_NLANES + (size_t)(ql + tl + 4) * 4 + 32);
	pa = __shfl(pa, 0, 64);
	if(pa == 0){ r.bad = 1; r.form = 64; if(WTZ_LANE == 0) res[t] = r; return; }
	uint32_t *tr = (uint32_t*)(uintptr_t)pa, *runs = tr + (size_t)ql * RS * WTZ_NLANES + 4;
	const bool live = WTZ_LANE == 0;
	wtz_lres_t R; memset(&R, 0, sizeof R);
	if(n_col <= 16)      wtz_lane_fixed<16, true>(live, p.qlen, p.q, p.tlen, p.t, init, W, ql, tl, M, X, I, D, E, T, tr, R);
	else if(n_col <= 32) wtz_lane_fixed<32, true>(live, p.qlen, p.q, p.tlen, p.t, init, W, ql, tl, M, X, I, D, E, T, tr, R);
	else if(n_col <= 64) wtz_lane_fixed<64, true>(live, p.qlen, p.q, p.tlen, p.t, init, W, ql, tl, M, X, I, D, E, T, tr, R);
	else                 wtz_lane_fixed<104, true>(live, p.qlen, p.q, p.tlen, p.t, init, W, ql, tl, M, X, I, D, E, T, tr, R);
	if(!live) return;
	wtz_lane_traceback<false>(true, R.qe - 1, R.te - 1, W, RS, p.q, p.qlen, p.t, p.tlen, tr, runs, R);
	wtz_aln_t x; memset(&x, 0, sizeof x);
	x.score = R.score; x.qe = R.qe; x.te = R.te; x.mat = R.mat; x.mis = R.mis; x.ins = R.ins; x.del = R.del; x.aln = R.mat + R.mis + R.ins + R.del;
	wtz_cigar_t none; none.a = NULL; none.n = none.cap = 0; none.pool = pool; none.bad = 0;
	wtz_testdp_store(&res[t], x, true, runs, R.n_runs, none, pool, 64, 0, R.cells);
}

static __device__ void wtz_task_test_lane_global(uint32_t t, const wtz_dpprob_dev_t *pr, const wtz_params_t *P, wtz_pool_t *pool, wtz_dpres_dev_t *res){
	const wtz_dpprob_dev_t p = pr[t];
	const int32_t M = P->M, X = P->X, I = P->O, D = P->O, E = P->E;
	wtz_dpres_dev_t r; memset(&r, 0, sizeof r);
	const int32_t w = p.W, n_col = p.qlen < 2 * w + 1 ? p.qlen : 2 * w + 1;
	if(p.qlen <= 0 || p.tlen <= 0 || WTZ_ABSDIFF(p.qlen, p.tlen) > w || n_col > WTZ_LN_MAXCOLS || p.tlen > WTZ_LG_MAXROWS){ if(WTZ_LANE == 0) res[t] = r; return; }
	const uint32_t RS = wtz_lane_rs(n_col);
	unsigned long long pa = 0;
	if(WTZ_LANE == 0) pa = (unsigned long long)(uintptr_t)wtz_pool_alloc(pool, (size_t)p.tlen * RS * 4 * WTZ_NLANES + (size_t)(p.qlen + p.tlen + 4) * 4 + 32);
	pa = __shfl(pa, 0, 64);
	if(pa == 0){ r.bad = 1; r.form = 64; if(WTZ_LANE == 0) res[t] = r; return; }
	uint32_t *tr = (uint32_t*)(uintptr_t)pa, *runs = tr + (size_t)p.tlen * RS * WTZ_NLANES + 4;
	const bool live = WTZ_LANE == 0;
	wtz_lres_t R; memset(&R, 0, sizeof R);
	if(n_col <= 16)      wtz_lane_global<16>(live, p.qlen, p.q, p.tlen, p.t, w, M, X, -I, -E, -D, -E, tr, R);
	else if(n_col <= 32) wtz_lane_global<32>(live, p.qlen, p.q, p.tlen, p.t, w, M, X, -I, -E, -D, -E, tr, R);
	else if(n_col <= 64) wtz_lane_global<64>(live, p.qlen, p.q, p.tlen, p.t, w, M, X, -I, -E, -D, -E, tr, R);
	else                 wtz_lane_global<104>(live, p.qlen, p.q, p.tlen, p.t, w, M, X, -I, -E, -D, -E, tr, R);
	if(!live) return;
	{ const int32_t r0 = p.tlen - 1, c0 = (r0 + w + 1 < p.qlen ? r0 + w + 1 : p.qlen) - 1; wtz_lane_traceback<true>(true, r0, c0, w, RS, p.t, p.tlen, p.q, p.qlen, tr, runs, R); }
	wtz_aln_t x; memset(&x, 0, sizeof x);
	x.score = R.score; x.mat = R.mat; x.mis = R.mis; x.ins = R.ins; x.del = R.del; x.aln = R.mat + R.mis + R.ins + R.del;
	wtz_cigar_t none; none.a = NULL; none.n = none.cap = 0; none.pool = pool; none.bad = 0;
	wtz_testdp_store(&res[t], x, true, runs, R.n_runs, none, pool, 64, 0, R.cells);
}

static __device__ void wtz_task_test_global(uint32_t t, const wtz_dpprob_dev_t *pr, const wtz_params_t *P, wtz_pool_t *pool, int force, uint32_t wide_lds, wtz_dpres_dev_t *res){
#if defined(__HIP_DEVICE_COMPILE__)
	const wtz_dpprob_dev_t p = pr[t];
	int32_t *lds = wtz_wave_scratch();
	wtz_trace_t tr; tr.chunk = NULL; tr.zb = NULL; tr.n_chunk = 0; tr.zrow = 0; tr.cap_rows = 0;
	wtz_swmem_t mem; wtz_swmem_init(mem, pool);
	wtz_cigar_t tmp; tmp.init(pool, WTZ_LANE == 0 ? 32 : 0);
	wtz_gapdp_t G;
	wtz_gap_problem_wave<true>(p.qlen, p.q, p.tlen, p.t, P, p.W, lds, wide_lds, false, pool, tmp, tr, mem, force == 33 ? WTZ_FORM_RING : force, G);
	if(WTZ_LANE != 0) return;
	if(G.form < 0){ wtz_dpres_dev_t r; memset(&r, 0, sizeof r); r.form = 0; res[t] = r; return; }
	wtz_aln_t x; memset(&x, 0, sizeof x); x.score = G.score;
	if(G.from_reg){
		x.mat = G.r_mat; x.mis = G.r_mis;
		for(uint32_t k = 0; k < G.n_runs; k++){ const uint32_t r = G.runs[k], op = r & 0xFu; const int32_t len = (int32_t)(r >> 4); x.aln += len; if(op == 1) x.ins += len; else if(op == 2) x.del += len; }
	} else {
		int32_t x1 = 0, x2 = 0;
		for(uint32_t idx = 0; idx < tmp.n; idx++){
			const int32_t op = (int32_t)(tmp.a[idx] & 0xF), len = (int32_t)(tmp.a[idx] >> 4);
			x.aln += len;
			if(op == 0){ for(int32_t j = 0; j < len; j++){ if(p.q.at(x1 + j) == p.t.at(x2 + j)) x.mat++; else x.mis++; } x1 += len; x2 += len; }
			else if(op == 1){ x1 += len; x.ins += len; }
			else if(op == 2){ x2 += len; x.del += len; }
		}
	}
	wtz_testdp_store(&res[t], x, G.from_reg, G.runs, G.n_runs, tmp, pool, (G.form == WTZ_FORM_RING && force == 33) ? 33 : G.form, G.bad, 0);
#endif
}
#endif

extern "C" int wtz_test_dp(wtz_ctx_t *c, int32_t kind, int32_t form, const wtz_dp_problem_t *pr, uint32_t n, wtz_dp_result_t *out, uint32_t *cigar, uint64_t cigar_cap){
	BATCH_ARGS(c, n, pr && out && (cigar || !cigar_cap), NULL, NULL);
#ifdef WTZ_EMUL
	(void)kind; (void)form;
	return wtz_fail(WTZ_E_STATE, "wtz_test_dp drives the DEVICE forms of the banded DPs: it needs the HIP build");
#else
	CTX_ENTER(c);
	std::vector<uint64_t> h_off; CHK(batch_begin(c, h_off));
	std::vector<wtz_dpprob_dev_t> hp(n);
	for(uint32_t i = 0; i < n; i++){
		const wtz_dp_problem_t &p = pr[i];
		wtz_dpprob_dev_t d; CHK(dp_problem_views(c, h_off, p, i, true, 0, &d.q, &d.t)); d.qlen = p.q_len; d.tlen = p.t_len; d.init_score = p.init_score; d.W = p.W;
		hp[i] = d;
	}
	const wtz_env_t V = ctx_env(c);
	std::vector<wtz_dpres_dev_t> hr(n);
	if(kind == WTZ_DP_SHIFT){
		std::vector<wtz_extjob_t> jobs(n);
		for(uint32_t i = 0; i < n; i++){ wtz_extjob_t j; memset(&j, 0, sizeof j); j.q = hp[i].q; j.t = hp[i].t; j.qlen = hp[i].qlen; j.tlen = hp[i].tlen; j.init_score = hp[i].init_score; j.W = hp[i].W; j.item = i; j.valid = 1; jobs[i] = j; }
		wtz_extjob_t *d_jobs = NULL; CHK(dev_alloc((void**)&d_jobs, (size_t)n * sizeof(wtz_extjob_t))); CHK(dev_h2d(d_jobs, jobs.data(), (size_t)n * sizeof(wtz_extjob_t)));
		wtz_timer tform; tform.start();
		if(form == 0){ CHK(run_extjobs(c, V, d_jobs, n)); }
		else if(form == 3){ WTZ_LAUNCH((wtz_kernel_extjobs<2048, 1032>), n, 64, 0, g_stream, d_jobs, (const uint32_t*)NULL, n, V.P, V.pool, V.pool + 1); }
		else if(form == 4){ CHK(wtz_launch_wave<K_extjob_scalar>(n, [=] WTZ_LAMBDA (uint64_t t){ wtz_task_extjob_scalar((uint32_t)t, V, d_jobs); })); }
		else if(form == 5){ WTZ_LAUNCH((wtz_kernel_extjobs_fr<1032>), n, 64, 0, g_stream, d_jobs, (const uint32_t*)NULL, n, V.P, V.pool, V.pool + 1); }
		else if(form == 7){ WTZ_LAUNCH((wtz_kernel_extjobs_pk<1032>), n, 64, 0, g_stream, d_jobs, (const uint32_t*)NULL, n, V.P, V.pool, V.pool + 1); }
		else return wtz_fail(WTZ_E_ARG, "WTZ_DP_SHIFT: unknown form %d", form);
		CHK(dev_sync());
		if(form != 0){ c->cnt.ms_ext += tform.stop(); c->cnt.n_extjobs += n; }
		CHK(tpool_check(c, "wtz_test_dp"));
		CHK(dev_d2h(jobs.data(), d_jobs, (size_t)n * sizeof(wtz_extjob_t)));
		for(uint32_t i = 0; i < n; i++){
			wtz_dpres_dev_t r; memset(&r, 0, sizeof r);
			const int done = form == 4 ? 4 : (int)jobs[i].done;
			const bool empty = jobs[i].qlen <= 0 || jobs[i].tlen <= 0;
			if(done || (form == 0) || (form == 3 && empty)){ r.x = jobs[i].x; r.cigar = jobs[i].cigar; r.cigar_len = jobs[i].cigar_len; r.form = done ? done : 3; r.bad = jobs[i].bad; r.cells = jobs[i].cells; }
			hr[i] = r;
		}
	} else if(kind == WTZ_DP_FIXED || kind == WTZ_DP_GLOBAL){
		wtz_dpprob_dev_t *d_pr = NULL; wtz_dpres_dev_t *d_res = NULL;
		CHK(batch_upload(hp, std::vector<uint32_t>(), &d_pr, (uint32_t**)NULL, &d_res));
		const wtz_params_t *dP = c->dP; wtz_pool_t *pool = c->dpool;
		if(kind == WTZ_DP_FIXED && form == 64){
			CHK(wtz_launch_coop<K_test_lane>(n, [=] WTZ_LAMBDA (uint64_t t){ wtz_task_test_lane((uint32_t)t, d_pr, dP, pool, d_res); }, 0));
		} else if(kind == WTZ_DP_FIXED){
			CHK(wtz_launch_coop<K_test_fixed>(n, [=] WTZ_LAMBDA (uint64_t t){ wtz_task_test_fixed((uint32_t)t, d_pr, dP, pool, form, d_res); }, WTZ_WINALIGN_LDS_BYTES + WTZ_WINALIGN_QW_BYTES));
		} else if(form == 64){
			CHK(wtz_launch_coop<K_test_lane>(n, [=] WTZ_LAMBDA (uint64_t t){ wtz_task_test_lane_global((uint32_t)t, d_pr, dP, pool, d_res); }, 0));
		} else if(form == 33){
			CHK(wtz_launch_coop<K_test_global_wide>(n, [=] WTZ_LAMBDA (uint64_t t){ wtz_task_test_global((uint32_t)t, d_pr, dP, pool, form, (uint32_t)WTZ_GAP_WIDE_LDS_BYTES, d_res); }, WTZ_GAP_WIDE_LDS_BYTES));
		} else {
			CHK(wtz_launch_coop<K_test_global>(n, [=] WTZ_LAMBDA (uint64_t t){ wtz_task_test_global((uint32_t)t, d_pr, dP, pool, form, 0u, d_res); }, WTZ_GAP_LDS_BYTES));
		}
		CHK(dev_sync());
		CHK(dev_d2h(hr.data(), d_res, (size_t)n * sizeof(wtz_dpres_dev_t)));
	} else return wtz_fail(WTZ_E_ARG, "unknown DP kind %d", kind);
	CHK(pool_check(c, "wtz_test_dp"));
	uint64_t off = 0;
	for(uint32_t i = 0; i < n; i++){
		const wtz_dpres_dev_t &r = hr[i];
		if(r.bad) return wtz_fail(WTZ_E_POOL, "wtz_test_dp: problem %u ran out of scratch", i);
		wtz_dp_result_t o; memset(&o, 0, sizeof o);
		o.form_used = (uint32_t)r.form;
		if(r.form){
			o.score = r.x.score; o.tb = r.x.tb; o.te = r.x.te; o.qb = r.x.qb; o.qe = r.x.qe; o.aln = r.x.aln; o.mat = r.x.mat; o.mis = r.x.mis; o.ins = r.x.ins; o.del = r.x.del;
			o.cigar_len = r.cigar_len; o.cigar_off = off; o.cells = r.cells;
			if(off + r.cigar_len > cigar_cap) return wtz_fail(WTZ_E_ARG, "wtz_test_dp: CIGAR buffer too small");
			if(r.cigar_len) CHK(dev_d2h(cigar + off, r.cigar, (size_t)r.cigar_len * 4));
			off += r.cigar_len;
		}
		out[i] = o;
	}
	return WTZ_OK;
#endif
}
#endif
```

Before: 10.69.

## Retry band-doubled gaps in extra lane rounds before falling to wavefront kernel

```diff
diff --git a/smartdenovo_amd/csrc/wtz_ctx.h b/smartdenovo_amd/csrc/wtz_ctx.h
--- a/smartdenovo_amd/csrc/wtz_ctx.h
+++ b/smartdenovo_amd/csrc/wtz_ctx.h
@@ -5,6 +5,7 @@
 	int ext_pk = 1;
 	int heavy_first = -1;
 	int gap_lane = 1;
+	int gap_round_min = 8192;
 	int lane = 1;
 	bool trace = false;
 	bool fail_once = false;
@@ -22,6 +23,7 @@
 	s->ext_pk = env_int("WTZ_EXT_PK", s->ext_pk);
 	s->heavy_first = env_int("WTZ_PAIR_HEAVY_FIRST", s->heavy_first);
 	s->gap_lane = env_int("WTZ_GAP_LANE", s->gap_lane);
+	s->gap_round_min = env_int("WTZ_GAP_ROUND_MIN", s->gap_round_min);
 	s->lane = env_int("WTZ_WINALIGN_LANE", s->lane);
 	s->trace = getenv("WTZ_STAGE_TRACE") != NULL;
 	s->fail_once = getenv("WTZ_POOL_FAIL_ONCE") != NULL;
diff --git a/smartdenovo_amd/csrc/wtz_lib_align.h b/smartdenovo_amd/csrc/wtz_lib_align.h
--- a/smartdenovo_amd/csrc/wtz_lib_align.h
+++ b/smartdenovo_amd/csrc/wtz_lib_align.h
@@ -226,7 +226,7 @@
 	wtz_pool_t *pool = c->dpool + which;
 	CHK(wtz_launch<K_poolalloc>(1, [=] WTZ_LAMBDA (uint64_t){ *d_p = (unsigned long long)(uintptr_t)wtz_pool_alloc(pool, bytes); }));
 	unsigned long long h = 0; CHK(dev_d2h(&h, d_p, 8));
-	if(h == 0) return wtz_fail(WTZ_E_POOL, "device scratch pool exhausted (%zu bytes for the K-sw1 problem lists)", bytes);
+	if(h == 0){ c->last_pool_fail = which ? 2 : 1; return wtz_fail(WTZ_E_POOL, "device scratch pool exhausted (%zu bytes for a host-planned array of the %s pool)", bytes, which ? "transient" : "main"); }
 	*out = (void*)(uintptr_t)h; return WTZ_OK;
 }
 static uint32_t lane_classes(const uint32_t ccnt[4], wtz_lclass_t *L){
@@ -300,8 +300,8 @@
 	return WTZ_OK;
 }
 
-static int run_gap_lane(wtz_ctx *c, const wtz_env_t &V, const wtz_wintask_t *d_wt, uint64_t nwt, const wtz_alnitem_t *d_items, wtz_gapres_t *d_gaps, uint32_t *d_list, uint32_t *n_list){
-	*n_list = 0;
+static int run_gap_lane(wtz_ctx *c, const wtz_env_t &V, const wtz_wintask_t *d_wt, uint64_t nwt, const wtz_alnitem_t *d_items, wtz_gapres_t *d_gaps, uint32_t *d_list, uint32_t *n_list, wtz_lgap_t **gp_out){
+	*n_list = 0; *gp_out = NULL;
 	if(nwt == 0) return WTZ_OK;
 	wtz_lgap_t *d_gp = NULL; uint32_t *d_cap = NULL, *d_roff = NULL, *d_val = NULL, *d_ccnt = NULL; uint64_t *d_key = NULL; uint8_t *d_done = NULL;
 	{
@@ -309,38 +309,50 @@
 		uint8_t *blk = NULL; CHK(pool_alloc_host(c, 0, carve_bytes(nsp, sizeof(wtz_lgap_t)) + 3 * carve_bytes(nsp, 4) + carve_bytes(nsp, 8) + carve_bytes(nsp, 1), (void**)&blk));
 		carve(blk, d_gp, nsp); carve(blk, d_cap, nsp); carve(blk, d_roff, nsp); carve(blk, d_val, nsp); carve(blk, d_key, nsp); carve(blk, d_done, nsp);
 	}
-	CHK(dev_alloc((void**)&d_ccnt, 32)); CHK(dev_set(d_ccnt, 0, 32));
+	*gp_out = d_gp;
+	CHK(dev_alloc((void**)&d_ccnt, 64)); CHK(dev_set(d_ccnt, 0, 64));
 	CHK(dev_set(d_cap, 0, ((size_t)nwt + 1) * 4));
 	CHK(wtz_launch<K_gplan>(nwt, [=] WTZ_LAMBDA (uint64_t t){ wtz_task_gplan((uint32_t)t, V, d_wt, d_items, d_gaps, d_gp, d_cap, d_key, d_val, d_done, d_ccnt); }));
 	CHK(dev_exclusive_scan_u32(d_cap, d_roff, nwt + 1));
 	uint32_t NR = 0, ccnt[4] = {0, 0, 0, 0};
 	CHK(dev_d2h(&NR, d_roff + nwt, 4)); CHK(dev_d2h(ccnt, d_ccnt, 16));
 	uint32_t *d_runs = NULL; CHK(pool_alloc_host(c, 0, ((size_t)NR + 16) * 4, (void**)&d_runs));
-	CHK(dev_sort_pairs_u64_u32(d_key, d_val, nwt, 18));
+	wtz_lres_t *d_res = NULL;
+	CHK(pool_alloc_host(c, 0, ((size_t)nwt + 1) * sizeof(wtz_lres_t), (void**)&d_res)); CHK(dev_set(d_res, 0, ((size_t)nwt + 1) * sizeof(wtz_lres_t)));
 	CHK(dev_set(d_list, 0, 4));
-	{
-		const uint32_t *d_ord = d_val; const wtz_lgap_t *gp = d_gp; const uint32_t *ro = d_roff; uint32_t *rn = d_runs; uint8_t *dn = d_done;
-		wtz_lclass_t L; const uint32_t wv = lane_classes(ccnt, &L);
-		uint64_t *d_wtr = NULL; uint32_t *d_wrm = NULL; wtz_lres_t *d_res = NULL;
+	uint32_t per_round[8] = {0, 0, 0, 0, 0, 0, 0, 0}, n_rounds = 0;
+	uint64_t *d_kcur = d_key, *d_knxt = NULL; uint32_t *d_vcur = d_val, *d_vnxt = NULL;
+	for(uint32_t round = 0;; round++){
+		wtz_lclass_t L; const uint32_t wv = lane_classes(ccnt, &L), n_r = L.hi[3];
+		if(wv == 0 || (round && n_r < (uint32_t)c->sw.gap_round_min)) break;
+		if(n_rounds < 8) per_round[n_rounds] = n_r;
+		n_rounds++;
+		if(round == 0){ CHK(dev_alloc((void**)&d_knxt, ((size_t)n_r + 1) * 8)); CHK(dev_alloc((void**)&d_vnxt, ((size_t)n_r + 1) * 4)); }
+		CHK(dev_sort_pairs_u64_u32(d_kcur, d_vcur, round ? n_r : nwt, 18));
+		uint32_t *cn = d_ccnt + 8 * ((round + 1) & 1u);
+		CHK(dev_set(cn, 0, 32));
+		const uint32_t *d_ord = d_vcur; wtz_lgap_t *gp = d_gp; const uint32_t *ro = d_roff; uint32_t *rn = d_runs; uint8_t *dn = d_done; uint64_t *nk = d_knxt; uint32_t *nv = d_vnxt;
+		uint64_t *d_wtr = NULL; uint32_t *d_wrm = NULL;
 		CHK(dev_alloc((void**)&d_wtr, ((size_t)wv + 1) * 8)); CHK(dev_alloc((void**)&d_wrm, ((size_t)wv + 1) * 4)); CHK(dev_set(d_wtr, 0, ((size_t)wv + 1) * 8));
-		CHK(pool_alloc_host(c, 0, ((size_t)nwt + 1) * sizeof(wtz_lres_t), (void**)&d_res)); CHK(dev_set(d_res, 0, ((size_t)nwt + 1) * sizeof(wtz_lres_t)));
-		if(wv) CHK(wtz_launch_coop<K_gdp>(wv, [=] WTZ_LAMBDA (uint64_t t){ wtz_task_gdp_all((uint32_t)t, L, V, d_wt, d_items, d_ord, gp, d_res, d_wtr, d_wrm); }, 0));
-		if(wv) CHK(wtz_launch_coop<K_gtb>(wv, [=] WTZ_LAMBDA (uint64_t t){ wtz_task_gtb_all((uint32_t)t, L, V, d_wt, d_items, d_ord, gp, ro, rn, d_res, d_gaps, dn, d_wtr, d_wrm); }, 0));
-		CHK(wtz_launch<K_glist>(nwt, [=] WTZ_LAMBDA (uint64_t t){ wtz_task_glist((uint32_t)t, dn, d_list); }));
-	}
+		CHK(wtz_launch_coop<K_gdp>(wv, [=] WTZ_LAMBDA (uint64_t t){ wtz_task_gdp_all((uint32_t)t, L, V, d_wt, d_items, d_ord, gp, d_res, d_wtr, d_wrm); }, 0));
+		CHK(wtz_launch_coop<K_gtb>(wv, [=] WTZ_LAMBDA (uint64_t t){ wtz_task_gtb_all((uint32_t)t, L, V, d_wt, d_items, d_ord, gp, ro, rn, d_res, d_gaps, dn, d_wtr, d_wrm, nk, nv, cn); }, 0));
+		CHK(dev_d2h(ccnt, cn, 16));
+		{ uint64_t *k2 = d_kcur; d_kcur = d_knxt; d_knxt = k2; uint32_t *v2 = d_vcur; d_vcur = d_vnxt; d_vnxt = v2; }
+	}
+	{ const uint8_t *dn = d_done; CHK(wtz_launch<K_glist>(nwt, [=] WTZ_LAMBDA (uint64_t t){ wtz_task_glist((uint32_t)t, dn, d_list); })); }
 	CHK(dev_d2h(n_list, d_list, 4));
 	{
 		const uint32_t nl = *n_list; const wtz_lgap_t *gp = d_gp; const uint32_t *lst = d_list + 1;
 		CHK(sort_leftovers(d_list, nl, [&](uint64_t *d_k2){ return wtz_launch<K_misc>(nl, [=] WTZ_LAMBDA (uint64_t i){
 			const wtz_lgap_t G = gp[lst[i]];
 			const int32_t nc = G.dq < 2 * G.w + 1 ? G.dq : 2 * G.w + 1;
-			unsigned long long wgt = (unsigned long long)(G.dt > 0 ? G.dt : 0) * (unsigned long long)((nc > 0 ? nc : 0) / 64 + 1);
+			unsigned long long wgt = (G.dq > 0 && G.dt > 0) ? (unsigned long long)G.dt * (unsigned long long)(nc / 64 + 1) : 0ull;
 			if(wgt > 0xFFFFFFFEull) wgt = 0xFFFFFFFEull;
 			d_k2[i] = 0xFFFFFFFFull - wgt;
 		}); }));
 	}
-	if(c->sw.profile) fprintf(stderr, "[lane-profile] %llu window slots, K-sw2 gaps by band class <=16 / <=32 / <=64 / <=104: %u / %u / %u / %u, %u left to the wavefront kernel\n",
-		(unsigned long long)nwt, ccnt[0], ccnt[1], ccnt[2], ccnt[3], *n_list);
+	if(c->sw.profile) fprintf(stderr, "[lane-profile] %llu window slots, K-sw2 lane rounds %u with %u / %u / %u / %u / %u / %u gaps, %u left to the wavefront kernel\n",
+		(unsigned long long)nwt, n_rounds, per_round[0], per_round[1], per_round[2], per_round[3], per_round[4], per_round[5], *n_list);
 	return WTZ_OK;
 }
 
@@ -378,17 +390,39 @@
 	return WTZ_OK;
 }
 
-static int run_gap_wave(wtz_ctx *c, const wtz_env_t &V, const wtz_wintask_t *d_wt, const wtz_alnitem_t *d_items, wtz_gapres_t *d_gaps, const uint32_t *d_glist, uint32_t n_glist, uint64_t nwt){
+static int gap_profile(const wtz_ctx *c, const wtz_lgap_t *d_gp, const uint32_t *d_glist, uint32_t n_glist, uint64_t nwt, uint32_t n_def){
+	std::vector<uint32_t> lst(n_glist); std::vector<wtz_lgap_t> gp((size_t)nwt);
+	CHK(dev_sync()); CHK(dev_d2h(lst.data(), d_glist + 1, (size_t)n_glist * 4)); CHK(dev_d2h(gp.data(), d_gp, (size_t)nwt * sizeof(wtz_lgap_t)));
+	unsigned long long n_empty = 0, n_doubled = 0, n_outside = 0, n_cols = 0, n_rows = 0, n_other = 0, cells_pre = 0, hist[12] = {0}, rows_ok[12] = {0};
+	for(uint32_t i = 0; i < n_glist; i++){
+		const wtz_lgap_t &G = gp[lst[i]];
+		if(G.w < 0) continue;
+		if(G.dq <= 0 || G.dt <= 0){ n_empty++; continue; }
+		const int32_t nc = G.dq < 2 * G.w + 1 ? G.dq : 2 * G.w + 1;
+		if(G.cells){ n_doubled++; cells_pre += G.cells; int k = 0; while(k < 11 && ((int32_t)c->P.w << k) < G.w) k++; hist[k]++; if(G.dt <= WTZ_LG_MAXROWS) rows_ok[k]++; continue; }
+		if(nc > WTZ_LN_MAXCOLS || G.dt > WTZ_LG_MAXROWS){ n_outside++; if(nc > WTZ_LN_MAXCOLS) n_cols++; if(G.dt > WTZ_LG_MAXROWS) n_rows++; continue; }
+		n_other++;
+	}
+	fprintf(stderr, "[gap-profile] %llu window slots, %u on a wavefront: empty side %llu, band doubled beyond a lane %llu (cells already counted %llu), outside the lane envelope from the start %llu (columns %llu, rows %llu), lane shape without a lane run %llu; %u wide gaps redone with 72 KB of LDS\n",
+		(unsigned long long)nwt, n_glist, n_empty, n_doubled, cells_pre, n_outside, n_cols, n_rows, n_other, n_def);
+	fprintf(stderr, "[gap-profile] doubled gaps by the width they start from on the wavefront (w << k, k = 1 ..): %llu %llu %llu %llu %llu %llu %llu; of these with <= %d rows: %llu %llu %llu %llu %llu %llu %llu\n",
+		hist[1], hist[2], hist[3], hist[4], hist[5], hist[6], hist[7], WTZ_LG_MAXROWS, rows_ok[1], rows_ok[2], rows_ok[3], rows_ok[4], rows_ok[5], rows_ok[6], rows_ok[7]);
+	return WTZ_OK;
+}
+
+static int run_gap_wave(wtz_ctx *c, const wtz_env_t &V, const wtz_wintask_t *d_wt, const wtz_alnitem_t *d_items, wtz_gapres_t *d_gaps, const wtz_lgap_t *d_gp, const uint32_t *d_glist, uint32_t n_glist, uint64_t nwt){
 #ifdef WTZ_EMUL
 	(void)c; (void)nwt;
-	return wtz_launch_coop<K_gap>(n_glist, [=] WTZ_LAMBDA (uint64_t t){ wtz_task_gap((uint32_t)t, V, d_wt, d_items, d_gaps, (uint32_t*)NULL, (const uint32_t*)d_glist); }, WTZ_GAP_LDS_BYTES);
+	return wtz_launch_coop<K_gap>(n_glist, [=] WTZ_LAMBDA (uint64_t t){ wtz_task_gap((uint32_t)t, V, d_wt, d_items, d_gaps, d_gp, (uint32_t*)NULL, (wtz_gdefer_t*)NULL, (const uint32_t*)d_glist); }, WTZ_GAP_LDS_BYTES);
 #else
-	uint32_t *d_defer = NULL, n_def = 0; CHK(dev_alloc((void**)&d_defer, (size_t)(nwt + 1) * 4)); CHK(dev_set(d_defer, 0, 4));
+	uint32_t *d_ndef = NULL, n_def = 0; wtz_gdefer_t *d_defer = NULL;
+	CHK(dev_alloc((void**)&d_ndef, 4)); CHK(dev_set(d_ndef, 0, 4)); CHK(dev_alloc((void**)&d_defer, ((size_t)n_glist + 1) * sizeof(wtz_gdefer_t)));
 	STAGE(c, "K_gap");
-	CHK(wtz_launch_coop<K_gap>(n_glist, [=] WTZ_LAMBDA (uint64_t t){ wtz_task_gap((uint32_t)t, V, d_wt, d_items, d_gaps, d_defer, (const uint32_t*)d_glist, 0u); }, WTZ_GAP_LDS_BYTES));
-	CHK(dev_d2h(&n_def, d_defer, 4));
-	if(n_def) CHK(wtz_launch_coop<K_gap_wide>(n_def, [=] WTZ_LAMBDA (uint64_t t){ wtz_task_gap((uint32_t)t, V, d_wt, d_items, d_gaps, NULL, d_defer, (uint32_t)WTZ_GAP_WIDE_LDS_BYTES); }, WTZ_GAP_WIDE_LDS_BYTES));
-	if(c->sw.profile){ CHK(dev_sync()); fprintf(stderr, "[gap-profile] %llu window slots, %u wide gaps redone with 72 KB of LDS\n", (unsigned long long)nwt, n_def); }
+	CHK(wtz_launch_coop<K_gap>(n_glist, [=] WTZ_LAMBDA (uint64_t t){ wtz_task_gap((uint32_t)t, V, d_wt, d_items, d_gaps, d_gp, d_ndef, d_defer, (const uint32_t*)d_glist, (const wtz_gdefer_t*)NULL, 0u); }, WTZ_GAP_LDS_BYTES));
+	CHK(dev_d2h(&n_def, d_ndef, 4));
+	if(n_def) CHK(wtz_launch_coop<K_gap_wide>(n_def, [=] WTZ_LAMBDA (uint64_t t){ wtz_task_gap((uint32_t)t, V, d_wt, d_items, d_gaps, d_gp, (uint32_t*)NULL, (wtz_gdefer_t*)NULL, (const uint32_t*)NULL, (const wtz_gdefer_t*)d_defer, (uint32_t)WTZ_GAP_WIDE_LDS_BYTES); }, WTZ_GAP_WIDE_LDS_BYTES));
+	if(c->sw.profile && d_gp && d_glist) CHK(gap_profile(c, d_gp, d_glist, n_glist, nwt, n_def));
+	else if(c->sw.profile){ CHK(dev_sync()); fprintf(stderr, "[gap-profile] %llu window slots, %u wide gaps redone with 72 KB of LDS\n", (unsigned long long)nwt, n_def); }
 	return WTZ_OK;
 #endif
 }
@@ -468,19 +502,19 @@
 #endif
 	STAGE(c, "K_stitch_left");
 	CHK(wtz_launch_wave<K_stitch_left>(m, [=] WTZ_LAMBDA (uint64_t t){ wtz_task_stitch_left((uint32_t)t, V, d_items, d_st, d_jl, d_rgeo); }));
-	uint32_t *d_glist = NULL, n_glist = (uint32_t)nwt;
+	uint32_t *d_glist = NULL, n_glist = (uint32_t)nwt; wtz_lgap_t *d_gp = NULL;
 	wtz_timer tgap; tgap.start();
 	if(c->sw.gap_lane){
 		CHK(dev_alloc((void**)&d_glist, (size_t)(nwt + 1) * 4));
 		STAGE(c, "K-sw2 lane pipeline");
-		CHK(run_gap_lane(c, V, d_wt, nwt, d_items, d_gaps, d_glist, &n_glist));
+		CHK(run_gap_lane(c, V, d_wt, nwt, d_items, d_gaps, d_glist, &n_glist, &d_gp));
 	}
 #ifndef WTZ_EMUL
 	if(gap_side){ HIPCHK(hipEventRecord(c->ev_gap_fork, g_stream)); HIPCHK(hipStreamWaitEvent(c->stream_gap, c->ev_gap_fork, 0)); }
-	{ wtz_stream_scope on_gap_stream(gap_side ? c->stream_gap : g_stream); CHK(run_gap_wave(c, V, d_wt, d_items, d_gaps, d_glist, n_glist, nwt)); }
+	{ wtz_stream_scope on_gap_stream(gap_side ? c->stream_gap : g_stream); CHK(run_gap_wave(c, V, d_wt, d_items, d_gaps, d_gp, d_glist, n_glist, nwt)); }
 	if(gap_side) HIPCHK(hipEventRecord(c->ev_gap_join, c->stream_gap));
 #else
-	CHK(run_gap_wave(c, V, d_wt, d_items, d_gaps, d_glist, n_glist, nwt));
+	CHK(run_gap_wave(c, V, d_wt, d_items, d_gaps, d_gp, d_glist, n_glist, nwt));
 #endif
 	if(!gap_side) tgap.lap();
 #ifndef WTZ_EMUL
diff --git a/smartdenovo_amd/csrc/wtz_tasks.h b/smartdenovo_amd/csrc/wtz_tasks.h
--- a/smartdenovo_amd/csrc/wtz_tasks.h
+++ b/smartdenovo_amd/csrc/wtz_tasks.h
@@ -702,26 +702,48 @@
 }
 #endif
 
+#define WTZ_LG_MAXROWS 768
+typedef struct { int32_t dq, dt, w, qe, te, pad; unsigned long long cells; } wtz_lgap_t;
+WTZ_HD bool wtz_lgap_fits(const wtz_lgap_t &G, uint64_t *ky, int32_t *cls){
+	if(G.dq <= 0 || G.dt <= 0 || G.dt > WTZ_LG_MAXROWS) return false;
+	const int32_t n_col = G.dq < 2 * G.w + 1 ? G.dq : 2 * G.w + 1;
+	if(n_col > WTZ_LN_MAXCOLS) return false;
+	*ky = 0x3FFFFull - (uint64_t)(((uint32_t)n_col << 11) | (uint32_t)G.dt);
+	*cls = (int32_t)wtz_lane_class(n_col);
+	return true;
+}
+typedef struct { uint32_t t; int32_t w; unsigned long long cells; } wtz_gdefer_t;
 WTZ_HD void wtz_task_gap(uint32_t t, const wtz_env_t &V, const wtz_wintask_t *tasks, const wtz_alnitem_t *items, wtz_gapres_t *gaps,
-		uint32_t *defer = NULL, const uint32_t *list = NULL, uint32_t wide_lds = 0){
-	if(list) t = list[1 + t];
-	const wtz_params_t *P = V.P;
+		const wtz_lgap_t *gp = NULL, uint32_t *ndefer = NULL, wtz_gdefer_t *defer = NULL, const uint32_t *list = NULL, const wtz_gdefer_t *resume = NULL, uint32_t wide_lds = 0){
+	const wtz_params_t *P = V.P;
+	int32_t w = P->w; unsigned long long cells0 = 0;
+	if(resume){ const wtz_gdefer_t rs = resume[t]; t = rs.t; w = rs.w; cells0 = rs.cells; }
+	else if(list) t = list[1 + t];
 	const wtz_alnitem_t &it = items[tasks[t].item];
 	const uint32_t k = tasks[t].widx;
 	wtz_gapres_t g; memset(&g, 0, sizeof g);
 	const unsigned long long pt_task = WTZ_PROF_T(); (void)pt_task;
 	wtz_gapres_t *slot = gaps + (it.regs - items[0].regs) + k;
-	if(k == 0 || it.regs[k].pass != 1){ if(WTZ_LANE == 0) *slot = g; return; }
-	int32_t prev = -1;
-	for(int32_t j = (int32_t)k - 1; j >= 0; j--) if(it.regs[j].pass == 1){ prev = j; break; }
-	if(prev < 0){ if(WTZ_LANE == 0) *slot = g; return; }
+	int32_t dq, dt, qe1, te1;
+	if(gp){
+		const wtz_lgap_t G = gp[t];
+		if(G.w < 0){ if(WTZ_LANE == 0) *slot = g; return; }
+		dq = G.dq; dt = G.dt; qe1 = G.qe; te1 = G.te;
+		if(!resume){ w = G.w; cells0 = G.cells; }
+	} else {
+		if(k == 0 || it.regs[k].pass != 1){ if(WTZ_LANE == 0) *slot = g; return; }
+		int32_t prev = -1;
+		for(int32_t j = (int32_t)k - 1; j >= 0; j--) if(it.regs[j].pass == 1){ prev = j; break; }
+		if(prev < 0){ if(WTZ_LANE == 0) *slot = g; return; }
+		const wtz_reg_t *reg1 = &it.regs[prev], *reg2 = &it.regs[k];
+		dq = reg2->x.qb - reg1->x.qe; dt = reg2->x.tb - reg1->x.te; qe1 = reg1->x.qe; te1 = reg1->x.te;
+	}
 	const int32_t M = P->M, X = P->X, I = P->O, D = P->O, E = P->E;
-	const wtz_reg_t *reg1 = &it.regs[prev], *reg2 = &it.regs[k];
 	const wtz_readview pb1 = wtz_view(V.R, it.q, 0), pb2 = wtz_view(V.R, it.c, it.dir);
-	const int32_t dq = reg2->x.qb - reg1->x.qe, dt = reg2->x.tb - reg1->x.te;
-	const wtz_seq_packed q = pb2.sub(reg1->x.qe, 1), tt = pb1.sub(reg1->x.te, 1);
+	const wtz_seq_packed q = pb2.sub(qe1, 1), tt = pb1.sub(te1, 1);
 	wtz_cigar_t tmp; tmp.init(V.pool, WTZ_LANE == 0 ? 32 : 0);
-	int32_t w = P->w, score, bad = 0;
+	int32_t score, bad = 0;
+	g.cells = cells0;
 #if defined(__HIP_DEVICE_COMPILE__)
 	bool from_reg = false; uint32_t n_runs = 0; uint32_t *runs = NULL; int32_t r_mat = 0, r_mis = 0;
 	{
@@ -734,7 +756,7 @@
 			wtz_gapdp_t G;
 			wtz_gap_problem_wave<false>(dq, q, dt, tt, P, w, lds, wide_lds, defer != NULL, V.pool, tmp, tr, mem, 0, G);
 			if(G.want_defer){
-				if(WTZ_LANE == 0){ const uint32_t idx = atomicAdd(&defer[0], 1u); defer[1 + idx] = t; }
+				if(WTZ_LANE == 0){ wtz_gdefer_t df; df.t = t; df.w = w; df.cells = g.cells; defer[atomicAdd(&ndefer[0], 1u)] = df; }
 				return;
 			}
 			score = G.score; from_reg = G.from_reg; runs = G.runs; n_runs = G.n_runs; r_mat = G.r_mat; r_mis = G.r_mis;
@@ -785,14 +807,12 @@
 	*slot = g;
 }
 
-#define WTZ_LG_MAXROWS 768
-typedef struct { uint32_t slot; int32_t dq, dt, w; } wtz_lgap_t;
 WTZ_HD void wtz_task_gplan(uint32_t t, const wtz_env_t &V, const wtz_wintask_t *tasks, const wtz_alnitem_t *items, wtz_gapres_t *gaps,
 		wtz_lgap_t *gp, uint32_t *runcap, uint64_t *key, uint32_t *val, uint8_t *done, uint32_t *ccnt){
 	const wtz_params_t *P = V.P;
 	const wtz_alnitem_t &it = items[tasks[t].item];
 	const uint32_t k = tasks[t].widx;
-	wtz_lgap_t G; G.slot = t; G.dq = G.dt = 0; G.w = 0;
+	wtz_lgap_t G; memset(&G, 0, sizeof G); G.w = -1;
 	uint32_t cap = 0; uint64_t ky = 0x3FFFFull; uint8_t dn = 0; int32_t cls = -1;
 	wtz_gapres_t *slot = gaps + (it.regs - items[0].regs) + k;
 	int32_t prev = -1;
@@ -801,16 +821,9 @@
 	else {
 		const wtz_reg_t *reg1 = &it.regs[prev], *reg2 = &it.regs[k];
 		const int32_t dq = reg2->x.qb - reg1->x.qe, dt = reg2->x.tb - reg1->x.te;
-		if(dq > 0 && dt > 0){
-			int32_t w = P->w; while(w < WTZ_ABSDIFF(dq, dt)) w <<= 1;
-			const int32_t n_col = dq < 2 * w + 1 ? dq : 2 * w + 1;
-			G.dq = dq; G.dt = dt; G.w = w;
-			if(n_col <= WTZ_LN_MAXCOLS && dt <= WTZ_LG_MAXROWS){
-				cap = (uint32_t)(dq + dt + 2);
-				ky = 0x3FFFFull - (uint64_t)(((uint32_t)n_col << 11) | (uint32_t)dt);
-				cls = (int32_t)wtz_lane_class(n_col);
-			}
-		}
+		int32_t w = P->w; while(w < WTZ_ABSDIFF(dq, dt)) w <<= 1;
+		G.dq = dq; G.dt = dt; G.w = w; G.qe = reg1->x.qe; G.te = reg1->x.te;
+		if(wtz_lgap_fits(G, &ky, &cls)) cap = (uint32_t)(dq + dt + 2);
 	}
 #if defined(__HIP_DEVICE_COMPILE__)
 	#pragma unroll
@@ -830,17 +843,13 @@
 	const uint32_t idx = lo + wv * WTZ_NLANES + WTZ_LANE;
 	const bool live = idx < hi;
 	const uint32_t t = live ? order[idx] : 0u;
-	wtz_lgap_t G; G.slot = 0; G.dq = G.dt = 0; G.w = P->w;
+	wtz_lgap_t G; memset(&G, 0, sizeof G); G.w = P->w;
 	if(live) G = gp[t];
 	const int32_t M = P->M, X = P->X, I = P->O, D = P->O, E = P->E;
 	wtz_seq_packed q, tt; q.bits = tt.bits = V.R.bits; q.start = tt.start = 0; q.strand = tt.strand = 1; q.comp = tt.comp = 0;
 	if(live){
 		const wtz_alnitem_t &it = items[tasks[t].item];
-		const uint32_t k = tasks[t].widx;
-		int32_t prev = -1;
-		for(int32_t j = (int32_t)k - 1; j >= 0; j--) if(it.regs[j].pass == 1){ prev = j; break; }
-		const wtz_reg_t *reg1 = &it.regs[prev];
-		q = wtz_view(V.R, it.c, it.dir).sub(reg1->x.qe, 1); tt = wtz_view(V.R, it.q, 0).sub(reg1->x.te, 1);
+		q = wtz_view(V.R, it.c, it.dir).sub(G.qe, 1); tt = wtz_view(V.R, it.q, 0).sub(G.te, 1);
 	}
 	constexpr uint32_t RS = (uint32_t)wtz_lane_geo<NC>::RS;
 	const uint32_t rows_max = (uint32_t)wtz_lane_wmax(G.dt);
@@ -857,7 +866,8 @@
 	if(live) res[t] = R;
 }
 WTZ_HD void wtz_task_gtb(uint32_t gw, uint32_t wv, uint32_t RS, const wtz_env_t &V, const wtz_wintask_t *tasks, const wtz_alnitem_t *items, const uint32_t *order, uint32_t lo, uint32_t hi,
-		const wtz_lgap_t *gp, const uint32_t *runoff, uint32_t *runs, const wtz_lres_t *res, wtz_gapres_t *gaps, uint8_t *done, const uint64_t *wtr, const uint32_t *wrm){
+		wtz_lgap_t *gp, const uint32_t *runoff, uint32_t *runs, const wtz_lres_t *res, wtz_gapres_t *gaps, uint8_t *done, const uint64_t *wtr, const uint32_t *wrm,
+		uint64_t *nkey, uint32_t *nval, uint32_t *ncnt){
 	const wtz_params_t *P = V.P;
 	const uint32_t idx = lo + wv * WTZ_NLANES + WTZ_LANE;
 	const uint64_t pa = wtr[gw];
@@ -866,13 +876,16 @@
 	const wtz_lgap_t G = gp[t];
 	wtz_lres_t R = res[t];
 	if(!(R.flags & WTZ_LR_DONE)) return;
-	if(R.score < 0 && G.w < (int32_t)P->W && G.w < WTZ_MAX(G.dq, G.dt)) return;
+	if(R.score < 0 && G.w < (int32_t)P->W && G.w < WTZ_MAX(G.dq, G.dt)){
+		wtz_lgap_t N = G; N.w = G.w << 1; N.cells = G.cells + R.cells;
+		gp[t] = N;
+		uint64_t ky; int32_t cls;
+		if(wtz_lgap_fits(N, &ky, &cls)){ const uint32_t z = WTZ_ATOMIC_INC32(&ncnt[4]); nkey[z] = ky; nval[z] = t; WTZ_ATOMIC_INC32(&ncnt[cls]); }
+		return;
+	}
 	const wtz_alnitem_t &it = items[tasks[t].item];
 	const uint32_t k = tasks[t].widx;
-	int32_t prev = -1;
-	for(int32_t j = (int32_t)k - 1; j >= 0; j--) if(it.regs[j].pass == 1){ prev = j; break; }
-	const wtz_reg_t *reg1 = &it.regs[prev];
-	const wtz_seq_packed q = wtz_view(V.R, it.c, it.dir).sub(reg1->x.qe, 1), tt = wtz_view(V.R, it.q, 0).sub(reg1->x.te, 1);
+	const wtz_seq_packed q = wtz_view(V.R, it.c, it.dir).sub(G.qe, 1), tt = wtz_view(V.R, it.q, 0).sub(G.te, 1);
 	const uint32_t *tr = (const uint32_t*)(uintptr_t)pa;
 	uint32_t *rr = runs + runoff[t];
 	const int32_t r0 = G.dt - 1, c0 = (r0 + G.w + 1 < G.dq ? r0 + G.w + 1 : G.dq) - 1;
@@ -880,7 +893,7 @@
 	wtz_gapres_t g; memset(&g, 0, sizeof g);
 	g.score = R.score; g.valid = 1; g.mat = R.mat; g.mis = R.mis; g.ins = R.ins; g.del = R.del; g.aln = R.mat + R.mis + R.ins + R.del;
 	for(uint32_t a = 0, b = R.n_runs; a + 1 < b; a++, b--){ const uint32_t x = rr[a]; rr[a] = rr[b - 1]; rr[b - 1] = x; }
-	g.cigar = rr; g.cigar_len = R.n_runs; g.cells = R.cells;
+	g.cigar = rr; g.cigar_len = R.n_runs; g.cells = G.cells + R.cells;
 	gaps[(it.regs - items[0].regs) + k] = g; done[t] = 1;
 }
 WTZ_HD void wtz_task_gdp_all(uint32_t wv, const wtz_lclass_t &L, const wtz_env_t &V, const wtz_wintask_t *tasks, const wtz_alnitem_t *items, const uint32_t *order,
@@ -893,10 +906,11 @@
 	else            wtz_task_gdp<16>(wv, wl, V, tasks, items, order, L.lo[3], L.hi[3], gp, res, wtr, wrm);
 }
 WTZ_HD void wtz_task_gtb_all(uint32_t wv, const wtz_lclass_t &L, const wtz_env_t &V, const wtz_wintask_t *tasks, const wtz_alnitem_t *items, const uint32_t *order,
-		const wtz_lgap_t *gp, const uint32_t *runoff, uint32_t *runs, const wtz_lres_t *res, wtz_gapres_t *gaps, uint8_t *done, const uint64_t *wtr, const uint32_t *wrm){
+		wtz_lgap_t *gp, const uint32_t *runoff, uint32_t *runs, const wtz_lres_t *res, wtz_gapres_t *gaps, uint8_t *done, const uint64_t *wtr, const uint32_t *wrm,
+		uint64_t *nkey, uint32_t *nval, uint32_t *ncnt){
 	uint32_t k = 0; while(k < 3 && wv >= L.wend[k]) k++;
 	const uint32_t wl = wv - (k ? L.wend[k - 1] : 0u);
-	wtz_task_gtb(wv, wl, 16u >> k, V, tasks, items, order, L.lo[k], L.hi[k], gp, runoff, runs, res, gaps, done, wtr, wrm);
+	wtz_task_gtb(wv, wl, 16u >> k, V, tasks, items, order, L.lo[k], L.hi[k], gp, runoff, runs, res, gaps, done, wtr, wrm, nkey, nval, ncnt);
 }
 WTZ_HD void wtz_task_glist(uint32_t t, const uint8_t *done, uint32_t *list){ if(!done[t]){ const uint32_t k = WTZ_ATOMIC_INC32(&list[0]); list[1 + k] = t; } }
 
diff --git a/smartdenovo_amd/csrc/wtz_testdp.h b/smartdenovo_amd/csrc/wtz_testdp.h
--- a/smartdenovo_amd/csrc/wtz_testdp.h
+++ b/smartdenovo_amd/csrc/wtz_testdp.h
@@ -122,14 +122,61 @@
 }
 #endif
 
+static int test_gap_stage(wtz_ctx *c, const wtz_dp_problem_t *pr, uint32_t n, bool lanes, std::vector<wtz_dpres_dev_t> &hr){
+	std::vector<wtz_reg_t> regs(2 * (size_t)n); std::vector<wtz_alnitem_t> items(n); std::vector<wtz_wintask_t> wt(2 * (size_t)n);
+	wtz_reg_t *d_regs = NULL; wtz_alnitem_t *d_items = NULL; wtz_wintask_t *d_wt = NULL; wtz_gapres_t *d_gaps = NULL;
+	const uint64_t nwt = 2 * (uint64_t)n;
+	CHK(dev_alloc((void**)&d_regs, (size_t)(nwt + 1) * sizeof(wtz_reg_t)));
+	for(uint32_t i = 0; i < n; i++){
+		const wtz_dp_problem_t &p = pr[i];
+		if(p.q_read >= c->n_reads || p.t_read >= c->n_reads) return wtz_fail(WTZ_E_ARG, "problem %u: read id out of range", i);
+		if(p.q_strand != 1 || p.t_strand != 1 || p.t_rev || p.q_len < 0 || p.t_len < 0 || p.q_from < 0 || p.t_from < 0
+				|| (int64_t)p.q_from + p.q_len > (int64_t)c->h_rdlen[p.q_read] || (int64_t)p.t_from + p.t_len > (int64_t)c->h_rdlen[p.t_read])
+			return wtz_fail(WTZ_E_ARG, "problem %u: a gap lies forward inside its reads, the target on the forward strand", i);
+		wtz_reg_t a, b; memset(&a, 0, sizeof a); memset(&b, 0, sizeof b);
+		a.pass = b.pass = 1; a.x.qe = p.q_from; a.x.te = p.t_from; b.x.qb = p.q_from + p.q_len; b.x.tb = p.t_from + p.t_len;
+		regs[2 * (size_t)i] = a; regs[2 * (size_t)i + 1] = b;
+		wtz_alnitem_t it; memset(&it, 0, sizeof it); it.q = p.t_read; it.c = p.q_read; it.dir = p.q_rev ? 1u : 0u; it.nwin = 2; it.regs = d_regs + 2 * (size_t)i;
+		items[i] = it;
+		wt[2 * (size_t)i].item = wt[2 * (size_t)i + 1].item = i; wt[2 * (size_t)i].widx = 0; wt[2 * (size_t)i + 1].widx = 1;
+	}
+	CHK(dev_h2d(d_regs, regs.data(), regs.size() * sizeof(wtz_reg_t)));
+	CHK(dev_alloc((void**)&d_items, (size_t)n * sizeof(wtz_alnitem_t))); CHK(dev_h2d(d_items, items.data(), (size_t)n * sizeof(wtz_alnitem_t)));
+	CHK(dev_alloc((void**)&d_wt, (size_t)(nwt + 1) * sizeof(wtz_wintask_t))); CHK(dev_h2d(d_wt, wt.data(), wt.size() * sizeof(wtz_wintask_t)));
+	CHK(dev_alloc((void**)&d_gaps, (size_t)(nwt + 1) * sizeof(wtz_gapres_t))); CHK(dev_set(d_gaps, 0, (size_t)(nwt + 1) * sizeof(wtz_gapres_t)));
+	const wtz_env_t V = ctx_env(c);
+	uint32_t *d_glist = NULL, n_glist = (uint32_t)nwt; wtz_lgap_t *d_gp = NULL;
+	if(lanes){
+		CHK(dev_alloc((void**)&d_glist, (size_t)(nwt + 1) * 4));
+		CHK(run_gap_lane(c, V, d_wt, nwt, d_items, d_gaps, d_glist, &n_glist, &d_gp));
+	}
+	CHK(run_gap_wave(c, V, d_wt, d_items, d_gaps, d_gp, d_glist, n_glist, nwt));
+	CHK(dev_sync());
+	std::vector<wtz_gapres_t> g((size_t)nwt); CHK(dev_d2h(g.data(), d_gaps, (size_t)nwt * sizeof(wtz_gapres_t)));
+	std::vector<uint32_t> lst(n_glist); std::vector<uint8_t> on_wave((size_t)nwt, lanes ? 0 : 1);
+	if(lanes && n_glist){ CHK(dev_d2h(lst.data(), d_glist + 1, (size_t)n_glist * 4)); for(uint32_t k = 0; k < n_glist; k++) on_wave[lst[k]] = 1; }
+	for(uint32_t i = 0; i < n; i++){
+		const wtz_gapres_t &x = g[2 * (size_t)i + 1];
+		wtz_dpres_dev_t r; memset(&r, 0, sizeof r);
+		r.x.score = x.score; r.x.aln = x.aln; r.x.mat = x.mat; r.x.mis = x.mis; r.x.ins = x.ins; r.x.del = x.del;
+		r.cigar = x.cigar; r.cigar_len = x.cigar_len; r.cells = x.cells; r.bad = (x.bad || !x.valid) ? 1 : 0; r.form = on_wave[2 * (size_t)i + 1] ? 1 : 64;
+		hr[i] = r;
+	}
+	return WTZ_OK;
+}
+
 extern "C" int wtz_test_dp(wtz_ctx_t *c, int32_t kind, int32_t form, const wtz_dp_problem_t *pr, uint32_t n, wtz_dp_result_t *out, uint32_t *cigar, uint64_t cigar_cap){
 	BATCH_ARGS(c, n, pr && out && (cigar || !cigar_cap), NULL, NULL);
+	const bool gap_stage = kind == WTZ_DP_GLOBAL && (form == 65 || form == 66);
 #ifdef WTZ_EMUL
-	(void)kind; (void)form;
-	return wtz_fail(WTZ_E_STATE, "wtz_test_dp drives the DEVICE forms of the banded DPs: it needs the HIP build");
-#else
+	if(!gap_stage) return wtz_fail(WTZ_E_STATE, "wtz_test_dp drives the DEVICE forms of the banded DPs: it needs the HIP build");
+#endif
 	CTX_ENTER(c);
 	std::vector<uint64_t> h_off; CHK(batch_begin(c, h_off));
+	std::vector<wtz_dpres_dev_t> hr(n);
+	if(gap_stage){ CHK(test_gap_stage(c, pr, n, form == 65, hr)); }
+#ifndef WTZ_EMUL
+	else {
 	std::vector<wtz_dpprob_dev_t> hp(n);
 	for(uint32_t i = 0; i < n; i++){
 		const wtz_dp_problem_t &p = pr[i];
@@ -137,7 +184,6 @@
 		hp[i] = d;
 	}
 	const wtz_env_t V = ctx_env(c);
-	std::vector<wtz_dpres_dev_t> hr(n);
 	if(kind == WTZ_DP_SHIFT){
 		std::vector<wtz_extjob_t> jobs(n);
 		for(uint32_t i = 0; i < n; i++){ wtz_extjob_t j; memset(&j, 0, sizeof j); j.q = hp[i].q; j.t = hp[i].t; j.qlen = hp[i].qlen; j.tlen = hp[i].tlen; j.init_score = hp[i].init_score; j.W = hp[i].W; j.item = i; j.valid = 1; jobs[i] = j; }
@@ -178,6 +224,8 @@
 		CHK(dev_sync());
 		CHK(dev_d2h(hr.data(), d_res, (size_t)n * sizeof(wtz_dpres_dev_t)));
 	} else return wtz_fail(WTZ_E_ARG, "unknown DP kind %d", kind);
+	}
+#endif
 	CHK(pool_check(c, "wtz_test_dp"));
 	uint64_t off = 0;
 	for(uint32_t i = 0; i < n; i++){
@@ -195,6 +243,5 @@
 		out[i] = o;
 	}
 	return WTZ_OK;
-#endif
-}
-#endif
+}
+#endif
```

Measured after the change: 10.72, median of 5. About the same (+0.3%).
